# ChASE-library/ChASE

Hardware: AMD Instinct MI355X
Metric: chebyshev_filter_hemm_gflops (higher is better)
Workload: dtype complex f64

## Files before the change

chase_amd/capi.py:

```python
import ctypes as C
import os
import numpy as np

_HERE = os.path.dirname(os.path.abspath(__file__))
LIB_PATH = os.environ.get("CHASE_HIP_LIB") or os.path.join(_HERE, "lib", "libchase_hip.so")


class ChaseHipError(RuntimeError):
    def __init__(self, code, where, text=""):
        super().__init__(f"{where} failed with status {code}: {text}")
        self.code = code


def _load():
    if not os.path.exists(LIB_PATH):
        raise ImportError(
            f"{LIB_PATH} not found: build it with `make` (or `python -c 'import __graft_entry__ as g; g.build()'`). "
            "chase_amd has no CPU fallback.")
    try:
        import torch
    except Exception:
        pass
    return C.CDLL(LIB_PATH, mode=C.RTLD_GLOBAL)

# ... 141 lines not shown

    def timer_start(self):
        check(lib.chase_hip_timer_start(self.h), "timer_start")

    def timer_stop(self):
        ms = C.c_float()
        check(lib.chase_hip_timer_stop(self.h, C.byref(ms)), "timer_stop")
        return ms.value

    def gemm(self, opA, m, n, k, alpha, A, lda, B, ldb, beta, Cm, ldc, cplx):
        op = opA.encode()[0:1]
        if cplx:
            check(lib.chase_hip_gemm_z(self.h, op, m, n, k, _z2(alpha), A, lda, B, ldb, _z2(beta), Cm, ldc), "gemm_z")
        else:
            check(lib.chase_hip_gemm_d(self.h, op, m, n, k, float(alpha), A, lda, B, ldb, float(beta), Cm, ldc),
                  "gemm_d")

    def hash64(self, ptr, m, n, ld, cplx):
        h = C.c_ulonglong()
        check(lib.chase_hip_hash64(self.h, int(cplx), m, n, ptr, ld, C.byref(h)), "hash64")
        return h.value

    def gen_clement(self, N, cplx, scale=1.0, perturb=0.0, seed=42):
        dH = self.empty((N, N), np.complex128 if cplx else np.float64)
        check(lib.chase_hip_gen_clement(self.h, int(cplx), dH.ptr, N, N, N, N, N, 1, 0, 0, N, 1, 0, 0, float(scale),
                                        float(perturb), seed), "gen_clement")
        return dH

    def load_matrix(self, path, N, cplx):
        dH = self.empty((N, N), np.complex128 if cplx else np.float64)
        check(lib.chase_hip_load_matrix_shard(self.h, str(path).encode(), int(cplx), N, N, N, N, 1, 0, N, 1, 0, dH.ptr, N),
              "load_matrix_shard")
        return dH

    def save_matrix(self, path, dA):
        cplx = dA.dtype == np.complex128
        check(lib.chase_hip_save_matrix(self.h, str(path).encode(), int(cplx), dA.shape[0],
                                        dA.shape[1] if len(dA.shape) > 1 else 1, dA.ptr, dA.shape[0]), "save_matrix")

    def gen_bse(self, N, cplx=True, dmin=1.0, dmax=11.0, offdiag=1e-3, seed=7):
        dH = self.empty((N, N), np.complex128 if cplx else np.float64)
        check(lib.chase_hip_gen_bse(self.h, int(cplx), dH.ptr, N, N, N, N, N, 1, 0, N, 1, 0, float(dmin), float(dmax),
                                    float(offdiag), seed), "gen_bse")
        return dH

    def mfma_f64_peak(self):
        t = c_double()
        check(lib.chase_hip_mfma_f64_peak(self.h, C.byref(t)), "mfma_f64_peak")
        return t.value

    def hbm_copy_peak(self, nbytes=1 << 30):
        g = c_double()
        check(lib.chase_hip_hbm_copy_peak(self.h, nbytes, C.byref(g)), "hbm_copy_peak")
        return g.value


_sig("chase_hip_set_lapack_lib", c_int, C.c_char_p)
_sig("chase_hip_lapack_provider", C.c_char_p)
_sig("chase_hip_set_host_threads", c_int, c_int)
_sig("chase_hip_ctx_set_phase", c_int, c_void_p, c_int)
_sig("chase_hip_ctx_set_gemm_min_rounds", c_int, c_void_p, c_int)
_sig("chase_hip_fill_normal", c_int, c_void_p, c_int, c_int, c_int, c_void_p, c_long, c_long, c_long, c_long,
     C.c_ulonglong)
_sig("chase_hip_gen_clement", c_int, c_void_p, c_int, c_void_p, c_long, c_int, c_int, c_long, c_int, c_int, c_int,
     c_long, c_int, c_int, c_int, c_long, c_double, c_double, C.c_ulonglong)
_sig("chase_hip_gen_bse", c_int, c_void_p, c_int, c_void_p, c_long, c_int, c_int, c_long, c_int, c_int, c_int, c_int, c_int,
     c_int, c_double, c_double, c_double, C.c_ulonglong)
_sig("chase_hip_load_matrix_shard", c_int, c_void_p, C.c_char_p, c_int, c_long, c_int, c_int, c_int, c_int, c_int, c_int,
     c_int, c_int, c_void_p, c_long)
_sig("chase_hip_save_matrix", c_int, c_void_p, C.c_char_p, c_int, c_int, c_int, c_void_p, c_long)
_sig("chase_hip_shift_diag", c_int, c_void_p, c_int, c_int, c_void_p, c_long, c_double)
_sig("chase_hip_shift_list", c_int, c_void_p, c_int, c_void_p, c_long, c_void_p, c_void_p, c_int, c_double)
_sig("chase_hip_lacpy", c_int, c_void_p, c_int, c_int, c_int, c_void_p, c_long, c_void_p, c_long)
_sig("chase_hip_swap_cols", c_int, c_void_p, c_int, c_int, c_void_p, c_long, c_long, c_long)
_sig("chase_hip_permute_cols", c_int, c_void_p, c_int, c_int, c_void_p, c_long, c_void_p, c_long, P(c_int), P(c_int),
     c_int)
_sig("chase_hip_upload_matrix", c_int, c_void_p, c_int, c_int, c_int, c_void_p, c_long, c_void_p, c_long)
_sig("chase_hip_download_matrix", c_int, c_void_p, c_int, c_int, c_int, c_void_p, c_long, c_void_p, c_long)
_sig("chase_hip_scale_rows", c_int, c_void_p, c_int, c_int, c_int, c_void_p, c_long, c_int, c_double)
_sig("chase_hip_scale_rows_bc", c_int, c_void_p, c_int, c_int, c_int, c_void_p, c_long, c_long, c_long, c_int, c_int,
     c_double)
_sig("chase_hip_conj", c_int, c_void_p, c_int, c_int, c_void_p, c_long)
_sig("chase_hip_resid_norms", c_int, c_void_p, c_int, c_int, c_int, c_void_p, c_long, c_void_p, c_long, c_void_p,
     c_void_p, c_int)
_sig("chase_hip_gemm_workspace_bytes", c_size_t, c_int, C.c_char, c_int, c_int, c_int, c_int, c_int)
_sig("chase_hip_herk", c_int, c_void_p, c_int, c_int, c_int, c_void_p, c_long, c_void_p, c_long)
_sig("chase_hip_herkx", c_int, c_void_p, c_int, c_int, c_int, c_void_p, c_long, c_void_p, c_long, c_void_p, c_long, c_int)
_sig("chase_hip_abs_trace", c_int, c_void_p, c_int, c_int, c_void_p, c_long, P(c_double))
_sig("chase_hip_potrf_upper", c_int, c_void_p, c_int, c_int, c_void_p, c_long)
_sig("chase_hip_trsm_right_upper", c_int, c_void_p, c_int, c_int, c_int, c_void_p, c_long, c_void_p, c_long)
_sig("chase_hip_cholqr", c_int, c_void_p, c_int, c_int, c_int, c_void_p, c_long, c_void_p, c_long, c_int, c_long)
_sig("chase_hip_houseqr", c_int, c_void_p, c_int, c_int, c_int, c_void_p, c_long)
_sig("chase_hip_heevd", c_int, c_void_p, c_int, c_int, c_void_p, c_long, c_void_p)
_sig("chase_hip_heevd_gpu", c_int, c_void_p, c_int, c_int, c_void_p, c_long, c_void_p)
_sig("chase_hip_heevd_host", c_int, c_int, c_int, c_void_p, c_long, c_void_p)
_sig("chase_hip_stedc", c_int, c_void_p, c_int, c_void_p, c_void_p, c_void_p, c_void_p, c_long)
_sig("chase_hip_stemr_host", c_int, c_int, c_void_p, c_void_p, c_void_p, c_void_p, c_int)
_sig("chase_hip_col_dot", c_int, c_void_p, c_int, c_int, c_int, c_void_p, c_long, c_void_p, c_long, c_void_p)
_sig("chase_hip_col_nrm2", c_int, c_void_p, c_int, c_int, c_int, c_void_p, c_long, c_void_p)
_sig("chase_hip_col_axpy", c_int, c_void_p, c_int, c_int, c_int, c_void_p, c_int, c_int, c_double, c_void_p, c_long,
     c_void_p, c_long)
_sig("chase_hip_col_scal", c_int, c_void_p, c_int, c_int, c_int, c_void_p, c_int, c_void_p, c_long)
_sig("chase_hip_pack_upper", c_int, c_void_p, c_int, c_int, c_void_p, c_long, c_void_p)
_sig("chase_hip_unpack_upper", c_int, c_void_p, c_int, c_int, c_void_p, c_void_p, c_long, c_int)


class Stats(C.Structure):
    _fields_ = [("iterations", c_size_t), ("filtered_vecs", c_size_t), ("lanczos_vecs", c_size_t),
                ("locked", c_size_t), ("t_all", c_double), ("t_init", c_double), ("t_lanczos", c_double),
                ("t_filter", c_double), ("t_qr", c_double), ("t_rr", c_double), ("t_resid", c_double),
                ("filter_ms_device", c_double), ("lowerb", c_double), ("upperb", c_double), ("lambda_", c_double)]

    def as_dict(self):
        return {k: getattr(self, k) for k, _ in self._fields_}


_sig("chase_hip_solver_create", c_int, P(c_void_p), c_void_p, c_int, c_size_t, c_size_t, c_size_t, c_void_p, c_size_t,
     c_void_p, c_size_t, c_void_p, c_int)
_sig("chase_hip_solver_destroy", c_int, c_void_p)
_sig("chase_hip_solver_set", c_int, c_void_p, C.c_char_p, c_double)
_sig("chase_hip_solver_get", c_int, c_void_p, C.c_char_p, P(c_double))
_sig("chase_hip_solver_solve", c_int, c_void_p, c_int)
ITER_FN = C.CFUNCTYPE(c_int, c_void_p, c_size_t, c_size_t, c_size_t, c_size_t)
_sig("chase_hip_solver_set_iteration_hook", c_int, c_void_p, ITER_FN, c_void_p)
_sig("chase_hip_set_gemm3m", c_int, c_int)
_sig("chase_hip_ctx_gemm_counters", c_int, c_void_p, c_int, P(c_double), P(c_double), P(C.c_ulonglong), c_int)
_sig("chase_hip_solver_stats", c_int, c_void_p, P(Stats))
_sig("chase_hip_solver_resid", P(c_double), c_void_p)
_sig("chase_hip_solver_trace", C.c_char_p, c_void_p)
_sig("chase_hip_solver_recompute_residuals", c_int, c_void_p, c_size_t, c_void_p, c_void_p)
_sig("chase_hip_solver_tape_mode", c_int, c_void_p, c_int)
_sig("chase_hip_solver_tape_data", c_int, c_void_p, P(P(c_double)), P(c_size_t))
_sig("chase_hip_solver_tape_load", c_int, c_void_p, c_void_p, c_size_t)
_sig("chase_hip_resid_norms_dev", c_int, c_void_p, c_int, c_int, c_int, c_void_p, c_long, c_void_p, c_long, c_void_p,
     c_void_p, c_int)
_sig("chase_hip_solver_peek_v", c_int, c_void_p, c_void_p, c_void_p, c_size_t)
_sig("chase_hip_solver_hash_v", c_int, c_void_p, c_void_p, c_size_t, P(C.c_ulonglong))
_sig("chase_hip_op_start", c_int, c_void_p)
_sig("chase_hip_op_end", c_int, c_void_p)
_sig("chase_hip_op_initvecs", c_int, c_void_p, c_int)
_sig("chase_hip_op_reinit_columns", c_int, c_void_p, c_size_t, P(c_size_t), c_size_t)
_sig("chase_hip_op_shift", c_int, c_void_p, c_double, c_int)
_sig("chase_hip_op_hemm", c_int, c_void_p, c_size_t, P(c_double), P(c_double), c_size_t, c_size_t)
_sig("chase_hip_op_qr", c_int, c_void_p, c_size_t, c_double)
_sig("chase_hip_op_rr", c_int, c_void_p, c_void_p, c_size_t)
_sig("chase_hip_op_resd", c_int, c_void_p, c_void_p, c_void_p, c_size_t)
_sig("chase_hip_op_swap", c_int, c_void_p, c_size_t, c_size_t)
_sig("chase_hip_op_lock", c_int, c_void_p, c_size_t)
_sig("chase_hip_op_lanczos", c_int, c_void_p, c_size_t, c_size_t, P(c_double), c_void_p, c_void_p, c_void_p)
_sig("chase_hip_op_lanczos_dos", c_int, c_void_p, c_size_t, c_size_t, c_void_p)
_sig("chase_hip_op_check_symmetry", c_int, c_void_p, P(c_int))
_sig("chase_hip_op_sym_or_herm", c_int, c_void_p, c_char)
_sig("chase_hip_complete_hermitian", c_int, c_void_p, c_int, c_char, c_int, c_void_p, c_long)
_sig("chase_hip_hash64", c_int, c_void_p, c_int, c_int, c_int, c_void_p, c_long, P(C.c_ulonglong))
_sig("chase_hip_cols_indexed", c_int, c_void_p, c_int, c_int, c_void_p, c_long, c_void_p, c_long, c_void_p, c_int)
_sig("chase_hip_tri_mask_bc", c_int, c_void_p, c_int, c_char, c_int, c_int, c_void_p, c_long, c_long, c_int, c_int, c_long, c_int,
     c_int)
_sig("chase_hip_conj_transpose_add", c_int, c_void_p, c_int, c_int, c_int, c_void_p, c_long, c_void_p, c_void_p, c_void_p, c_long)


def set_iteration_hook(solver, fn):
    if fn is None:
        solver._iter_cb = ITER_FN()
    else:
        def _cb(user, it, filtered, locked, unconverged):
            try:
                return 1 if fn(int(it), int(filtered), int(locked), int(unconverged)) else 0
            except Exception as e:
                print("iteration hook failed:", repr(e), flush=True)
                return 1
        solver._iter_cb = ITER_FN(_cb)
    check(lib.chase_hip_solver_set_iteration_hook(solver.h, solver._iter_cb, None), "set_iteration_hook")


def recompute_residuals(solver, ncols, lam=None):
    lam = np.ascontiguousarray(solver.ritzv[:ncols] if lam is None else lam, dtype=np.float64)
    out = np.zeros(ncols)
    check(lib.chase_hip_solver_recompute_residuals(solver.h, ncols, lam.ctypes.data, out.ctypes.data), "recompute_residuals")
    return out


TAPE_OFF, TAPE_RECORD, TAPE_REPLAY = 0, 1, 2


def tape_mode(solver, mode):
    check(lib.chase_hip_solver_tape_mode(solver.h, int(mode)), "tape_mode")


def tape_get(solver):
    p, n = P(c_double)(), c_size_t()
    check(lib.chase_hip_solver_tape_data(solver.h, C.byref(p), C.byref(n)), "tape_data")
    return np.ctypeslib.as_array(p, shape=(n.value,)).copy() if n.value else np.zeros(0)


def tape_load(solver, tape):
    t = np.ascontiguousarray(tape, dtype=np.float64)
    check(lib.chase_hip_solver_tape_load(solver.h, t.ctypes.data, t.size), "tape_load")


def gemm_counters(ctx, phase, reset=False):
    a, b, n = c_double(), c_double(), C.c_ulonglong()
    check(lib.chase_hip_ctx_gemm_counters(ctx.h, phase, C.byref(a), C.byref(b), C.byref(n), int(reset)), "gemm_counters")
    return a.value, b.value, n.value


class GemmLaunch(C.Structure):
    _fields_ = [(f, c_int) for f in ("row0", "col0", "k0", "m", "n", "k", "beta_one", "bn_cols", "narrow", "m3", "ragged",
                                     "glds_ok", "gm", "gn")] + \
               [("full_tiles", c_long), ("tail_tiles", c_long)] + \
               [(f, c_int) for f in ("tail_sk", "tail_kchunk", "group_rows", "forced_split")] + \
               [("slab_bytes", c_size_t), ("plane_bytes", c_size_t)]

    def as_dict(self):
        return {k: getattr(self, k) for k, _ in self._fields_}


_sig("chase_hip_gemm_plan", c_int, c_int, c_char, c_int, c_int, c_int, c_long, c_long, c_int, c_int, c_int, c_int,
     P(GemmLaunch), c_int)


def gemm_plan(cplx, op, m, n, k, lda=None, ldb=None, aligned=True, phase=0, num_cu=256, min_rounds=0):
    lda = (m if op == "N" else k) if lda is None else lda
    ldb = k if ldb is None else ldb
    args = (int(cplx), op.encode(), m, n, k, max(lda, 1), max(ldb, 1), int(aligned), phase, num_cu, min_rounds)
    cnt = lib.chase_hip_gemm_plan(*args, None, 0)
    if cnt < 0:
        check(cnt, "gemm_plan")
    out = (GemmLaunch * max(cnt, 1))()
    assert lib.chase_hip_gemm_plan(*args, out, cnt) == cnt
    return [out[i].as_dict() for i in range(cnt)]


class Solver:

    def __init__(self, ctx, H, nev, nex, V=None, h_on_device_ptr=None, N=None, cplx=None):
        self.ctx = ctx
        if h_on_device_ptr is None:
            assert H.flags.f_contiguous and H.ndim == 2 and H.shape[0] == H.shape[1]
            self.cplx = bool(np.iscomplexobj(H))
            self.N = H.shape[0]
            self.H = H
            hptr, on_dev = H.ctypes.data, 0
        else:
            self.cplx, self.N, self.H = bool(cplx), int(N), None
            hptr, on_dev = h_on_device_ptr, 1
        self.nev, self.nex = nev, nex
        dt = np.complex128 if self.cplx else np.float64
        self.V = np.zeros((self.N, nev + nex), dtype=dt, order="F") if V is None else V
        assert self.V.flags.f_contiguous and self.V.dtype == dt
        self.ritzv = np.zeros(nev + nex, dtype=np.float64)
        h = c_void_p()
        check(lib.chase_hip_solver_create(C.byref(h), ctx.h, int(self.cplx), self.N, nev, nex, hptr, self.N,
                                          self.V.ctypes.data, self.N, self.ritzv.ctypes.data, on_dev),
              "solver_create")
        self.h = h

    def close(self):
        if self.h:
            lib.chase_hip_solver_destroy(self.h)
            self.h = None

    def set(self, **kw):
        for k, v in kw.items():
            check(lib.chase_hip_solver_set(self.h, k.encode(), float(v)), f"solver_set({k})")

    def get(self, key):
        v = c_double()
        check(lib.chase_hip_solver_get(self.h, key.encode(), C.byref(v)), f"solver_get({key})")
        return v.value

    def solve(self, trace=False):
        check(lib.chase_hip_solver_solve(self.h, int(trace)), "solver_solve")
        return self.stats()

    def set_iteration_hook(self, fn):
        set_iteration_hook(self, fn)

    def stats(self):
        s = Stats()
        check(lib.chase_hip_solver_stats(self.h, C.byref(s)), "solver_stats")
        return s.as_dict()

    def resid(self):
        p = lib.chase_hip_solver_resid(self.h)
        return np.ctypeslib.as_array(p, shape=(self.nev + self.nex,)).copy()

    def trace(self):
        return lib.chase_hip_solver_trace(self.h).decode().splitlines()

    def recompute_residuals(self, ncols, lam=None):
        return recompute_residuals(self, ncols, lam)

    def peek_v(self):
        out = np.empty_like(self.V, order="F")
        check(lib.chase_hip_solver_peek_v(self.h, self.ctx.h, out.ctypes.data, self.N), "peek_v")
        return out

    def Start(self): check(lib.chase_hip_op_start(self.h), "Start")
    def End(self): check(lib.chase_hip_op_end(self.h), "End")
    def initVecs(self, random): check(lib.chase_hip_op_initvecs(self.h, int(random)), "initVecs")

    def ReinitColumns(self, fixednev, cols):
        a = (c_size_t * len(cols))(*cols)
        check(lib.chase_hip_op_reinit_columns(self.h, fixednev, a, len(cols)), "ReinitColumns")
    def Shift(self, c, isunshift=False): check(lib.chase_hip_op_shift(self.h, float(c), int(isunshift)), "Shift")

    def HEMM(self, block, alpha, beta, offset_left, offset_right=0):
        check(lib.chase_hip_op_hemm(self.h, block, _z2(alpha), _z2(beta), offset_left, offset_right), "HEMM")

    def QR(self, fixednev, cond): check(lib.chase_hip_op_qr(self.h, fixednev, float(cond)), "QR")

    def RR(self, block, offset):
        check(lib.chase_hip_op_rr(self.h, self.ritzv.ctypes.data + 8 * offset, block), "RR")

    def Resd(self, offset):
        n = self.nev + self.nex - offset
        out = np.zeros(n)
        check(lib.chase_hip_op_resd(self.h, self.ritzv.ctypes.data + 8 * offset, out.ctypes.data, offset), "Resd")
        return out

    def Swap(self, i, j): check(lib.chase_hip_op_swap(self.h, i, j), "Swap")
    def Lock(self, n): check(lib.chase_hip_op_lock(self.h, n), "Lock")

    def Lanczos(self, M, numvec):
        ub = c_double()
        if numvec == 0:
            check(lib.chase_hip_op_lanczos(self.h, M, 0, C.byref(ub), None, None, None), "Lanczos")
            return ub.value
        theta, tau, ritzV = np.zeros(M * numvec), np.zeros(M * numvec), np.zeros(M * M)
        check(lib.chase_hip_op_lanczos(self.h, M, numvec, C.byref(ub), theta.ctypes.data, tau.ctypes.data,
                                       ritzV.ctypes.data), "Lanczos")
        return ub.value, theta, tau, ritzV.reshape(M, M, order="F")

    def checkSymmetryEasy(self):
        f = c_int()
        check(lib.chase_hip_op_check_symmetry(self.h, C.byref(f)), "checkSymmetryEasy")
        return bool(f.value)

    def symOrHermMatrix(self, uplo):
        check(lib.chase_hip_op_sym_or_herm(self.h, uplo.encode()[0:1]), "symOrHermMatrix")


_sig("chase_hip_solver_create_pseudo", c_int, P(c_void_p), c_void_p, c_int, c_size_t, c_size_t, c_size_t, c_void_p,
     c_size_t, c_void_p, c_size_t, c_void_p, c_int)
_sig("chase_hip_op_hemm_h2", c_int, c_void_p, c_size_t, P(c_double), P(c_double), P(c_double), c_size_t, c_size_t)
_sig("chase_hip_op_kconj", c_int, c_void_p, c_size_t)
_sig("chase_hip_pseudo_rr_small", c_int, c_void_p, c_int, c_int, c_void_p, c_void_p, c_void_p)
_sig("chase_hip_set_identity", c_int, c_void_p, c_int, c_int, c_void_p, c_long)


_sig("chase_hip_solver_lanczos_for_h2", c_int, c_void_p, c_int, c_int, P(c_double), P(c_size_t))


class PseudoSolver(Solver):

    def __init__(self, ctx, H, nev, nex):
        assert H.flags.f_contiguous and H.shape[0] == H.shape[1]
        self.ctx, self.H = ctx, H
        self.cplx = bool(np.iscomplexobj(H))
        self.N, self.nev, self.nex = H.shape[0], nev, nex
        dt = np.complex128 if self.cplx else np.float64
        self.ncol = 2 * (nev + nex)
        self.V = np.zeros((self.N, self.ncol), dtype=dt, order="F")
        self.ritzv = np.zeros(self.ncol)
# ... 31 lines not shown
```

chase_amd/csrc/capi_blas.hip:

```cpp
#include <hip/hip_runtime.h>
#include <cmath>
#include <cstdio>
#include <cstdlib>
#include <cstring>
#include <limits>
#include <vector>
#include "../../include/chase_hip.h"
#include "ctx.h"
#include "kernels.h"
#include "host_lapack.h"

using namespace chase_hip;

#define HIPCHK(x)                                                                                                      \
    do {                                                                                                               \
        hipError_t e_ = (x);                                                                                           \
        if (e_ != hipSuccess) return hip_fail(e_, #x);                                                                 \
    } while (0)
#define KCHK(x, what)                                                                                                  \
    do {                                                                                                               \
        int e_ = (x);                                                                                                  \
        if (e_) return hip_fail((hipError_t)e_, what);                                                                 \
    } while (0)
#define RCCHK(x)                                                                                                       \
    do {                                                                                                               \
        int r_ = (x);                                                                                                  \
        if (r_) return r_;                                                                                             \
    } while (0)

namespace {
constexpr int NB = 64;

inline int ept_of(int cplx) { return cplx ? 2 : 1; }

int gemm(chase_hip_ctx* c, int cplx, char op, int m, int n, int k, double ar, double ai, const double* A, long lda,
         const double* B, long ldb, double br, double bi, double* C, long ldc)
{
    if (m <= 0 || n <= 0) return 0;
    const double alpha[2] = {ar, ai}, beta[2] = {br, bi};
    return c->gemm(cplx != 0, op, m, n, k, alpha, A, lda, B, ldb, beta, C, ldc);
}
}

extern "C" {

int chase_hip_set_lapack_lib(const char* path) { return lapack_bind(path); }
const char* chase_hip_lapack_provider(void)
{
    lapack_bind(nullptr);
    return lapack_provider();
}
int chase_hip_host_lapack_warmup(void)
{
    int rc = lapack_bind(nullptr);
    if (rc) return rc;
    static bool done = false;
    if (done) return 0;
    const int n = 8;
    double d[n], e[n], w[n], Z[n * n];
    for (int i = 0; i < n; ++i) { d[i] = i; e[i] = 0.5; }
    rc = host_stedc(n, d, e, w, Z, n);
    if (rc) return rc;
    for (int i = 0; i < n; ++i) { d[i] = i; e[i] = 0.5; }
    rc = host_stemr(n, d, e, w, Z, n);
    if (rc) return rc;
    double A[2 * n * n];
    for (int i = 0; i < 2 * n * n; ++i) A[i] = 0.0;
    for (int i = 0; i < n; ++i) A[2 * (i + i * n)] = 1.0 + i;
    rc = host_heevd(true, n, A, n, w);
    if (rc) return rc;
    done = true;
    return 0;
}

int chase_hip_set_host_threads(int n)
{
    lapack_bind(nullptr);
    lapack_set_threads(n);
    return 0;
}

int chase_hip_ctx_set_phase(chase_hip_ctx* c, int phase)
{
    if (!c) return set_error(CHASE_HIP_EINVAL, "set_phase: NULL ctx");
    (void)hipSetDevice(c->device);
    c->phase = phase;
    return 0;
}

int chase_hip_ctx_set_gemm_min_rounds(chase_hip_ctx* c, int rounds)
{
    if (!c) return set_error(CHASE_HIP_EINVAL, "ctx_set_gemm_min_rounds: NULL context");
    c->gemm_min_rounds = rounds < 0 ? 0 : (rounds > 16 ? 16 : rounds);
    return 0;
}

int chase_hip_fill_normal(chase_hip_ctx* c, int cplx, int m, int n, void* X, long ldx, long grow0, long gcol0, long gld,
                          unsigned long long seed)
{
    if (!c || !X) return set_error(CHASE_HIP_EINVAL, "fill_normal: NULL argument");
    (void)hipSetDevice(c->device);
    if (c->oplog_on) c->oplog_add("fill_normal", m, n, 0, 0);
    if (m < 0 || n < 0 || ldx < m) return set_error(CHASE_HIP_EINVAL, "fill_normal: bad shape");
    KCHK(fill_normal(c->stream, cplx != 0, (double*)X, ldx, m, n, grow0, gcol0, gld, seed), "fill_normal");
    return 0;
}

int chase_hip_fill_normal_bc(chase_hip_ctx* c, int cplx, int m, int n, void* X, long ldx, long gld, int mb, int pr,
                             int pi, unsigned long long seed)
{
    if (!c || !X) return set_error(CHASE_HIP_EINVAL, "fill_normal_bc: NULL argument");
    (void)hipSetDevice(c->device);
    if (c->oplog_on) c->oplog_add("fill_normal_bc", m, n, 0, 0);
    if (m < 0 || n < 0 || ldx < m || mb <= 0 || pr <= 0) return set_error(CHASE_HIP_EINVAL, "fill_normal_bc: bad shape");
    KCHK(fill_normal(c->stream, cplx != 0, (double*)X, ldx, m, n, 0, 0, gld, seed, mb, pr, pi), "fill_normal_bc");
    return 0;
}

int chase_hip_rows_indexed(chase_hip_ctx* c, int cplx, const void* in, long ld_in, void* out, long ld_out,
                           const int* idx_dev, int np, int ncols, int scatter)
{
    if (!c) return set_error(CHASE_HIP_EINVAL, "rows_indexed: NULL ctx");
    (void)hipSetDevice(c->device);
    if (c->oplog_on) c->oplog_add("rows_indexed", np, ncols, scatter, 0);
    KCHK(rows_indexed(c->stream, cplx != 0, (const double*)in, ld_in, (double*)out, ld_out, idx_dev, np, ncols, scatter),
         "rows_indexed");
    return 0;
}

int chase_hip_hash64(chase_hip_ctx* c, int cplx, int m, int n, const void* A, long lda, unsigned long long* out_host)
{
    if (!c || !out_host) return set_error(CHASE_HIP_EINVAL, "hash64: NULL argument");
    (void)hipSetDevice(c->device);
    if (m < 0 || n < 0 || lda < m) return set_error(CHASE_HIP_EINVAL, "hash64: bad shape");
    *out_host = 0;
    if (m == 0 || n == 0) return 0;
    if (!A) return set_error(CHASE_HIP_EINVAL, "hash64: NULL matrix");
    const int e = ept_of(cplx);
    RCCHK(c->ensure_buf(chase_hip_ctx::BUF_SCAL, 4096));
    unsigned long long* d = (unsigned long long*)c->bufs[chase_hip_ctx::BUF_SCAL];
    HIPCHK(hipMemsetAsync(d, 0, sizeof(unsigned long long), c->stream));
    KCHK(hash64(c->stream, (const double*)A, lda * e, (long)m * e, n, d), "hash64");
    HIPCHK(hipMemcpyAsync(out_host, d, sizeof(unsigned long long), hipMemcpyDeviceToHost, c->stream));
    HIPCHK(hipStreamSynchronize(c->stream));
    return 0;
}

int chase_hip_cols_indexed(chase_hip_ctx* c, int cplx, int m, const void* in, long ld_in, void* out, long ld_out,
                           const int* idx_dev, int ncols)
{
    if (!c) return set_error(CHASE_HIP_EINVAL, "cols_indexed: NULL ctx");
    (void)hipSetDevice(c->device);
    if (c->oplog_on) c->oplog_add("cols_indexed", m, ncols, 0, 0);
    if (m < 0 || ncols < 0 || ld_in < m || ld_out < m) return set_error(CHASE_HIP_EINVAL, "cols_indexed: bad shape");
    if (m == 0 || ncols == 0) return 0;
    if (!in || !out || !idx_dev) return set_error(CHASE_HIP_EINVAL, "cols_indexed: NULL argument");
    const int e = ept_of(cplx);
    KCHK(copy_cols_indexed_range(c->stream, (const double*)in, ld_in * e, (double*)out, ld_out * e, (long)m * e, idx_dev, 0, ncols),
         "cols_indexed");
    return 0;
}

int chase_hip_complete_hermitian(chase_hip_ctx* c, int cplx, char uplo, int n, void* A, long lda)
{
    if (!c) return set_error(CHASE_HIP_EINVAL, "complete_hermitian: NULL ctx");
    (void)hipSetDevice(c->device);
    if (c->oplog_on) c->oplog_add("complete_hermitian", n, uplo, 0, 0);
    if (uplo != 'U' && uplo != 'L' && uplo != 'u' && uplo != 'l') return set_error(CHASE_HIP_EINVAL, "complete_hermitian: uplo must be 'U' or 'L'");
    if (n < 0 || lda < n) return set_error(CHASE_HIP_EINVAL, "complete_hermitian: bad shape");
    if (n == 0) return 0;
    if (!A) return set_error(CHASE_HIP_EINVAL, "complete_hermitian: NULL matrix");
    if (uplo == 'U' || uplo == 'u') KCHK(mirror_upper(c->stream, (double*)A, lda, n, ept_of(cplx)), "mirror_upper");
    else KCHK(mirror_lower(c->stream, (double*)A, lda, n, ept_of(cplx), 0), "mirror_lower");
    return 0;
}

int chase_hip_tri_mask_bc(chase_hip_ctx* c, int cplx, char uplo, int mloc, int nloc, void* H, long ldh, long mb, int pr, int pi,
                          long nb, int pc, int pj)
{
    if (!c) return set_error(CHASE_HIP_EINVAL, "tri_mask_bc: NULL ctx");
    (void)hipSetDevice(c->device);
    if (c->oplog_on) c->oplog_add("tri_mask_bc", mloc, nloc, uplo, 0);
    if (uplo != 'U' && uplo != 'L' && uplo != 'u' && uplo != 'l') return set_error(CHASE_HIP_EINVAL, "tri_mask_bc: uplo must be 'U' or 'L'");
    if (mloc < 0 || nloc < 0 || ldh < mloc || mb <= 0 || nb <= 0 || pr <= 0 || pc <= 0 || pi < 0 || pi >= pr || pj < 0 || pj >= pc)
        return set_error(CHASE_HIP_EINVAL, "tri_mask_bc: bad shape / layout");
    if (mloc == 0 || nloc == 0) return 0;
    if (!H) return set_error(CHASE_HIP_EINVAL, "tri_mask_bc: NULL matrix");
    KCHK(tri_mask_bc(c->stream, cplx != 0, (double*)H, ldh, mloc, nloc, mb, pr, pi, nb, pc, pj, (uplo == 'U' || uplo == 'u') ? 1 : 0),
         "tri_mask_bc");
    return 0;
}

int chase_hip_conj_transpose_add(chase_hip_ctx* c, int cplx, int nr, int nc, const void* P, long ldp, const int* rowmap_dev,
                                 const int* colmap_dev, void* H, long ldh)
{
    if (!c) return set_error(CHASE_HIP_EINVAL, "conj_transpose_add: NULL ctx");
    (void)hipSetDevice(c->device);
    if (c->oplog_on) c->oplog_add("conj_transpose_add", nr, nc, 0, 0);
    if (nr < 0 || nc < 0 || ldp < nr) return set_error(CHASE_HIP_EINVAL, "conj_transpose_add: bad shape");
    if (nr == 0 || nc == 0) return 0;
    if (!P || !H || !rowmap_dev || !colmap_dev) return set_error(CHASE_HIP_EINVAL, "conj_transpose_add: NULL argument");
    KCHK(conj_transpose_add(c->stream, cplx != 0, (const double*)P, ldp, nr, nc, rowmap_dev, colmap_dev, (double*)H, ldh),
         "conj_transpose_add");
    return 0;
}

int chase_hip_gen_clement(chase_hip_ctx* c, int cplx, void* H, long ldh, int mloc, int nloc, long N, int mb, int pr,
                          int pi, long roff, int nb, int pc, int pj, long coff, double scale, double perturb,
                          unsigned long long seed)
{
    if (!c || !H) return set_error(CHASE_HIP_EINVAL, "gen_clement: NULL argument");
    (void)hipSetDevice(c->device);
    if (mloc < 0 || nloc < 0 || ldh < mloc || mb <= 0 || nb <= 0 || pr <= 0 || pc <= 0)
        return set_error(CHASE_HIP_EINVAL, "gen_clement: bad shape");
    KCHK(gen_clement(c->stream, cplx != 0, (double*)H, ldh, mloc, nloc, N, mb, pr, pi, roff, nb, pc, pj, coff, scale,
                     perturb, seed),
         "gen_clement");
    return 0;
}

int chase_hip_gen_bse(chase_hip_ctx* c, int cplx, void* H, long ldh, int mloc, int nloc, long N, int mb, int pr, int pi,
                      int nb, int pc, int pj, double dmin, double dmax, double offdiag, unsigned long long seed)
{
    if (!c || !H) return set_error(CHASE_HIP_EINVAL, "gen_bse: NULL argument");
    (void)hipSetDevice(c->device);
    if (mloc < 0 || nloc < 0 || ldh < mloc || mb <= 0 || nb <= 0 || pr <= 0 || pc <= 0 || N <= 0 || N % 2)
        return set_error(CHASE_HIP_EINVAL, "gen_bse: bad shape (N must be even)");
    KCHK(gen_bse(c->stream, cplx != 0, (double*)H, ldh, mloc, nloc, N, mb, pr, pi, nb, pc, pj, dmin, dmax, offdiag, seed),
         "gen_bse");
    return 0;
}

int chase_hip_shift_diag(chase_hip_ctx* c, int cplx, int n, void* H, long ldh, double shift)
{
    if (!c || (!H && n > 0)) return set_error(CHASE_HIP_EINVAL, "shift_diag: NULL argument");
    (void)hipSetDevice(c->device);
    if (c->oplog_on) c->oplog_add("shift_diag", n, 0, 0, 0);
    if (n < 0 || ldh < n) return set_error(CHASE_HIP_EINVAL, "shift_diag: bad shape");
    KCHK(shift_diag(c->stream, (double*)H, ldh, n, ept_of(cplx), shift), "shift_diag");
    return 0;
}

int chase_hip_shift_list(chase_hip_ctx* c, int cplx, void* H, long ldh, const int* rows_dev, const int* cols_dev, int cnt,
                         double shift)
{
    if (!c) return set_error(CHASE_HIP_EINVAL, "shift_list: NULL ctx");
    (void)hipSetDevice(c->device);
    if (c->oplog_on) c->oplog_add("shift_list", cnt, 0, 0, 0);
    if (cnt < 0) return set_error(CHASE_HIP_EINVAL, "shift_list: negative count");
    KCHK(shift_list(c->stream, (double*)H, ldh, rows_dev, cols_dev, cnt, ept_of(cplx), shift), "shift_list");
    return 0;
}

int chase_hip_lacpy(chase_hip_ctx* c, int cplx, int m, int n, const void* A, long lda, void* B, long ldb)
{
    if (!c) return set_error(CHASE_HIP_EINVAL, "lacpy: NULL ctx");
    (void)hipSetDevice(c->device);
    if (c->oplog_on) c->oplog_add("lacpy", m, n, 0, 0);
    if (m < 0 || n < 0 || lda < m || ldb < m) return set_error(CHASE_HIP_EINVAL, "lacpy: bad shape");
    if (m == 0 || n == 0) return 0;
    const int e = ept_of(cplx);
    KCHK(copy2d(c->stream, (const double*)A, lda * e, (double*)B, ldb * e, (long)m * e, n), "lacpy");
    return 0;
}

int chase_hip_swap_cols(chase_hip_ctx* c, int cplx, int m, void* V, long ldv, long i, long j)
{
    if (!c || !V) return set_error(CHASE_HIP_EINVAL, "swap_cols: NULL argument");
    (void)hipSetDevice(c->device);
    if (c->oplog_on) c->oplog_add("swap_cols", m, 0, 0, 0);
    if (i == j) return 0;
    const int e = ept_of(cplx);
    double* v = (double*)V;
    KCHK(swap_cols(c->stream, v + i * ldv * e, v + j * ldv * e, (long)m * e), "swap_cols");
    return 0;
}

int chase_hip_permute_cols(chase_hip_ctx* c, int cplx, int m, void* V, long ldv, void* scratch, long lds_,
                           const int* src_host, const int* dst_host, int cnt)
{
    if (!c || !V || !scratch) return set_error(CHASE_HIP_EINVAL, "permute_cols: NULL argument");
    (void)hipSetDevice(c->device);
    if (c->oplog_on) c->oplog_add("permute_cols", m, cnt, 0, 0);
    if (cnt <= 0) return 0;
    const int e = ept_of(cplx);
    RCCHK(c->ensure_buf(chase_hip_ctx::BUF_LAMBDA, (size_t)2 * cnt * sizeof(int) + 64));
    int* ds = (int*)c->bufs[chase_hip_ctx::BUF_LAMBDA];
    int* dd = ds + cnt;
    HIPCHK(hipMemcpyAsync(ds, src_host, (size_t)cnt * sizeof(int), hipMemcpyHostToDevice, c->stream));
    HIPCHK(hipMemcpyAsync(dd, dst_host, (size_t)cnt * sizeof(int), hipMemcpyHostToDevice, c->stream));
    HIPCHK(hipStreamSynchronize(c->stream));
    KCHK(copy_cols_indexed(c->stream, (const double*)V, ldv * e, (double*)scratch, lds_ * e, (long)m * e, ds, dd, cnt),
         "permute gather");
    KCHK(copy_cols_indexed(c->stream, (const double*)scratch, lds_ * e, (double*)V, ldv * e, (long)m * e, dd, dd, cnt),
         "permute scatter");
    return 0;
}

int chase_hip_upload_matrix(chase_hip_ctx* c, int cplx, int m, int n, const void* host, long ldh, void* dev, long ldd)
{
    if (!c) return set_error(CHASE_HIP_EINVAL, "upload_matrix: NULL ctx");
    (void)hipSetDevice(c->device);
    if (c->oplog_on) c->oplog_add("upload_matrix", m, n, 0, 0);
    if (m <= 0 || n <= 0) return 0;
    const size_t es = sizeof(double) * ept_of(cplx);
    HIPCHK(hipMemcpy2DAsync(dev, (size_t)ldd * es, host, (size_t)ldh * es, (size_t)m * es, n, hipMemcpyHostToDevice,
                            c->stream));
    HIPCHK(hipStreamSynchronize(c->stream));
    return 0;
}
int chase_hip_download_matrix(chase_hip_ctx* c, int cplx, int m, int n, const void* dev, long ldd, void* host, long ldh)
{
    if (!c) return set_error(CHASE_HIP_EINVAL, "download_matrix: NULL ctx");
    (void)hipSetDevice(c->device);
    if (c->oplog_on) c->oplog_add("download_matrix", m, n, 0, 0);
    if (m <= 0 || n <= 0) return 0;
    const size_t es = sizeof(double) * ept_of(cplx);
    HIPCHK(hipMemcpy2DAsync(host, (size_t)ldh * es, dev, (size_t)ldd * es, (size_t)m * es, n, hipMemcpyDeviceToHost,
                            c->stream));
    HIPCHK(hipStreamSynchronize(c->stream));
    return 0;
}

int chase_hip_scale_rows(chase_hip_ctx* c, int cplx, int m, int n, void* X, long ldx, int row0, double s)
{
    if (!c) return set_error(CHASE_HIP_EINVAL, "scale_rows: NULL ctx");
// ... 410 lines not shown
```

chase_amd/csrc/gemm_mfma_f64.hip:

```cpp

#include <hip/hip_runtime.h>
#include <stdint.h>
#include <algorithm>
#include <atomic>
#include <cstdlib>
#include <type_traits>
#include "../../include/chase_hip.h"
#include "kernels.h"

#ifndef CHASE_M3_PIPELINE
#define CHASE_M3_PIPELINE 1
#endif
#ifndef CHASE_M3_SPLANE
#define CHASE_M3_SPLANE 1
#endif
#ifndef CHASE_M3_DEPTH
#define CHASE_M3_DEPTH 2
#endif

namespace chase_hip {

typedef double d4_t __attribute__((ext_vector_type(4)));
typedef double d2_t __attribute__((ext_vector_type(2)));
typedef d2_t d2u_t __attribute__((aligned(8)));

template <bool CPLX, bool OPA_C, bool NARROW = false>
struct Cfg {
    static_assert(!(CPLX && NARROW), "the complex tile is 64 columns wide already");
    static constexpr int NTHREADS = 256;
    static constexpr int WAVES_M = 4, WAVES_N = 1;
    static constexpr int TM = 2;
    static constexpr int TN = (CPLX || NARROW) ? 4 : 8;
    static constexpr int BM = 16 * TM * WAVES_M;
    static constexpr int BN = 16 * TN * WAVES_N;
    static constexpr int BK = CPLX ? 8 : 16;
    static constexpr int KPU = CPLX ? 1 : 2;
    static constexpr int RPU = CPLX ? 1 : 2;
    static constexpr int A_UNITS = OPA_C ? BM * 8 : BK * (BM / RPU);
    static constexpr int B_UNITS = BN * 8;
    static constexpr int A_PASSES = A_UNITS / NTHREADS;
    static constexpr int B_PASSES = B_UNITS / NTHREADS;
    static constexpr int STAGE_UNITS = A_UNITS + B_UNITS;
    static constexpr int EPT = CPLX ? 2 : 1;
    static constexpr int STAGES = (CPLX || NARROW) ? 3 : 2;
    static constexpr bool PIPELINED = CPLX || NARROW;
    static constexpr int A_GLDS = A_UNITS / 64, B_GLDS = B_UNITS / 64;
    static constexpr int GLDS_PER_WAVE = (A_GLDS + B_GLDS) / 4;
};

__device__ __forceinline__ int kidx(int r, int ku) { return r * 8 + (ku ^ ((r >> 1) & 7)); }

__device__ __forceinline__ unsigned xcd_remap(unsigned b, unsigned nblk)
{
    const unsigned q = nblk >> 3, r = nblk & 7u, x = b & 7u;
    const unsigned base = (x < r) ? x * (q + 1) : r * (q + 1) + (x - r) * q;
    return base + (b >> 3);
}

__host__ __device__ __forceinline__ void tile_coords(int t, int gm, int gn, int GR, int& bm, int& bn)
{
    const int gsz = GR * gn;
    const int g = t / gsz;
    const int first = g * GR;
    const int rows = (gm - first < GR) ? gm - first : GR;
    const int r = t - g * gsz;
    bm = first + r % rows;
    bn = r / rows;
}

struct GemmArgs {
    const double* A; const double* B; double* C;
    long lda, ldb, ldc;
    int m, n, k;
    int gm, gn;
    int group_rows;
    int bn_cols;
    int full_tiles, tail_sk, tail_kchunk;
    double* slabs;
    int glds_ok;
    const double* S; int s_nkt;
    double alpha_re, alpha_im, beta_re, beta_im;
};

template <bool CPLX, bool OPA_C, int TAG, bool RAGGED, bool M3, bool NARROW = false>
__global__ __launch_bounds__(256, 2) void gemm_f64_kernel(GemmArgs p)
{
    static_assert(CPLX || !M3, "3M applies to complex products");
    using C_ = Cfg<CPLX, OPA_C, NARROW>;
    constexpr int BM = C_::BM, BN = C_::BN, BK = C_::BK, TM = C_::TM, TN = C_::TN;
    constexpr int EPT = C_::EPT, KPU = C_::KPU, RPU = C_::RPU;
    constexpr int UM = BM / RPU;

    extern __shared__ __attribute__((aligned(16))) d2_t lds[];

    const int tid = threadIdx.x;
    const int lane = tid & 63, wave = tid >> 6;
    const int wm = wave % C_::WAVES_M, wn = wave / C_::WAVES_M;
    const int c16 = lane & 15, q = lane >> 4;

    unsigned tile;
    int kbeg = 0, kend = p.k;
    bool raw = false;
    double* slab = nullptr;
    if (blockIdx.x < (unsigned)p.full_tiles) {
        tile = xcd_remap(blockIdx.x, (unsigned)p.full_tiles);
    } else {
        const unsigned P = xcd_remap(blockIdx.x - (unsigned)p.full_tiles, gridDim.x - (unsigned)p.full_tiles);
        tile = (unsigned)p.full_tiles + P / (unsigned)p.tail_sk;
        const int bz = (int)(P % (unsigned)p.tail_sk);
        kbeg = bz * p.tail_kchunk;
        kend = min(p.k, kbeg + p.tail_kchunk);
        raw = true;
        slab = p.slabs + (size_t)P * (BM * BN * EPT);
    }
    int bm, bn;
    tile_coords((int)tile, p.gm, p.gn, p.group_rows, bm, bn);
    const int row0 = bm * BM, col0 = bn * p.bn_cols;
    const int nkt = (kend > kbeg) ? (kend - kbeg + BK - 1) / BK : 0;

    const bool interior = (row0 + BM <= p.m) && (col0 + BN <= p.n);

    d2_t ra[C_::A_PASSES], rb[C_::B_PASSES];

    auto load_tile = [&](int k0) {
        const bool kfull = (k0 + BK <= kend);
        if (interior && kfull) {
            #pragma unroll
            for (int ps = 0; ps < C_::A_PASSES; ++ps) {
                const int idx = ps * 256 + tid;
                if constexpr (!OPA_C) {
                    const int kk = idx / UM, u = idx % UM;
                    const double* g = p.A + ((long)(k0 + kk) * p.lda + row0 + u * RPU) * EPT;
                    ra[ps] = *(const d2u_t*)g;
                } else {
                    const int r = idx >> 3, ku = idx & 7;
                    const double* g = p.A + ((long)(row0 + r) * p.lda + k0 + ku * KPU) * EPT;
                    ra[ps] = *(const d2u_t*)g;
                }
            }
            #pragma unroll
            for (int ps = 0; ps < C_::B_PASSES; ++ps) {
                const int idx = ps * 256 + tid;
                const int r = idx >> 3, ku = idx & 7;
                const double* g = p.B + ((long)(col0 + r) * p.ldb + k0 + ku * KPU) * EPT;
                rb[ps] = *(const d2u_t*)g;
            }
        } else {
            #pragma unroll
            for (int ps = 0; ps < C_::A_PASSES; ++ps) {
                const int idx = ps * 256 + tid;
                d2_t v = {0.0, 0.0};
                if constexpr (!OPA_C) {
                    const int kk = idx / UM, u = idx % UM;
                    const int gi = row0 + u * RPU, gk = k0 + kk;
                    if (gk < kend) {
                        const double* g = p.A + ((long)gk * p.lda + gi) * EPT;
                        if constexpr (CPLX) { if (gi < p.m) v = *(const d2u_t*)g; }
                        else { if (gi < p.m) v.x = g[0]; if (gi + 1 < p.m) v.y = g[1]; }
                    }
                } else {
                    const int r = idx >> 3, ku = idx & 7;
                    const int gi = row0 + r, gk = k0 + ku * KPU;
                    if (gi < p.m) {
                        const double* g = p.A + ((long)gi * p.lda + gk) * EPT;
                        if constexpr (CPLX) { if (gk < kend) v = *(const d2u_t*)g; }
                        else { if (gk < kend) v.x = g[0]; if (gk + 1 < kend) v.y = g[1]; }
                    }
                }
                ra[ps] = v;
            }
            #pragma unroll
            for (int ps = 0; ps < C_::B_PASSES; ++ps) {
                const int idx = ps * 256 + tid;
                const int r = idx >> 3, ku = idx & 7;
                const int gj = col0 + r, gk = k0 + ku * KPU;
                d2_t v = {0.0, 0.0};
                if (gj < p.n) {
                    const double* g = p.B + ((long)gj * p.ldb + gk) * EPT;
                    if constexpr (CPLX) { if (gk < kend) v = *(const d2u_t*)g; }
                    else { if (gk < kend) v.x = g[0]; if (gk + 1 < kend) v.y = g[1]; }
                }
                rb[ps] = v;
            }
        }
    };

    auto store_tile = [&](int stage) {
        d2_t* sA = lds + stage * C_::STAGE_UNITS;
        d2_t* sB = sA + C_::A_UNITS;
        #pragma unroll
        for (int ps = 0; ps < C_::A_PASSES; ++ps) {
            const int idx = ps * 256 + tid;
            if constexpr (!OPA_C) {
                sA[idx] = ra[ps];
            } else {
                const int r = idx >> 3, ku = idx & 7;
                sA[kidx(r, ku)] = ra[ps];
            }
        }
        #pragma unroll
        for (int ps = 0; ps < C_::B_PASSES; ++ps) {
            const int idx = ps * 256 + tid;
            const int r = idx >> 3, ku = idx & 7;
            sB[kidx(r, ku)] = rb[ps];
        }
    };

    constexpr int NACC = CPLX ? (M3 ? 3 : 2) : 1;
    d4_t acc[NACC][TN][TM];
    #pragma unroll
    for (int z = 0; z < NACC; ++z)
        #pragma unroll
        for (int j = 0; j < TN; ++j)
            #pragma unroll
            for (int i = 0; i < TM; ++i) acc[z][j][i] = d4_t{0.0, 0.0, 0.0, 0.0};

    const int wrow = wm * (16 * TM);
    const int wcol = wn * (16 * TN);
    const int jv = RAGGED ? __builtin_amdgcn_readfirstlane(min(p.bn_cols >> 4, max(0, (p.n - col0 - wcol + 15) >> 4))) : TN;

    struct Frag { d2_t b[TN]; double a[TM][2]; };

    auto read_chunk = [&](int stage, int ch, Frag& f) __attribute__((always_inline)) {
        const d2_t* sA = lds + stage * C_::STAGE_UNITS;
        const d2_t* sB = sA + C_::A_UNITS;
        const int ku = 4 * ch + q;
        if constexpr (CPLX || OPA_C) {
            #pragma unroll
            for (int i = 0; i < TM; ++i) {
                const int r = wrow + 16 * i + c16;
                d2_t v;
                if constexpr (OPA_C) v = sA[kidx(r, ku)];
                else                 v = sA[ku * UM + r];
                f.a[i][0] = v.x; f.a[i][1] = v.y;
            }
            #pragma unroll
            for (int j = 0; j < TN; ++j) f.b[j] = sB[kidx(wcol + 16 * j + c16, ku)];
        } else {
            #pragma unroll
            for (int j = 0; j < TN; ++j) f.b[j] = sB[kidx(wcol + 16 * j + c16, ku)];
            #pragma unroll
            for (int pr = 0; pr < TM / 2; ++pr)
                #pragma unroll
                for (int s = 0; s < 2; ++s) {
                    const int kk = 8 * ch + 2 * q + s;
                    const d2_t v = sA[kk * UM + (wrow / 2) + 16 * pr + c16];
                    f.a[2 * pr][s] = v.x;
                    f.a[2 * pr + 1][s] = v.y;
                }
        }
    };

    auto no_hook = [](int) __attribute__((always_inline)) {};
    auto mfma_chunk = [&](const Frag& f, auto&& hook) __attribute__((always_inline)) {
        constexpr bool FULL = !RAGGED;
        if constexpr (CPLX && M3) {
            double sa[TM], sb[TN];
            #pragma unroll
            for (int i = 0; i < TM; ++i) sa[i] = OPA_C ? f.a[i][0] - f.a[i][1] : f.a[i][0] + f.a[i][1];
            #pragma unroll
            for (int j = 0; j < TN; ++j) sb[j] = f.b[j].x + f.b[j].y;
            #pragma unroll
            for (int j = 0; j < TN; ++j) {
                #pragma unroll
                for (int i = 0; i < TM; ++i) {
                    if (FULL || j < jv) {
                        acc[0][j][i] = __builtin_amdgcn_mfma_f64_16x16x4f64(f.b[j].x, f.a[i][0], acc[0][j][i], 0, 0, 0);
                        acc[1][j][i] = __builtin_amdgcn_mfma_f64_16x16x4f64(f.b[j].y, f.a[i][1], acc[1][j][i], 0, 0, 0);
                        acc[2][j][i] = __builtin_amdgcn_mfma_f64_16x16x4f64(sb[j], sa[i], acc[2][j][i], 0, 0, 0);
                    }
                    hook(TM * j + i);
                }
            }
        } else if constexpr (CPLX) {
            double nb[TN];
            #pragma unroll
            for (int j = 0; j < TN; ++j) nb[j] = OPA_C ? -f.b[j].x : -f.b[j].y;
            #pragma unroll
            for (int j = 0; j < TN; ++j) {
                if (FULL || j < jv)
                #pragma unroll
                for (int i = 0; i < TM; ++i) {
                    acc[0][j][i] = __builtin_amdgcn_mfma_f64_16x16x4f64(f.b[j].x, f.a[i][0], acc[0][j][i], 0, 0, 0);
                    acc[1][j][i] = __builtin_amdgcn_mfma_f64_16x16x4f64(f.b[j].y, f.a[i][0], acc[1][j][i], 0, 0, 0);
                }
                hook(j);
            }
            #pragma unroll
            for (int j = 0; j < TN; ++j) {
                if (FULL || j < jv)
                #pragma unroll
                for (int i = 0; i < TM; ++i) {
                    acc[0][j][i] = __builtin_amdgcn_mfma_f64_16x16x4f64(OPA_C ? f.b[j].y : nb[j], f.a[i][1], acc[0][j][i], 0, 0, 0);
                    acc[1][j][i] = __builtin_amdgcn_mfma_f64_16x16x4f64(OPA_C ? nb[j] : f.b[j].x, f.a[i][1], acc[1][j][i], 0, 0, 0);
                }
                hook(TN + j);
            }
        } else {
            #pragma unroll
            for (int s = 0; s < 2; ++s)
                #pragma unroll
                for (int j = 0; j < TN; ++j) {
                    if (FULL || j < jv)
                    #pragma unroll
                    for (int i = 0; i < TM; ++i)
                        acc[0][j][i] = __builtin_amdgcn_mfma_f64_16x16x4f64(
                            s == 0 ? f.b[j].x : f.b[j].y, f.a[i][s], acc[0][j][i], 0, 0, 0);
                    hook(s * TN + j);
                }
        }
    };

    auto compute = [&](int stage, auto&& hook) __attribute__((always_inline)) {
        if constexpr (C_::PIPELINED && !M3) {
            Frag f0, f1;
            read_chunk(stage, 0, f0);
            read_chunk(stage, 1, f1);
            __builtin_amdgcn_sched_barrier(0);
            mfma_chunk(f0, hook);
            mfma_chunk(f1, no_hook);
        } else {
            {
                Frag f;
                read_chunk(stage, 0, f);
                mfma_chunk(f, hook);
            }
            {
                Frag f;
                read_chunk(stage, 1, f);
                mfma_chunk(f, no_hook);
            }
        }
    };

    bool done = false;
    {
        const int nfull = (kend - kbeg) / BK;
        if ((row0 + BM <= p.m) && nfull >= 1 && p.glds_ok) {
            const int wv = __builtin_amdgcn_readfirstlane(wave);
            constexpr int NA = C_::A_GLDS / 4, NB = C_::B_GLDS / 4;
            const char* sa[NA];
            unsigned va[NA];
#ifdef CHASE_DIAG_SAME_A
            const int row0_src = 0;
#else
            const int row0_src = row0;
#endif
#ifdef CHASE_DIAG_SAME_B
            const int col0_src = 0;
#else
            const int col0_src = col0;
#endif
            const char* sb = (const char*)(p.B + ((long)col0_src * p.ldb + kbeg) * EPT);
            unsigned vb[NB];
            #pragma unroll
            for (int u = 0; u < NA; ++u) {
                const int t = wv * NA + u;
                if constexpr (!OPA_C) {
                    const int kk = CPLX ? (t >> 1) : t, half = CPLX ? (t & 1) : 0;
                    sa[u] = (const char*)(p.A + ((long)(kbeg + kk) * p.lda + row0_src) * EPT + (long)half * 128);
                    va[u] = (unsigned)lane * 16u;
                } else {
                    const int rl = lane >> 3, ku = (lane & 7) ^ ((4 * t + (lane >> 4)) & 7);
                    sa[u] = (const char*)(p.A + ((long)(row0_src + 8 * t) * p.lda + kbeg) * EPT);
                    va[u] = (unsigned)(((long)rl * p.lda + ku * KPU) * EPT * 8);
                }
            }
            #pragma unroll
            for (int u = 0; u < NB; ++u) {
                const int t = wv * NB + u;
                const int r = 8 * t + (lane >> 3), ku = (lane & 7) ^ ((r >> 1) & 7);
                const int rc = min(r, p.n - 1 - col0);
                vb[u] = (unsigned)(((long)rc * p.ldb + ku * KPU) * EPT * 8);
            }
            const long stepA = (OPA_C ? (long)BK * EPT : (long)BK * p.lda * EPT) * 8;
            constexpr long stepB = (long)BK * EPT * 8;
            int st_issue = 0;
            auto issue_one = [&](int u, int stage) __attribute__((always_inline)) {
                constexpr bool SPLIT = CPLX && M3 && CHASE_M3_SPLANE;
                d2_t* sA = SPLIT ? lds + stage * C_::A_UNITS : lds + stage * C_::STAGE_UNITS;
                d2_t* sB = SPLIT ? lds + C_::STAGES * C_::A_UNITS + stage * C_::B_UNITS : sA + C_::A_UNITS;
                if (u < NA) {
                    const unsigned dst = (unsigned)(size_t)(__attribute__((address_space(3))) void*)(sA + (wv * NA + u) * 64);
                    asm volatile("s_mov_b32 m0, %2\n\ts_nop 0\n\tglobal_load_lds_dwordx4 %0, %1"
                                 :: "v"(va[u]), "s"(sa[u]), "s"(dst) : "memory");
                    sa[u] += stepA;
                } else {
                    const int ub = u - NA;
                    const unsigned dst = (unsigned)(size_t)(__attribute__((address_space(3))) void*)(sB + (wv * NB + ub) * 64);
                    asm volatile("s_mov_b32 m0, %2\n\ts_nop 0\n\tglobal_load_lds_dwordx4 %0, %1"
                                 :: "v"(vb[ub]), "s"(sb), "s"(dst) : "memory");
                }
                if (u == NA + NB - 1) sb += stepB;
            };
            auto issue = [&]() __attribute__((always_inline)) {
                #pragma unroll
                for (int u = 0; u < NA + NB; ++u) issue_one(u, st_issue);
                st_issue = (st_issue + 1 == C_::STAGES) ? 0 : st_issue + 1;
            };
            if constexpr (C_::PIPELINED && !M3) {
                constexpr int G = C_::GLDS_PER_WAVE;
                const int npre = min(nfull, C_::STAGES);
                for (int t = 0; t < npre; ++t) issue();
                if (npre == 3)      asm volatile("s_waitcnt vmcnt(%0)" ::"n"(2 * G) : "memory");
                else if (npre == 2) asm volatile("s_waitcnt vmcnt(%0)" ::"n"(G) : "memory");
                else                asm volatile("s_waitcnt vmcnt(0)" ::: "memory");
                __builtin_amdgcn_s_barrier();
                asm volatile("" ::: "memory");
                Frag fA, fB;
                read_chunk(0, 0, fA);
                constexpr std::true_type yes{};
                constexpr std::false_type no{};
                auto kstep = [&](int kt, int st, auto fill_c) __attribute__((always_inline)) {
                    const int stn = (st + 1 == C_::STAGES) ? 0 : st + 1;
                    read_chunk(st, 1, fB);
                    __builtin_amdgcn_sched_barrier(0);
                    mfma_chunk(fA, no_hook);
                    __builtin_amdgcn_sched_barrier(0);
                    if (C_::STAGES > 2 && (decltype(fill_c)::value || kt + 2 < nfull))
                        asm volatile("s_waitcnt vmcnt(%0) lgkmcnt(0)" ::"n"(G) : "memory");
                    else
                        asm volatile("s_waitcnt vmcnt(0) lgkmcnt(0)" ::: "memory");
                    __builtin_amdgcn_s_barrier();
                    asm volatile("" ::: "memory");
                    read_chunk(stn, 0, fA);
                    __builtin_amdgcn_sched_barrier(0);
                    mfma_chunk(fB, [&](int slot) __attribute__((always_inline)) {
                        if (decltype(fill_c)::value && slot < NA + NB) {
                            __builtin_amdgcn_sched_barrier(0);
                            issue_one(slot, st);
                            __builtin_amdgcn_sched_barrier(0);
                        }
                    });
                    __builtin_amdgcn_sched_barrier(0);
                };
                static_assert(2 * TN >= NA + NB, "one copy per MFMA group of the cluster");
                int st = 0, kt = 0;
                for (; kt + C_::STAGES < nfull; ++kt) { kstep(kt, st, yes); st = (st + 1 == C_::STAGES) ? 0 : st + 1; }
                for (; kt + 1 < nfull; ++kt)          { kstep(kt, st, no);  st = (st + 1 == C_::STAGES) ? 0 : st + 1; }
                read_chunk(st, 1, fB);
                __builtin_amdgcn_sched_barrier(0);
                mfma_chunk(fA, no_hook);
                __builtin_amdgcn_sched_barrier(0);
                mfma_chunk(fB, no_hook);
            } else if constexpr (CPLX && M3 && CHASE_M3_SPLANE) {
                constexpr int G = C_::GLDS_PER_WAVE;
                constexpr int S_UNITS = 256;
                d2_t* const sring = lds + C_::STAGES * C_::STAGE_UNITS;
                const char* ssrc = (const char*)(p.S + ((size_t)bn * (size_t)p.s_nkt + (size_t)(kbeg / BK)) * 512) + wv * 1024;
                const unsigned vs = (unsigned)lane * 16u;
                int s_issue = 0;
                auto issue_s = [&]() __attribute__((always_inline)) {
                    const unsigned dst = (unsigned)(size_t)(__attribute__((address_space(3))) void*)(sring + s_issue * S_UNITS + wv * 64);
                    asm volatile("s_mov_b32 m0, %2\n\ts_nop 0\n\tglobal_load_lds_dwordx4 %0, %1"
                                 :: "v"(vs), "s"(ssrc), "s"(dst) : "memory");
                    ssrc += 4096;
                    s_issue ^= 1;
                };
                constexpr bool DEPTH1 = (CHASE_M3_DEPTH == 1);
                const int npre = min(nfull, DEPTH1 ? 2 : C_::STAGES);
                issue_s(); issue();
                if (npre > 1) { issue_s(); issue(); }
                if (npre > 2) issue();
                if (npre == 3)      asm volatile("s_waitcnt vmcnt(%0)" ::"n"(2 * G + 1) : "memory");
                else if (npre == 2) asm volatile("s_waitcnt vmcnt(%0)" ::"n"(G + 1) : "memory");
                else                asm volatile("s_waitcnt vmcnt(0)" ::: "memory");
                __builtin_amdgcn_s_barrier();
                asm volatile("" ::: "memory");
                auto ld_a = [&](int stage, int ch, int i) __attribute__((always_inline)) -> d2_t {
                    const d2_t* sA = lds + stage * C_::A_UNITS;
                    const int ku = 4 * ch + q, r = wrow + 16 * i + c16;
                    if constexpr (OPA_C) return sA[kidx(r, ku)];
                    else                 return sA[ku * UM + r];
                };
                auto ld_b = [&](int stage, int ch, int j) __attribute__((always_inline)) -> d2_t {
                    const d2_t* sB = lds + C_::STAGES * C_::A_UNITS + stage * C_::B_UNITS;
                    return sB[kidx(wcol + 16 * j + c16, 4 * ch + q)];
                };
                static_assert(((C_::STAGES * C_::STAGE_UNITS * 16) & 4096) == 0, "ring base must have bit 12 clear");
                unsigned soff = (unsigned)(C_::STAGES * C_::STAGE_UNITS * 16) + (unsigned)((q >> 1) * 1024 + c16 * 16 + (q & 1) * 8);
                auto ld_s = [&](int ch, int j) __attribute__((always_inline)) -> double {
                    return *(const double*)((const char*)lds + soff + ch * 2048 + j * 256);
                };
                d2_t aC[TM], bF[TN];
                double sS[TN];
                #pragma unroll
                for (int i = 0; i < TM; ++i) aC[i] = ld_a(0, 0, i);
                #pragma unroll
                for (int j = 0; j < TN; ++j) { bF[j] = ld_b(0, 0, j); sS[j] = ld_s(0, j); }
                auto cluster = [&](int nstage, int nch, auto more_c, auto fill_t_c, auto fill_s_c, int fstage = 0) __attribute__((always_inline)) {
                    constexpr bool more = decltype(more_c)::value;
                    constexpr bool fill_t = decltype(fill_t_c)::value;
                    constexpr bool fill_s = decltype(fill_s_c)::value;
                    #pragma unroll
                    for (int i = 0; i < TM; ++i) {
#ifdef CHASE_DIAG_NO_SA
                        const double sa = aC[i].x;
#else
                        const double sa = OPA_C ? aC[i].x - aC[i].y : aC[i].x + aC[i].y;
#endif
                        #pragma unroll
                        for (int j = 0; j < TN; ++j) {
                            if (!RAGGED || j < jv) {
                                acc[0][j][i] = __builtin_amdgcn_mfma_f64_16x16x4f64(bF[j].x, aC[i].x, acc[0][j][i], 0, 0, 0);
                                acc[1][j][i] = __builtin_amdgcn_mfma_f64_16x16x4f64(bF[j].y, aC[i].y, acc[1][j][i], 0, 0, 0);
                                acc[2][j][i] = __builtin_amdgcn_mfma_f64_16x16x4f64(sS[j], sa, acc[2][j][i], 0, 0, 0);
                            }
                            const int slot = TN * i + j;
                            if (fill_s && slot == 0) {
                                __builtin_amdgcn_sched_barrier(0);
                                issue_s();
                                __builtin_amdgcn_sched_barrier(0);
                            }
                            if (fill_t && slot >= 1 && slot - 1 < NA + NB) {
                                __builtin_amdgcn_sched_barrier(0);
                                issue_one(slot - 1, fstage);
                                __builtin_amdgcn_sched_barrier(0);
                            }
                            __builtin_amdgcn_sched_barrier(0);
                            if (more && i == TM - 1) { bF[j] = ld_b(nstage, nch, j); sS[j] = ld_s(nch, j); }
                            __builtin_amdgcn_sched_barrier(0);
                        }
                        if (more) aC[i] = ld_a(nstage, nch, i);
                        __builtin_amdgcn_sched_barrier(0);
                    }
                };
                static_assert(TM * TN >= NA + NB + 1, "one copy per (i, j) slot of the cluster");
                constexpr std::true_type yes{};
                constexpr std::false_type no{};
                auto kstep = [&](int kt, int st, auto fill_t_c, auto fill_s_c) __attribute__((always_inline)) {
                    const int stn = (st + 1 == C_::STAGES) ? 0 : st + 1;
                    cluster(st, 1, yes, no, no);
                    if (!DEPTH1 && (decltype(fill_t_c)::value || kt + 2 < nfull))
                        asm volatile("s_waitcnt vmcnt(%0) lgkmcnt(0)" ::"n"(G) : "memory");
                    else
                        asm volatile("s_waitcnt vmcnt(0) lgkmcnt(0)" ::: "memory");
                    __builtin_amdgcn_s_barrier();
                    asm volatile("" ::: "memory");
                    soff ^= 4096u;
                    __builtin_amdgcn_sched_barrier(0);
                    cluster(stn, 0, yes, fill_t_c, fill_s_c, DEPTH1 ? (st == 0 ? C_::STAGES - 1 : st - 1) : st);
                };
                int kt = 0;
                constexpr int AHEAD = DEPTH1 ? 2 : C_::STAGES;
                if constexpr (C_::STAGES == 3) {
                    for (; kt + 2 + AHEAD < nfull; kt += 3) {
                        kstep(kt, 0, yes, yes);
                        kstep(kt + 1, 1, yes, yes);
                        kstep(kt + 2, 2, yes, yes);
                    }
                }
                int st = 0;
                for (; kt + AHEAD < nfull; ++kt) { kstep(kt, st, yes, yes); st = (st + 1 == C_::STAGES) ? 0 : st + 1; }
                if (!DEPTH1 && kt + 2 < nfull)        { kstep(kt, st, no, yes);  st = (st + 1 == C_::STAGES) ? 0 : st + 1; ++kt; }
                for (; kt + 1 < nfull; ++kt)          { kstep(kt, st, no, no);   st = (st + 1 == C_::STAGES) ? 0 : st + 1; }
                cluster(st, 1, yes, no, no);
                __builtin_amdgcn_sched_barrier(0);
                cluster(st, 1, no, no, no);
            } else if constexpr (CPLX && M3 && CHASE_M3_PIPELINE) {
                constexpr int G = C_::GLDS_PER_WAVE;
                const int npre = min(nfull, C_::STAGES);
                for (int t = 0; t < npre; ++t) issue();
                if (npre == 3)      asm volatile("s_waitcnt vmcnt(%0)" ::"n"(2 * G) : "memory");
                else if (npre == 2) asm volatile("s_waitcnt vmcnt(%0)" ::"n"(G) : "memory");
                else                asm volatile("s_waitcnt vmcnt(0)" ::: "memory");
                __builtin_amdgcn_s_barrier();
                asm volatile("" ::: "memory");
                auto ld_a = [&](int stage, int ch, d2_t (&a)[TM]) __attribute__((always_inline)) {
                    const d2_t* sA = lds + stage * C_::STAGE_UNITS;
                    const int ku = 4 * ch + q;
                    #pragma unroll
                    for (int i = 0; i < TM; ++i) {
                        const int r = wrow + 16 * i + c16;
                        if constexpr (OPA_C) a[i] = sA[kidx(r, ku)];
                        else                 a[i] = sA[ku * UM + r];
                    }
                };
                auto ld_b = [&](int stage, int ch, int j) __attribute__((always_inline)) -> d2_t {
                    const d2_t* sB = lds + stage * C_::STAGE_UNITS + C_::A_UNITS;
                    return sB[kidx(wcol + 16 * j + c16, 4 * ch + q)];
                };
                d2_t aC[TM], aN[TM], bF[TN];
                ld_a(0, 0, aC);
                #pragma unroll
                for (int j = 0; j < TN; ++j) bF[j] = ld_b(0, 0, j);
                auto cluster = [&](int nstage, int nch, auto more_c, auto fill_c, int fstage = 0) __attribute__((always_inline)) {
                    constexpr bool more = decltype(more_c)::value;
                    constexpr bool fill = decltype(fill_c)::value;
                    double sa[TM];
                    #pragma unroll
                    for (int i = 0; i < TM; ++i) sa[i] = OPA_C ? aC[i].x - aC[i].y : aC[i].x + aC[i].y;
                    if (more) ld_a(nstage, nch, aN);
                    #pragma unroll
                    for (int j = 0; j < TN; ++j) {
                        const double sb = bF[j].x + bF[j].y;
                        #pragma unroll
                        for (int i = 0; i < TM; ++i) {
                            if (!RAGGED || j < jv) {
                                acc[0][j][i] = __builtin_amdgcn_mfma_f64_16x16x4f64(bF[j].x, aC[i].x, acc[0][j][i], 0, 0, 0);
                                acc[1][j][i] = __builtin_amdgcn_mfma_f64_16x16x4f64(bF[j].y, aC[i].y, acc[1][j][i], 0, 0, 0);
                                acc[2][j][i] = __builtin_amdgcn_mfma_f64_16x16x4f64(sb, sa[i], acc[2][j][i], 0, 0, 0);
                            }
                            if (fill && (TM * j + i) < NA + NB) {
                                __builtin_amdgcn_sched_barrier(0);
                                issue_one(TM * j + i, fstage);
                                __builtin_amdgcn_sched_barrier(0);
                            }
                        }
                        if (more) bF[j] = ld_b(nstage, nch, j);
                        __builtin_amdgcn_sched_barrier(0);
                    }
                    #pragma unroll
                    for (int i = 0; i < TM; ++i) aC[i] = aN[i];
                };
                static_assert(TM * TN >= NA + NB, "one copy per (j, i) slot of the cluster");
                constexpr std::true_type yes{};
                constexpr std::false_type no{};
                auto kstep = [&](int kt, int st, auto fill_c) __attribute__((always_inline)) {
                    const int stn = (st + 1 == C_::STAGES) ? 0 : st + 1;
                    cluster(st, 1, yes, no);
                    if (C_::STAGES > 2 && (decltype(fill_c)::value || kt + 2 < nfull))
                        asm volatile("s_waitcnt vmcnt(%0) lgkmcnt(0)" ::"n"(G) : "memory");
                    else
                        asm volatile("s_waitcnt vmcnt(0) lgkmcnt(0)" ::: "memory");
                    __builtin_amdgcn_s_barrier();
                    asm volatile("" ::: "memory");
                    __builtin_amdgcn_sched_barrier(0);
                    cluster(stn, 0, yes, fill_c, st);
                };
                int kt = 0;
#ifdef CHASE_NO_RAGGED_C_UNROLL
                constexpr bool unroll3 = (C_::STAGES == 3) && !(RAGGED && OPA_C);
#else
                constexpr bool unroll3 = (C_::STAGES == 3);
#endif
                if constexpr (unroll3) {
                    for (; kt + 2 + C_::STAGES < nfull; kt += 3) {
                        kstep(kt, 0, yes);
                        kstep(kt + 1, 1, yes);
                        kstep(kt + 2, 2, yes);
                    }
                }
                int st = 0;
                for (; kt + C_::STAGES < nfull; ++kt) { kstep(kt, st, yes); st = (st + 1 == C_::STAGES) ? 0 : st + 1; }
                for (; kt + 1 < nfull; ++kt)          { kstep(kt, st, no);  st = (st + 1 == C_::STAGES) ? 0 : st + 1; }
                cluster(st, 1, yes, no);
                __builtin_amdgcn_sched_barrier(0);
                cluster(st, 1, no, no);
            } else {
                constexpr int DEPTH = C_::STAGES - 1;
                issue();
                if (DEPTH > 1 && nfull > 1) issue();
                int st_comp = 0;
                auto kstep = [&](int kt, auto fill_c) __attribute__((always_inline)) {
                    if (DEPTH > 1 && kt + 1 < nfull) asm volatile("s_waitcnt vmcnt(%0)" ::"n"(C_::GLDS_PER_WAVE) : "memory");
                    else                             asm volatile("s_waitcnt vmcnt(0)" ::: "memory");
                    __builtin_amdgcn_s_barrier();
                    asm volatile("" ::: "memory");
                    const int st_fill = (st_comp + DEPTH) % C_::STAGES;
                    compute(st_comp, [&](int slot) __attribute__((always_inline)) {
                        if (decltype(fill_c)::value && slot < NA + NB) {
                            __builtin_amdgcn_sched_barrier(0);
                            issue_one(slot, st_fill);
                            __builtin_amdgcn_sched_barrier(0);
                        }
                    });
                    st_comp = (st_comp + 1 == C_::STAGES) ? 0 : st_comp + 1;
                };
                static_assert(2 * TN >= NA + NB, "one copy per MFMA group of the cluster");
                int kt = 0;
                for (; kt + DEPTH < nfull; ++kt) kstep(kt, std::true_type());
                for (; kt < nfull; ++kt)         kstep(kt, std::false_type());
            }
            if constexpr (!M3) {
            if (nfull * BK < kend - kbeg) {
                const int st = nfull % C_::STAGES;
                __syncthreads();
                load_tile(kbeg + nfull * BK);
                store_tile(st);
                __syncthreads();
                compute(st, no_hook);
            }
            }
            done = true;
        }
    }
    if constexpr (!M3) {
    if (!done && nkt > 0) {
        load_tile(kbeg);
        store_tile(0);
        __syncthreads();
        for (int kt = 0; kt < nkt; ++kt) {
            const int cur = kt & 1;
            if (kt + 1 < nkt) load_tile(kbeg + (kt + 1) * BK);
            compute(cur, no_hook);
            if (kt + 1 < nkt) store_tile(cur ^ 1);
            __syncthreads();
        }
    }

    }
    double* Cb = raw ? slab : p.C;
    const long ldc_e = raw ? BM : p.ldc;
    const int srow0 = raw ? 0 : row0, scol0 = raw ? 0 : col0;
    const int m_e = raw ? BM : p.m, n_e = raw ? BN : p.n;
    const double are = p.alpha_re, aim = p.alpha_im, bre = p.beta_re, bim = p.beta_im;
    const bool has_beta = (bre != 0.0) || (bim != 0.0);

    #pragma unroll
    for (int j = 0; j < TN; ++j) {
        if (j >= jv) continue;
        #pragma unroll
        for (int g = 0; g < 4; ++g) {
            __builtin_amdgcn_sched_barrier(0);
            const int gj = scol0 + wcol + 16 * j + q + 4 * g;
            if (gj >= n_e) continue;
            if constexpr (CPLX) {
                #pragma unroll
                for (int i = 0; i < TM; ++i) {
                    const int gi = srow0 + wrow + 16 * i + c16;
                    if (gi >= m_e) continue;
                    double* c = Cb + ((long)gj * ldc_e + gi) * 2;
                    double xr, xi;
                    if constexpr (M3) {
                        const double p1 = acc[0][j][i][g], p2 = acc[1][j][i][g], p3 = acc[NACC - 1][j][i][g];
                        xr = OPA_C ? p1 + p2 : p1 - p2;
                        xi = OPA_C ? (p3 - p1) + p2 : (p3 - p1) - p2;
                    } else { xr = acc[0][j][i][g]; xi = acc[1][j][i][g]; }
                    d2_t out;
                    if (raw) { out = d2_t{xr, xi}; }
                    else {
                        out = d2_t{are * xr - aim * xi, are * xi + aim * xr};
                        if (has_beta) {
                            const d2_t old = *(const d2u_t*)c;
                            out.x += bre * old.x - bim * old.y;
                            out.y += bre * old.y + bim * old.x;
                        }
                    }
                    *(d2u_t*)c = out;
                }
            } else if constexpr (!OPA_C) {
                #pragma unroll
                for (int pr = 0; pr < TM / 2; ++pr) {
                    const int gi = srow0 + wrow + 32 * pr + 2 * c16;
                    if (gi >= m_e) continue;
                    double* c = Cb + (long)gj * ldc_e + gi;
                    double x0 = acc[0][j][2 * pr][g], x1 = acc[0][j][2 * pr + 1][g];
                    if (!raw) {
                        x0 *= are; x1 *= are;
                        if (has_beta) { x0 += bre * c[0]; if (gi + 1 < m_e) x1 += bre * c[1]; }
                    }
                    if (gi + 1 < m_e) *(d2u_t*)c = d2_t{x0, x1};
                    else c[0] = x0;
                }
            } else {
                #pragma unroll
                for (int i = 0; i < TM; ++i) {
                    const int gi = srow0 + wrow + 16 * i + c16;
                    if (gi >= m_e) continue;
                    double* c = Cb + (long)gj * ldc_e + gi;
                    double x0 = acc[0][j][i][g];
                    if (!raw) { x0 *= are; if (has_beta) x0 += bre * c[0]; }
                    c[0] = x0;
                }
            }
        }
    }
}

constexpr int TAIL_PARTS = 4;
template <bool CPLX, int BM, int BN>
__global__ __launch_bounds__(256) void tail_reduce_kernel(const double* __restrict__ slabs, int first_tile, int sk,
                                                          int gn, int m, int n, double* __restrict__ C, long ldc,
                                                          double are, double aim, double bre, double bim, int group_rows,
                                                          int bn_cols)
{
    constexpr int EPT = CPLX ? 2 : 1;
    const int tt = blockIdx.x / TAIL_PARTS, part = blockIdx.x % TAIL_PARTS;
    const int tile = first_tile + tt;
    int bm, bn;
    tile_coords(tile, (m + BM - 1) / BM, gn, group_rows, bm, bn);
    const int row0 = bm * BM, col0 = bn * bn_cols;
    const double* base = slabs + (size_t)tt * sk * (BM * BN * EPT);
    const bool has_beta = (bre != 0.0) || (bim != 0.0);
    constexpr int SHARE = BM * BN / TAIL_PARTS;
    for (int e = part * SHARE + threadIdx.x; e < (part + 1) * SHARE; e += 256) {
        const int li = e % BM, lj = e / BM;
        const int gi = row0 + li, gj = col0 + lj;
        if (gi >= m || gj >= n || lj >= bn_cols) continue;
        if constexpr (CPLX) {
            double sr = 0.0, si = 0.0;
            for (int z = 0; z < sk; ++z) {
                const d2_t v = *(const d2_t*)(base + ((size_t)z * BM * BN + e) * 2);
                sr += v.x; si += v.y;
            }
            double* c = C + ((long)gj * ldc + gi) * 2;
            double orr = are * sr - aim * si, oi = are * si + aim * sr;
            if (has_beta) { const double cr = c[0], ci = c[1]; orr += bre * cr - bim * ci; oi += bre * ci + bim * cr; }
            c[0] = orr; c[1] = oi;
        } else {
            double sum = 0.0;
            for (int z = 0; z < sk; ++z) sum += base[(size_t)z * BM * BN + e];
            double* c = C + (long)gj * ldc + gi;
            double o = are * sum;
            if (has_beta) o += bre * c[0];
            c[0] = o;
        }
    }
}

__global__ __launch_bounds__(256) void splane_kernel(const double* __restrict__ B, long ldb, int n, int k, int bn_cols, int nkt,
                                                     double* __restrict__ S)
{
    __shared__ double sm[64][65];
    const int bn = blockIdx.y, k0 = blockIdx.x * 64, col0 = bn * bn_cols, t = threadIdx.x;
    #pragma unroll 4
    for (int it = 0; it < 16; ++it) {
        const int c = 4 * it + (t >> 6), kl = t & 63;
        const int col = min(col0 + c, n - 1);
        double v = 0.0;
        if (k0 + kl < k) { const d2_t b = *(const d2u_t*)(B + ((long)col * ldb + k0 + kl) * 2); v = b.x + b.y; }
        sm[kl][c] = v;
    }
    __syncthreads();
    #pragma unroll 4
    for (int it = 0; it < 8; ++it) {
        const int kp = 4 * it + (t >> 6), c = t & 63, kk = k0 + 2 * kp;
        if (kk < k) *(d2_t*)(S + ((size_t)bn * nkt + (kk >> 3)) * 512 + ((kk & 7) >> 1) * 128 + c * 2) = d2_t{sm[2 * kp][c], sm[2 * kp + 1][c]};
    }
}
static size_t splane_bytes(int n, int k, int bn_cols)
{
    if (bn_cols <= 0 || bn_cols > 64) bn_cols = 64;
    return (size_t)((n + bn_cols - 1) / bn_cols) * (size_t)((k + 7) / 8) * 4096;
}

static std::atomic<int> g_gemm3m{-1};
int gemm3m_enabled()
{
    int v = g_gemm3m.load(std::memory_order_relaxed);
    if (v < 0) {
        const char* e = getenv("CHASE_HIP_GEMM3M");
        v = (e ? atoi(e) != 0 : true) ? 1 : 0;
        g_gemm3m.store(v, std::memory_order_relaxed);
    }
    return v;
}
void gemm3m_set(int on) { g_gemm3m.store(on ? 1 : 0, std::memory_order_relaxed); }

static int choose_tail_sk(long tail, long slots, int nkt, size_t slab_bytes, size_t ws_bytes)
{
    if (tail <= 0 || nkt < 16) return 1;
    const int sk_max = (int)std::min<long>(std::min<long>(64, nkt / 8), (long)(ws_bytes / (slab_bytes * (size_t)tail)));
    int sk = 1;
    double best = 1e30;
    for (int c = 1; c <= sk_max; ++c) {
        const double rounds = (double)((tail * c + slots - 1) / slots) / c + 0.004 * c;
        if (rounds < best - 1e-12) { best = rounds; sk = c; }
    }
    return sk;
}

struct LaunchInfo { int device; double* exec_flops; int min_rounds; };

static int forced_split(long tiles, long slots, int nkt, size_t slab_bytes, int min_rounds)
{
    if (min_rounds <= 0 || tiles <= 0 || tiles >= (long)min_rounds * slots) return 1;
    long sk = ((long)min_rounds * slots + tiles - 1) / tiles;
    sk = std::min<long>(sk, 8);
    sk = std::min<long>(sk, nkt / 64);
    sk = std::min<long>(sk, (long)(GEMM_WS_CAP / (slab_bytes * (size_t)tiles)));
    return sk < 2 ? 1 : (int)sk;
}
constexpr int MAX_DEVICES = 64;

struct PartPlan { long full, tail; int sk; size_t ws_bytes; bool forced = false; };
template <bool CPLX, bool OPA_C, bool NARROW = false>
static PartPlan plan_part(int m, int n, int k, int bn_cols, int num_cu, int min_rounds)
{
    using C_ = Cfg<CPLX, OPA_C, NARROW>;
    if (bn_cols <= 0 || bn_cols > C_::BN) bn_cols = C_::BN;
    const long tiles = (long)((m + C_::BM - 1) / C_::BM) * ((n + bn_cols - 1) / bn_cols);
    const long slots = 2L * num_cu;
    const int nkt = (k + C_::BK - 1) / C_::BK;
    const size_t slab_bytes = (size_t)C_::BM * C_::BN * sizeof(double) * C_::EPT;
    PartPlan p{tiles, 0, 1, 0};
    if (m <= 0 || n <= 0 || k <= 0) return p;
    const int fs = forced_split(tiles, slots, nkt, slab_bytes, min_rounds);
    if (fs > 1) { p.full = 0; p.tail = tiles; p.sk = fs; p.forced = true; }
    else {
        const long tail = tiles % slots;
        const int sk = tail > 0 ? choose_tail_sk(tail, slots, nkt, slab_bytes, GEMM_WS_CAP) : 1;
        if (sk > 1) { p.full = tiles - tail; p.tail = tail; p.sk = sk; }
    }
    p.ws_bytes = p.tail > 0 ? slab_bytes * (size_t)p.tail * p.sk : 0;
    return p;
}

struct ColPiece { int c0, n, bn_cols; bool narrow; };
struct ColsPlan { int npieces; ColPiece piece[2]; };
template <bool CPLX, bool OPA_C> static int uniform_tile_cols(int m, int n, int k);
static int real_narrow_mode()
{
    static const int mode = [] { const char* e = getenv("CHASE_HIP_REAL_NARROW"); return e ? atoi(e) : 1; }();
    return mode;
}
template <bool CPLX, bool OPA_C>
static ColsPlan plan_cols(int m, int n, int k, bool have_ws)
{
    using C_ = Cfg<CPLX, OPA_C>;
    const ColsPlan single{1, {{0, n, 0, false}, {0, 0, 0, false}}};
    const int rem = n % C_::BN;
    if constexpr (!CPLX) {
        const int mode = real_narrow_mode();
        auto narrow_stride = [](int r) { const int ng = (r + 15) / 16, nt = (ng + 3) / 4; return 16 * ((ng + nt - 1) / nt); };
        if (mode != 0 && n <= 64) return ColsPlan{1, {{0, n, narrow_stride(n), true}, {0, 0, 0, false}}};
        if (!have_ws || n <= C_::BN || rem == 0) return single;
        if (rem > C_::BN - 16) return single;
        if (mode != 0 && rem <= 64) {
            const double t_group = 2.0 * m * (double)k * 16.0 / 75.0e12;
            const double t_pass = (double)m * k * 8.0 / 5.5e12;
            const int g = (rem + 15) / 16;
            if (mode == 2 || 0.75 * t_pass + 0.68 * g * t_group + 10e-6 < C_::TN * t_group)
                return ColsPlan{2, {{0, n - rem, 0, false}, {n - rem, rem, 16 * g, true}}};
            return single;
        }
        return ColsPlan{2, {{0, n - rem, 0, false}, {n - rem, rem, 0, false}}};
    } else {
        const bool balanced = (C_::WAVES_N == 1);
        if (!(have_ws && balanced && n > C_::BN && rem != 0 && rem <= C_::BN - 16)) return single;
        const int bnu = uniform_tile_cols<CPLX, OPA_C>(m, n, k);
        if (bnu > 0) return ColsPlan{1, {{0, n, bnu, false}, {0, 0, 0, false}}};
        return ColsPlan{2, {{0, n - rem, 0, false}, {n - rem, rem, 0, false}}};
    }
}

struct PartDecision {
    int gm, gn, bn_cols, group_rows;
    PartPlan pl;
    int kchunk;
    bool glds_ok, ragged, m3;
    size_t plane_bytes;
};
template <bool CPLX, bool OPA_C, bool NARROW>
static PartDecision decide_part(int m, int n, int k, long lda, long ldb, bool aligned16, bool have_ws, int num_cu,
                                bool allow3m, int min_rounds, int bn_cols)
{
    using C_ = Cfg<CPLX, OPA_C, NARROW>;
    PartDecision d;
    if (bn_cols <= 0 || bn_cols > C_::BN) bn_cols = C_::BN;
    d.bn_cols = bn_cols;
    d.gm = (m + C_::BM - 1) / C_::BM; d.gn = (n + bn_cols - 1) / bn_cols;
    static const int group_env = [] { const char* e = getenv("CHASE_HIP_TILE_GROUP"); const int v = e ? atoi(e) : 0; return v < 0 ? 0 : v; }();
    d.group_rows = group_env > 0 ? group_env : ((d.gn >= 16 && (long)d.gm * d.gn >= 16L * 2 * num_cu) ? 4 : 2);
    const int nkt = (k + C_::BK - 1) / C_::BK;
    d.pl = plan_part<CPLX, OPA_C, NARROW>(m, n, k, bn_cols, num_cu, min_rounds);
    if (!have_ws) d.pl = PartPlan{(long)d.gm * d.gn, 0, 1, 0};
    d.kchunk = ((nkt + d.pl.sk - 1) / d.pl.sk) * C_::BK;
    d.glds_ok = aligned16 && (CPLX || ((lda % 2 == 0) && (ldb % 2 == 0))) &&
                (double)std::max(lda, ldb) * C_::BM * C_::EPT * 8 < 4.0e9;
    d.ragged = (bn_cols < C_::BN) || (d.gn * C_::BN - n) >= 16;
    d.m3 = CPLX && allow3m && gemm3m_enabled() != 0 && d.glds_ok && k > 0 && (m % C_::BM == 0) && (k % C_::BK == 0) &&
           (d.kchunk % C_::BK == 0) && (!CHASE_M3_SPLANE || have_ws);
    d.plane_bytes = (d.m3 && CHASE_M3_SPLANE) ? splane_bytes(n, k, bn_cols) : 0;
    return d;
}

template <bool CPLX, bool OPA_C, int TAG, bool NARROW = false>
static int launch_gemm_part(hipStream_t st, int m, int n, int k, const double* alpha, const double* A, long lda,
                            const double* B, long ldb, const double* beta, double* C, long ldc,
                            double* ws, size_t ws_bytes, int num_cu, bool allow3m, const LaunchInfo& li,
                            int bn_cols = 0)
{
    using C_ = Cfg<CPLX, OPA_C, NARROW>;
    if (m <= 0 || n <= 0) return 0;
    const PartDecision d = decide_part<CPLX, OPA_C, NARROW>(m, n, k, lda, ldb, (((uintptr_t)A | (uintptr_t)B) % 16 == 0),
                                                            ws != nullptr, num_cu, allow3m, li.min_rounds, bn_cols);
    if (d.pl.ws_bytes > ws_bytes) return GEMM_F64_EWORKSPACE;
    GemmArgs a;
    a.A = A; a.B = B; a.C = C; a.lda = lda; a.ldb = ldb; a.ldc = ldc; a.m = m; a.n = n; a.k = k;
    a.gm = d.gm; a.gn = d.gn; a.bn_cols = d.bn_cols; a.group_rows = d.group_rows;
    a.alpha_re = alpha[0]; a.alpha_im = CPLX ? alpha[1] : 0.0;
    a.beta_re = beta[0];   a.beta_im = CPLX ? beta[1] : 0.0;
    const long full = d.pl.full, tail = d.pl.tail;
    const int sk = d.pl.sk;
    a.full_tiles = (int)full; a.tail_sk = sk; a.tail_kchunk = d.kchunk; a.slabs = ws;
    a.glds_ok = d.glds_ok;
    const unsigned grid = (unsigned)(full + tail * sk);
    const size_t lds_bytes = (size_t)C_::STAGES * C_::STAGE_UNITS * sizeof(d2_t);
    const size_t lds_bytes3 = lds_bytes + (CHASE_M3_SPLANE ? 2 * 4096 : 0);
    const bool ragged = d.ragged;
    const int dev = (li.device >= 0 && li.device < MAX_DEVICES) ? li.device : 0;
    static std::atomic<bool> attr_set[MAX_DEVICES];
    if (!attr_set[dev].load(std::memory_order_relaxed)) {
        (void)hipFuncSetAttribute((const void*)gemm_f64_kernel<CPLX, OPA_C, TAG, false, false, NARROW>, hipFuncAttributeMaxDynamicSharedMemorySize, (int)lds_bytes);
        (void)hipFuncSetAttribute((const void*)gemm_f64_kernel<CPLX, OPA_C, TAG, true, false, NARROW>, hipFuncAttributeMaxDynamicSharedMemorySize, (int)lds_bytes);
        attr_set[dev].store(true, std::memory_order_relaxed);
    }
    constexpr bool CAN3M = CPLX;
    const bool ok3m = d.m3;
    a.S = nullptr; a.s_nkt = 0;
    if constexpr (CAN3M) {
        static std::atomic<bool> attr3[MAX_DEVICES];
        if (!attr3[dev].load(std::memory_order_relaxed)) {
            (void)hipFuncSetAttribute((const void*)gemm_f64_kernel<CPLX, OPA_C, TAG, false, CAN3M>, hipFuncAttributeMaxDynamicSharedMemorySize, (int)lds_bytes3);
            (void)hipFuncSetAttribute((const void*)gemm_f64_kernel<CPLX, OPA_C, TAG, true, CAN3M>, hipFuncAttributeMaxDynamicSharedMemorySize, (int)lds_bytes3);
            attr3[dev].store(true, std::memory_order_relaxed);
        }
        if (ok3m && CHASE_M3_SPLANE) {
            const size_t off = (d.pl.ws_bytes + 255) & ~(size_t)255;
            if (off + d.plane_bytes > ws_bytes) return GEMM_F64_EWORKSPACE;
            double* S = (double*)((char*)ws + off);
            hipLaunchKernelGGL(splane_kernel, dim3((unsigned)((k + 63) / 64), (unsigned)a.gn), dim3(256), 0, st, B, ldb, n, k,
                               d.bn_cols, k / C_::BK, S);
            a.S = S; a.s_nkt = k / C_::BK;
        }
        if (ok3m) {
            if (ragged) hipLaunchKernelGGL((gemm_f64_kernel<CPLX, OPA_C, TAG, true, CAN3M>), dim3(grid), dim3(256), lds_bytes3, st, a);
            else        hipLaunchKernelGGL((gemm_f64_kernel<CPLX, OPA_C, TAG, false, CAN3M>), dim3(grid), dim3(256), lds_bytes3, st, a);
        }
    }
    if (!(CAN3M && ok3m)) {
        if (ragged) hipLaunchKernelGGL((gemm_f64_kernel<CPLX, OPA_C, TAG, true, false, NARROW>), dim3(grid), dim3(256), lds_bytes, st, a);
        else        hipLaunchKernelGGL((gemm_f64_kernel<CPLX, OPA_C, TAG, false, false, NARROW>), dim3(grid), dim3(256), lds_bytes, st, a);
    }
    if (tail > 0) {
        hipLaunchKernelGGL((tail_reduce_kernel<CPLX, C_::BM, C_::BN>), dim3((unsigned)tail * TAIL_PARTS), dim3(256), 0, st, ws,
                           (int)full, sk, a.gn, m, n, C, ldc, a.alpha_re, a.alpha_im, a.beta_re, a.beta_im, a.group_rows, a.bn_cols);
    }
    if (li.exec_flops) *li.exec_flops += 2.0 * (CPLX ? 4.0 : 1.0) * m * (double)n * k * ((CAN3M && ok3m) ? 0.75 : 1.0);
    return (int)hipGetLastError();
}

template <bool CPLX, bool OPA_C>
static int uniform_tile_cols(int m, int n, int k)
{
    using C_ = Cfg<CPLX, OPA_C>;
    static const int mode = [] { const char* e = getenv("CHASE_HIP_UNIFORM_TILES"); return e ? atoi(e) : 1; }();
    if (mode == 0 || (!CPLX && mode != 2)) return 0;
    const int ng = (n + 15) / 16, ntiles = (ng + C_::TN - 1) / C_::TN, g = (ng + ntiles - 1) / ntiles;
    if (g >= C_::TN) return 0;
    const double t_group = 2.0 * (CPLX ? 3.0 : 1.0) * m * (double)k * 16.0 / 73.0e12;
    const double t_pass = (double)m * k * C_::EPT * 8.0 / 6.0e12;
    const int whole = n / C_::BN, rem_groups = (n % C_::BN + 15) / 16;
    const double cost_split = whole * C_::TN * t_group + std::max(rem_groups * t_group, t_pass) + 10e-6;
    const double cost_uniform = std::max((double)ntiles * g * t_group, t_pass);
    if (mode == 2 || cost_uniform < cost_split) return 16 * g;
    return 0;
}

template <bool CPLX, bool OPA_C>
static bool split3m_applies(int m, int n, int k, bool allow3m)
{
    using C_ = Cfg<CPLX, OPA_C>;
    if (!CPLX || !allow3m || gemm3m_enabled() == 0) return false;
    if (m % C_::BM == 0 && k % C_::BK == 0) return false;
    return m >= 8 * C_::BM && k >= 64 * C_::BK && n >= 16;
}

struct Piece { int r0, c0, k0, m, n, k, bn_cols; bool narrow, beta_one, allow3m; };

template <bool CPLX, bool OPA_C, class F>
static int for_each_piece(int m, int n, int k, bool have_ws, bool allow3m, F&& f)
{
    auto cols = [&](int r0, int k0, int mm, int kk, bool beta_one, bool a3) {
        const ColsPlan cp = plan_cols<CPLX, OPA_C>(mm, n, kk, have_ws);
        for (int i = 0; i < cp.npieces; ++i) {
            const ColPiece& pc = cp.piece[i];
            if (const int rc = f(Piece{r0, pc.c0, k0, mm, pc.n, kk, pc.bn_cols, pc.narrow, beta_one, a3})) return rc;
        }
        return 0;
    };
    if (!split3m_applies<CPLX, OPA_C>(m, n, k, allow3m)) return cols(0, 0, m, k, false, allow3m);
    using C_ = Cfg<CPLX, OPA_C>;
    const int m1 = m - m % C_::BM, k1 = k - k % C_::BK;
    int rc = cols(0, 0, m1, k1, false, true);
    if (rc == 0 && k1 < k) rc = cols(0, k1, m1, k - k1, true, false);
    if (rc == 0 && m1 < m) rc = cols(m1, 0, m - m1, k, false, false);
    return rc;
}

template <bool CPLX, bool OPA_C, int TAG>
static int launch_gemm(hipStream_t st, int m, int n, int k, const double* alpha, const double* A, long lda,
                       const double* B, long ldb, const double* beta, double* C, long ldc,
                       double* ws, size_t ws_bytes, int num_cu, bool allow3m, const LaunchInfo& li)
{
    constexpr int EPT = CPLX ? 2 : 1;
    const double one[2] = {1.0, 0.0};
    return for_each_piece<CPLX, OPA_C>(m, n, k, ws != nullptr, allow3m, [&](const Piece& pc) {
        const double* Ap = A + (OPA_C ? ((long)pc.r0 * lda + pc.k0) : ((long)pc.k0 * lda + pc.r0)) * EPT;
        const double* Bp = B + ((long)pc.c0 * ldb + pc.k0) * EPT;
        double* Cp = C + ((long)pc.c0 * ldc + pc.r0) * EPT;
        const double* bp = pc.beta_one ? one : beta;
        if constexpr (!CPLX) {
            if (pc.narrow)
                return launch_gemm_part<CPLX, OPA_C, TAG, true>(st, pc.m, pc.n, pc.k, alpha, Ap, lda, Bp, ldb, bp, Cp, ldc, ws, ws_bytes, num_cu, pc.allow3m, li, pc.bn_cols);
        }
        return launch_gemm_part<CPLX, OPA_C, TAG, false>(st, pc.m, pc.n, pc.k, alpha, Ap, lda, Bp, ldb, bp, Cp, ldc, ws, ws_bytes, num_cu, pc.allow3m, li, pc.bn_cols);
    });
}

template <bool CPLX, bool OPA_C>
static size_t ws_need(int m, int n, int k, int num_cu, int min_rounds)
{
    if (m <= 0 || n <= 0 || k <= 0) return 0;
    const ColsPlan cp = plan_cols<CPLX, OPA_C>(m, n, k, true);
    size_t need = 0;
    for (int i = 0; i < cp.npieces; ++i) {
        const ColPiece& pc = cp.piece[i];
        size_t b;
        if constexpr (!CPLX) {
            b = pc.narrow ? plan_part<CPLX, OPA_C, true>(m, pc.n, k, pc.bn_cols, num_cu, min_rounds).ws_bytes
                          : plan_part<CPLX, OPA_C, false>(m, pc.n, k, pc.bn_cols, num_cu, min_rounds).ws_bytes;
        } else {
            b = plan_part<CPLX, OPA_C, false>(m, pc.n, k, pc.bn_cols, num_cu, min_rounds).ws_bytes;
            if (CHASE_M3_SPLANE && gemm3m_enabled() != 0) b = ((b + 255) & ~(size_t)255) + splane_bytes(pc.n, k, pc.bn_cols);
        }
        need = std::max(need, b);
    }
    return need;
}

size_t gemm_f64_ws_need(bool cplx, char opA, int m, int n, int k, int num_cu, int min_rounds)
{
    const bool opc = (opA == 'C' || opA == 'c' || opA == 'T' || opA == 't');
    if (!cplx) return opc ? ws_need<false, true>(m, n, k, num_cu, min_rounds) : ws_need<false, false>(m, n, k, num_cu, min_rounds);
    auto need = [&](int mm, int kk) {
        return opc ? ws_need<true, true>(mm, n, kk, num_cu, min_rounds) : ws_need<true, false>(mm, n, kk, num_cu, min_rounds);
    };
    size_t r = need(m, k);
    const bool split = opc ? split3m_applies<true, true>(m, n, k, true) : split3m_applies<true, false>(m, n, k, true);
    if (split) {
        const int m1 = m - m % 128, k1 = k - k % 8;
        r = std::max(r, need(m1, k1));
        if (k1 < k) r = std::max(r, need(m1, k - k1));
        if (m1 < m) r = std::max(r, need(m - m1, k));
    }
    return r;
}

static bool tag_allows3m(int tag)
{
    static const bool rr3m = [] { const char* e = getenv("CHASE_HIP_GEMM3M_RR"); return e ? atoi(e) != 0 : true; }();
    return tag == 1 || (tag == 2 && rr3m);
}

int gemm_f64(hipStream_t st, bool cplx, char opA, int m, int n, int k, const double* alpha, const double* A, long lda,
             const double* B, long ldb, const double* beta, double* C, long ldc, double* ws, size_t ws_bytes, int num_cu,
             int tag, int device, double* exec_flops, int min_rounds)
{
    const bool opc = (opA == 'C' || opA == 'c' || opA == 'T' || opA == 't');
    const LaunchInfo li{device, exec_flops, min_rounds};
    const bool allow3m = tag_allows3m(tag);
#define CHASE_GEMM_DISPATCH(CP, OC)                                                                                    \
    (tag == 1 ? launch_gemm<CP, OC, 1>(st, m, n, k, alpha, A, lda, B, ldb, beta, C, ldc, ws, ws_bytes, num_cu, allow3m, li) \
              : launch_gemm<CP, OC, 0>(st, m, n, k, alpha, A, lda, B, ldb, beta, C, ldc, ws, ws_bytes, num_cu, allow3m, li))
    if (!cplx) return opc ? CHASE_GEMM_DISPATCH(false, true) : CHASE_GEMM_DISPATCH(false, false);
    return opc ? CHASE_GEMM_DISPATCH(true, true) : CHASE_GEMM_DISPATCH(true, false);
#undef CHASE_GEMM_DISPATCH
}

template <bool CPLX, bool OPA_C>
static int plan_query(int m, int n, int k, long lda, long ldb, bool aligned16, bool allow3m, int num_cu, int min_rounds,
                      chase_hip_gemm_launch* out, int max_out)
{
    constexpr int EPT = CPLX ? 2 : 1;
    int cnt = 0;
    for_each_piece<CPLX, OPA_C>(m, n, k, true, allow3m, [&](const Piece& pc) {
        if (pc.m <= 0 || pc.n <= 0) return 0;
        const long aoff = OPA_C ? (long)pc.r0 * lda + pc.k0 : (long)pc.k0 * lda + pc.r0, boff = (long)pc.c0 * ldb + pc.k0;
        const bool al = aligned16 && (((aoff | boff) * EPT * 8) % 16 == 0);
        PartDecision d;
        if (!CPLX && pc.narrow) d = decide_part<CPLX, OPA_C, !CPLX>(pc.m, pc.n, pc.k, lda, ldb, al, true, num_cu, pc.allow3m, min_rounds, pc.bn_cols);
        else                    d = decide_part<CPLX, OPA_C, false>(pc.m, pc.n, pc.k, lda, ldb, al, true, num_cu, pc.allow3m, min_rounds, pc.bn_cols);
        if (out && cnt < max_out) {
            chase_hip_gemm_launch& r = out[cnt];
            r.row0 = pc.r0; r.col0 = pc.c0; r.k0 = pc.k0; r.m = pc.m; r.n = pc.n; r.k = pc.k;
            r.beta_one = pc.beta_one; r.bn_cols = d.bn_cols; r.narrow = pc.narrow; r.m3 = d.m3; r.ragged = d.ragged;
            r.glds_ok = d.glds_ok; r.gm = d.gm; r.gn = d.gn; r.full_tiles = d.pl.full; r.tail_tiles = d.pl.tail;
            r.tail_sk = d.pl.sk; r.tail_kchunk = d.kchunk; r.group_rows = d.group_rows; r.forced_split = d.pl.forced;
            r.slab_bytes = d.pl.ws_bytes; r.plane_bytes = d.plane_bytes;
        }
        ++cnt;
        return 0;
    });
    return cnt;
}

int gemm_f64_plan(bool cplx, char opA, int m, int n, int k, long lda, long ldb, bool aligned16, int tag, int num_cu, int min_rounds,
                  chase_hip_gemm_launch* out, int max_out)
{
    const bool opc = (opA == 'C' || opA == 'c' || opA == 'T' || opA == 't');
    if (m <= 0 || n <= 0) return 0;
    const bool a3 = tag_allows3m(tag);
    if (!cplx) return opc ? plan_query<false, true>(m, n, k, lda, ldb, aligned16, a3, num_cu, min_rounds, out, max_out)
                          : plan_query<false, false>(m, n, k, lda, ldb, aligned16, a3, num_cu, min_rounds, out, max_out);
    return opc ? plan_query<true, true>(m, n, k, lda, ldb, aligned16, a3, num_cu, min_rounds, out, max_out)
               : plan_query<true, false>(m, n, k, lda, ldb, aligned16, a3, num_cu, min_rounds, out, max_out);
}

__global__ __launch_bounds__(256, 2) void mfma_f64_peak_kernel(double* out, int iters)
{
    d4_t acc[16];
    #pragma unroll
    for (int i = 0; i < 16; ++i) acc[i] = d4_t{0.0, 0.0, 0.0, 0.0};
    double a = 1.0 + threadIdx.x * 1e-3, b = 1.0 - threadIdx.x * 1e-3;
    for (int it = 0; it < iters; ++it) {
        #pragma unroll
        for (int i = 0; i < 16; ++i) acc[i] = __builtin_amdgcn_mfma_f64_16x16x4f64(a, b, acc[i], 0, 0, 0);
    }
    double s = 0.0;
    #pragma unroll
    for (int i = 0; i < 16; ++i) s += acc[i][0] + acc[i][1] + acc[i][2] + acc[i][3];
    out[(size_t)blockIdx.x * blockDim.x + threadIdx.x] = s;
}

int mfma_f64_peak(hipStream_t st, double* out, int blocks, int iters)
{
    hipLaunchKernelGGL(mfma_f64_peak_kernel, dim3(blocks), dim3(256), 0, st, out, iters);
    return (int)hipGetLastError();
}

}
```

chase_amd/csrc/kernels.h:

```cpp
#pragma once
#include <hip/hip_runtime.h>
#include <stddef.h>

struct chase_hip_gemm_launch;

namespace chase_hip {

int gemm_f64(hipStream_t st, bool cplx, char opA, int m, int n, int k, const double* alpha, const double* A, long lda,
             const double* B, long ldb, const double* beta, double* C, long ldc, double* ws, size_t ws_bytes,
             int num_cu, int tag = 0, int device = 0, double* exec_flops = nullptr, int min_rounds = 0);
constexpr size_t GEMM_WS_CAP = (size_t)640 << 20;
size_t gemm_f64_ws_need(bool cplx, char opA, int m, int n, int k, int num_cu, int min_rounds = 0);
constexpr int GEMM_F64_EWORKSPACE = -77001;
int gemm3m_enabled();
void gemm3m_set(int on);
int gemm_f64_plan(bool cplx, char opA, int m, int n, int k, long lda, long ldb, bool aligned16, int tag, int num_cu, int min_rounds,
                  chase_hip_gemm_launch* out, int max_out);

int mfma_f64_peak(hipStream_t st, double* out, int blocks, int iters);
int stream_copy(hipStream_t st, void* dst, const void* src, size_t bytes);

int shift_diag(hipStream_t st, double* H, long ld, int n, int ept, double shift);
int shift_list(hipStream_t st, double* H, long ld, const int* rows, const int* cols, int cnt, int ept, double shift);
int shift_diag_dev(hipStream_t st, double* A, long ld, int n, int ept, const double* nrmf_dev, double factor);
int abs_trace(hipStream_t st, const double* A, long ld, int n, int ept, double* out_dev);
int copy2d(hipStream_t st, const double* src, long ld_src_d, double* dst, long ld_dst_d, long md, int ncols);
int swap_cols(hipStream_t st, double* a, double* b, long md);
int rows_indexed(hipStream_t st, bool cplx, const double* in, long ld_in, double* out, long ld_out, const int* idx_dev,
                 int np, int ncols, int scatter);
int hash64(hipStream_t st, const double* x, long ld_d, long md, int ncols, unsigned long long* out_dev);
int tri_mask_bc(hipStream_t st, bool cplx, double* H, long ldh, int mloc, int nloc, long mb, int pr, int pi, long nb, int pc,
                int pj, int keep_upper);
int conj_transpose_add(hipStream_t st, bool cplx, const double* P, long ldp, int nr, int nc, const int* rowmap_dev,
                       const int* colmap_dev, double* H, long ldh);
int copy_cols_indexed(hipStream_t st, const double* src, long ld_src_d, double* dst, long ld_dst_d, long md,
                      const int* src_idx_dev, const int* dst_idx_dev, int cnt);
int copy_cols_indexed_range(hipStream_t st, const double* src, long ld_src_d, double* dst, long ld_dst_d, long md,
                            const int* src_idx_dev, int dst0, int cnt);
int resid_norms(hipStream_t st, const double* W, long ldw_d, const double* V, long ldv_d, const double* lambda_dev,
                long md, int ncols, double* out_dev, int do_sqrt);
int sqrt_inplace(hipStream_t st, double* x, int n);
int col_dot(hipStream_t st, bool cplx, const double* X, long ldx_d, const double* Y, long ldy_d, int m, int ncols,
            double* out_dev);
int col_axpy(hipStream_t st, bool cplx, const double* a_dev, int a_is_real, int a_stride, double sgn, const double* X,
             long ldx_d, double* Y, long ldy_d, int m, int ncols);
int col_scal(hipStream_t st, const double* a_dev, int inv, double* X, long ldx_d, long md, int ncols);
int scale_rows(hipStream_t st, double* X, long ldx_d, long row0_d, long md, int ncols, double s);
int scale_rows_bc(hipStream_t st, double* X, long ldx_d, long m, int ncols, int ept, long g0, long nb, int p, int q, double s);
int conj_inplace(hipStream_t st, double* X, long ldx_d, int m, int ncols);
int pack_upper(hipStream_t st, const double* A, long lda, int n, int ept, double* P);
int unpack_upper(hipStream_t st, double* P, int n, int ept, double* A, long lda);
int mirror_upper(hipStream_t st, double* A, long lda, int n, int ept);
int mirror_lower(hipStream_t st, double* A, long lda, int n, int ept, int zero_diag_imag = 1);

int fill_normal(hipStream_t st, bool cplx, double* X, long ldx, int m, int n, long grow0, long gcol0, long gld,
                unsigned long long seed, int mb = 0, int pr = 1, int pi = 0);
int gen_clement(hipStream_t st, bool cplx, double* H, long ldh, int mloc, int nloc, long N, int mb, int pr, int pi,
                long roff, int nb, int pc, int pj, long coff, double scale, double perturb, unsigned long long seed);
int gen_bse(hipStream_t st, bool cplx, double* H, long ldh, int mloc, int nloc, long N, int mb, int pr, int pi, int nb,
            int pc, int pj, double dmin, double dmax, double offdiag, unsigned long long seed);

}
struct chase_hip_ctx;
namespace chase_hip {
int stedc_gpu(chase_hip_ctx* c, int n, const double* d, const double* e, double* w_host, double* Z_dev, long ldz);

int potf2_trtri(hipStream_t st, bool cplx, double* A, long lda, int nb, int joff, double* Tinv, int* info_dev);
int trtri_diag(hipStream_t st, bool cplx, const double* R, long ldr, int n, double* Tinv);

}
```

chase_amd/csrc/vec_kernels.hip:

```cpp
#include <hip/hip_runtime.h>
#include <algorithm>
#include <cstdio>
#include "kernels.h"
#include "ctx.h"
#include "../../include/chase_hip.h"

int chase_hip_ctx::gemm(bool cplx, char opA, int m, int n, int k, const double* alpha, const double* A, long lda,
                        const double* B, long ldb, const double* beta, double* C, long ldc)
{
    if (m <= 0 || n <= 0) return 0;
    if (oplog_on) oplog_add(cplx ? (opA == 'N' ? "gemm_zN" : "gemm_zC") : (opA == 'N' ? "gemm_dN" : "gemm_dC"), m, n, k,
                            phase * 100 + gemm_min_rounds);
    const size_t need = std::max(chase_hip::gemm_f64_ws_need(cplx, opA, m, n, k, num_cu, gemm_min_rounds), (size_t)8 << 20);
    int rc = ensure_ws((need + ((size_t)32 << 20) - 1) & ~(((size_t)32 << 20) - 1));
    if (rc) return rc;
    const int ph = (phase >= 0 && phase <= 3) ? phase : 0;
    int e = chase_hip::gemm_f64(stream, cplx, opA, m, n, k, alpha, A, lda, B, ldb, beta, C, ldc, (double*)ws, ws_bytes,
                                num_cu, phase, device, &flops_exec[ph], gemm_min_rounds);
    if (e == chase_hip::GEMM_F64_EWORKSPACE)
        return chase_hip::set_error(CHASE_HIP_EINVAL, "gemm: split-K workspace smaller than gemm_f64_ws_need for this shape");
    if (e) return chase_hip::hip_fail((hipError_t)e, "gemm launch");
    flops_model[ph] += 2.0 * (cplx ? 4.0 : 1.0) * m * (double)n * k;
    ++gemm_calls[ph];
    return 0;
// ... 206 lines not shown
            const double2* x = (const double2*)(X + (long)j * ldx);
            double2* y = (double2*)(Y + (long)j * ldy);
            for (int i = blockIdx.x * 256 + threadIdx.x; i < m; i += gridDim.x * 256) {
                const double2 xv = x[i]; double2 yv = y[i];
                yv.x += ar * xv.x - ai * xv.y;
                yv.y += ar * xv.y + ai * xv.x;
                y[i] = yv;
            }
        } else {
            const double av = sgn * a[(long)j * a_stride];
            const double* x = X + (long)j * ldx;
            double* y = Y + (long)j * ldy;
            for (int i = blockIdx.x * 256 + threadIdx.x; i < m; i += gridDim.x * 256) y[i] += av * x[i];
        }
    }
}

__global__ __launch_bounds__(256) void col_scal_kernel(const double* __restrict__ a, int inv, double* __restrict__ X,
                                                       long ldx, long md, int ncols)
{
    for (int j = blockIdx.y; j < ncols; j += gridDim.y) {
        const double s = inv ? 1.0 / a[j] : a[j];
        double* x = X + (long)j * ldx;
        for (long i = (long)blockIdx.x * 256 + threadIdx.x; i < md; i += (long)gridDim.x * 256) x[i] *= s;
    }
}

__global__ __launch_bounds__(256) void scale_rows_kernel(double* __restrict__ X, long ldx, long row0_d, long md,
                                                         int ncols, double s)
{
    for (int j = blockIdx.y; j < ncols; j += gridDim.y) {
        double* x = X + (long)j * ldx;
        for (long i = row0_d + (long)blockIdx.x * 256 + threadIdx.x; i < md; i += (long)gridDim.x * 256) x[i] *= s;
    }
}

__global__ __launch_bounds__(256) void scale_rows_bc_kernel(double* __restrict__ X, long ldx_d, long m, int ncols, int ept,
                                                            long g0, long nb, int p, int q, double s)
{
    for (int j = blockIdx.y; j < ncols; j += gridDim.y) {
        double* x = X + (long)j * ldx_d;
        for (long i = (long)blockIdx.x * 256 + threadIdx.x; i < m * ept; i += (long)gridDim.x * 256) {
            const long l = i / ept;
            const long g = ((l / nb) * p + q) * nb + l % nb;
            if (g >= g0) x[i] *= s;
        }
    }
}

__global__ __launch_bounds__(256) void conj_kernel(double* __restrict__ X, long ldx_d, int m, int ncols)
{
    for (int j = blockIdx.y; j < ncols; j += gridDim.y) {
        double* x = X + (long)j * ldx_d;
        for (int i = blockIdx.x * 256 + threadIdx.x; i < m; i += gridDim.x * 256) x[2 * i + 1] = -x[2 * i + 1];
    }
}

__global__ void pack_upper_kernel(const double* __restrict__ A, long lda, int n, int ept, double* __restrict__ P, int unpack,
                                  double* __restrict__ Aout)
{
    const int j = blockIdx.x;
    const long base = (long)j * (j + 1) / 2;
    for (int i = threadIdx.x; i <= j; i += blockDim.x) {
        for (int e = 0; e < ept; ++e) {
            if (!unpack) P[(base + i) * ept + e] = A[((long)j * lda + i) * ept + e];
            else Aout[((long)j * lda + i) * ept + e] = P[(base + i) * ept + e];
        }
    }
}

__global__ void mirror_upper_kernel(double* __restrict__ A, long lda, int n, int ept)
{
    const int j = blockIdx.x;
    for (int i = j + 1 + threadIdx.x; i < n; i += blockDim.x) {
        const double* s = A + ((long)i * lda + j) * ept;
        double* d = A + ((long)j * lda + i) * ept;
        d[0] = s[0];
        if (ept == 2) d[1] = -s[1];
    }
}

__global__ __launch_bounds__(256) void copy_cols_indexed_kernel(const double* __restrict__ src, long lds_, double* __restrict__ dst,
                                                                long ldd, long md, const int* __restrict__ src_idx,
                                                                const int* __restrict__ dst_idx, int cnt)
{
    for (int c = blockIdx.y; c < cnt; c += gridDim.y) {
        const double* s = src + (long)src_idx[c] * lds_;
        double* d = dst + (long)(dst_idx ? dst_idx[c] : c) * ldd;
        for (long i = (long)blockIdx.x * 256 + threadIdx.x; i < md; i += (long)gridDim.x * 256) d[i] = s[i];
    }
}

template <int EPT>
__global__ __launch_bounds__(256) void rows_indexed_kernel(const double* __restrict__ in, long ld_in,
                                                           double* __restrict__ out, long ld_out,
                                                           const int* __restrict__ idx, int np, int ncols, int scatter)
{
    for (int c = blockIdx.y; c < ncols; c += gridDim.y) {
        for (int p = blockIdx.x * 256 + threadIdx.x; p < np; p += gridDim.x * 256) {
            const long r = idx[p];
            const double* s = in + ((long)c * ld_in + (scatter ? p : r)) * EPT;
            double* d = out + ((long)c * ld_out + (scatter ? r : p)) * EPT;
            d[0] = s[0];
            if (EPT == 2) d[1] = s[1];
        }
    }
}

template <int EPT>
__global__ __launch_bounds__(256) void tri_mask_bc_kernel(double* __restrict__ H, long ldh, int mloc, int nloc, long mb, int pr,
                                                          int pi, long nb, int pc, int pj, int keep_upper)
{
    for (int jl = blockIdx.y; jl < nloc; jl += gridDim.y) {
        const long gj = ((long)(jl / nb) * pc + pj) * nb + jl % nb;
        for (int il = blockIdx.x * 256 + threadIdx.x; il < mloc; il += gridDim.x * 256) {
            const long gi = ((long)(il / mb) * pr + pi) * mb + il % mb;
            double* h = H + ((long)jl * ldh + il) * EPT;
            if (gi == gj) { h[0] *= 0.5; if (EPT == 2) h[1] *= 0.5; }
            else if (keep_upper ? (gi > gj) : (gi < gj)) { h[0] = 0.0; if (EPT == 2) h[1] = 0.0; }
        }
    }
}

template <int EPT>
__global__ __launch_bounds__(256) void conj_transpose_add_kernel(const double* __restrict__ P, long ldp, int nr, int nc,
                                                                 const int* __restrict__ rowmap, const int* __restrict__ colmap,
                                                                 double* __restrict__ H, long ldh)
{
    for (int b = blockIdx.y; b < nc; b += gridDim.y) {
        const long hr = colmap[b];
        for (int a = blockIdx.x * 256 + threadIdx.x; a < nr; a += gridDim.x * 256) {
            const double* p = P + ((long)b * ldp + a) * EPT;
            double* h = H + ((long)rowmap[a] * ldh + hr) * EPT;
            h[0] += p[0];
            if (EPT == 2) h[1] -= p[1];
        }
    }
}

__global__ __launch_bounds__(256) void hash64_kernel(const unsigned long long* __restrict__ x, long ld_w, long m_w, int ncols,
                                                     unsigned long long* __restrict__ out)
{
    unsigned long long acc = 0;
    for (int c = blockIdx.y; c < ncols; c += gridDim.y)
        for (long i = (long)blockIdx.x * 256 + threadIdx.x; i < m_w; i += (long)gridDim.x * 256) {
            unsigned long long v = x[(long)c * ld_w + i] ^ (0x9E3779B97F4A7C15ull * (unsigned long long)((long)c * m_w + i + 1));
            v ^= v >> 33; v *= 0xff51afd7ed558ccdull; v ^= v >> 33; v *= 0xc4ceb9fe1a85ec53ull; v ^= v >> 33;
            acc += v;
        }
    for (int off = 32; off > 0; off >>= 1) acc += __shfl_down(acc, off);
    if ((threadIdx.x & 63) == 0) atomicAdd(out, acc);
}

__global__ void mirror_lower_kernel(double* __restrict__ A, long lda, int n, int ept, int zero_diag_imag)
{
    const int j = blockIdx.x;
    if (threadIdx.x == 0 && ept == 2 && zero_diag_imag) A[((long)j * lda + j) * 2 + 1] = 0.0;
    for (int i = j + 1 + threadIdx.x; i < n; i += blockDim.x) {
        const double* s = A + ((long)j * lda + i) * ept;
        double* d = A + ((long)i * lda + j) * ept;
        d[0] = s[0];
        if (ept == 2) d[1] = -s[1];
    }
}

static inline unsigned cdiv(long a, long b) { return (unsigned)((a + b - 1) / b); }
static inline dim3 grid2(long md, int ncols)
{
    unsigned gx = cdiv(md, 256 * 4); if (gx < 1) gx = 1; if (gx > 64) gx = 64;
    unsigned gy = ncols < 1 ? 1 : (ncols > 1024 ? 1024 : ncols);
    return dim3(gx, gy);
}

int shift_diag(hipStream_t st, double* H, long ld, int n, int ept, double shift)
{
    if (n <= 0) return 0;
    hipLaunchKernelGGL(shift_diag_kernel, dim3(cdiv(n, 256)), dim3(256), 0, st, H, ld, n, ept, shift);
    return (int)hipGetLastError();
}
int shift_list(hipStream_t st, double* H, long ld, const int* rows, const int* cols, int cnt, int ept, double shift)
{
    if (cnt <= 0) return 0;
    hipLaunchKernelGGL(shift_list_kernel, dim3(cdiv(cnt, 256)), dim3(256), 0, st, H, ld, rows, cols, cnt, ept, shift);
    return (int)hipGetLastError();
}
int shift_diag_dev(hipStream_t st, double* A, long ld, int n, int ept, const double* nrmf, double factor)
{
    if (n <= 0) return 0;
    hipLaunchKernelGGL(shift_diag_dev_kernel, dim3(cdiv(n, 256)), dim3(256), 0, st, A, ld, n, ept, nrmf, factor);
    return (int)hipGetLastError();
}
int abs_trace(hipStream_t st, const double* A, long ld, int n, int ept, double* out_dev)
{
    hipLaunchKernelGGL(abs_trace_kernel, dim3(1), dim3(256), 0, st, A, ld, n, ept, out_dev);
    return (int)hipGetLastError();
}
int copy2d(hipStream_t st, const double* src, long ld_src_d, double* dst, long ld_dst_d, long md, int ncols)
{
    if (md <= 0 || ncols <= 0) return 0;
    const int vec2 = ((md & 1) == 0) && ((ld_src_d & 1) == 0) && ((ld_dst_d & 1) == 0) &&
                     (((uintptr_t)src & 15) == 0) && (((uintptr_t)dst & 15) == 0);
    hipLaunchKernelGGL(copy2d_kernel, grid2(md, ncols), dim3(256), 0, st, src, ld_src_d, dst, ld_dst_d, md, ncols, vec2);
    return (int)hipGetLastError();
}
int copy_cols_indexed(hipStream_t st, const double* src, long ld_src_d, double* dst, long ld_dst_d, long md,
                      const int* src_idx_dev, const int* dst_idx_dev, int cnt)
{
    if (cnt <= 0 || md <= 0) return 0;
    hipLaunchKernelGGL(copy_cols_indexed_kernel, grid2(md, cnt), dim3(256), 0, st, src, ld_src_d, dst, ld_dst_d, md,
                       src_idx_dev, dst_idx_dev, cnt);
    return (int)hipGetLastError();
}
int copy_cols_indexed_range(hipStream_t st, const double* src, long ld_src_d, double* dst, long ld_dst_d, long md,
                            const int* src_idx_dev, int dst0, int cnt)
{
    if (cnt <= 0 || md <= 0) return 0;
    hipLaunchKernelGGL(copy_cols_indexed_kernel, grid2(md, cnt), dim3(256), 0, st, src, ld_src_d, dst + (long)dst0 * ld_dst_d,
                       ld_dst_d, md, src_idx_dev, (const int*)nullptr, cnt);
    return (int)hipGetLastError();
}
int hash64(hipStream_t st, const double* x, long ld_d, long md, int ncols, unsigned long long* out_dev)
{
    if (md <= 0 || ncols <= 0) return 0;
    hipLaunchKernelGGL(hash64_kernel, grid2(md, ncols), dim3(256), 0, st, (const unsigned long long*)x, ld_d, md, ncols, out_dev);
    return (int)hipGetLastError();
}
int tri_mask_bc(hipStream_t st, bool cplx, double* H, long ldh, int mloc, int nloc, long mb, int pr, int pi, long nb, int pc,
                int pj, int keep_upper)
{
    if (mloc <= 0 || nloc <= 0) return 0;
    const dim3 g = grid2(mloc, nloc);
    if (cplx) hipLaunchKernelGGL(tri_mask_bc_kernel<2>, g, dim3(256), 0, st, H, ldh, mloc, nloc, mb, pr, pi, nb, pc, pj, keep_upper);
    else      hipLaunchKernelGGL(tri_mask_bc_kernel<1>, g, dim3(256), 0, st, H, ldh, mloc, nloc, mb, pr, pi, nb, pc, pj, keep_upper);
    return (int)hipGetLastError();
}
int conj_transpose_add(hipStream_t st, bool cplx, const double* P, long ldp, int nr, int nc, const int* rowmap_dev,
                       const int* colmap_dev, double* H, long ldh)
{
    if (nr <= 0 || nc <= 0) return 0;
    const dim3 g = grid2(nr, nc);
    if (cplx) hipLaunchKernelGGL(conj_transpose_add_kernel<2>, g, dim3(256), 0, st, P, ldp, nr, nc, rowmap_dev, colmap_dev, H, ldh);
    else      hipLaunchKernelGGL(conj_transpose_add_kernel<1>, g, dim3(256), 0, st, P, ldp, nr, nc, rowmap_dev, colmap_dev, H, ldh);
    return (int)hipGetLastError();
}
int rows_indexed(hipStream_t st, bool cplx, const double* in, long ld_in, double* out, long ld_out, const int* idx_dev,
                 int np, int ncols, int scatter)
{
    if (np <= 0 || ncols <= 0) return 0;
    const dim3 g = grid2(np, ncols);
    if (cplx) hipLaunchKernelGGL(rows_indexed_kernel<2>, g, dim3(256), 0, st, in, ld_in, out, ld_out, idx_dev, np, ncols, scatter);
    else      hipLaunchKernelGGL(rows_indexed_kernel<1>, g, dim3(256), 0, st, in, ld_in, out, ld_out, idx_dev, np, ncols, scatter);
    return (int)hipGetLastError();
}
int swap_cols(hipStream_t st, double* a, double* b, long md)
{
    if (md <= 0 || a == b) return 0;
    unsigned g = cdiv(md, 256 * 4); if (g > 256) g = 256;
    hipLaunchKernelGGL(swap_kernel, dim3(g), dim3(256), 0, st, a, b, md);
    return (int)hipGetLastError();
}
int resid_norms(hipStream_t st, const double* W, long ldw_d, const double* V, long ldv_d, const double* lambda_dev,
                long md, int ncols, double* out_dev, int do_sqrt)
{
    if (ncols <= 0) return 0;
    hipLaunchKernelGGL(resid_norms_kernel, dim3(ncols), dim3(256), 0, st, W, ldw_d, V, ldv_d, lambda_dev, md, out_dev,
                       do_sqrt);
    return (int)hipGetLastError();
}
int sqrt_inplace(hipStream_t st, double* x, int n)
{
    if (n <= 0) return 0;
    hipLaunchKernelGGL(sqrt_inplace_kernel, dim3(cdiv(n, 256)), dim3(256), 0, st, x, n);
    return (int)hipGetLastError();
}
int col_dot(hipStream_t st, bool cplx, const double* X, long ldx_d, const double* Y, long ldy_d, int m, int ncols,
            double* out_dev)
{
    if (ncols <= 0) return 0;
    if (cplx) hipLaunchKernelGGL(col_dot_kernel<true>, dim3(ncols), dim3(256), 0, st, X, ldx_d, Y, ldy_d, m, out_dev);
    else      hipLaunchKernelGGL(col_dot_kernel<false>, dim3(ncols), dim3(256), 0, st, X, ldx_d, Y, ldy_d, m, out_dev);
    return (int)hipGetLastError();
}
int col_axpy(hipStream_t st, bool cplx, const double* a_dev, int a_is_real, int a_stride, double sgn, const double* X,
             long ldx_d, double* Y, long ldy_d, int m, int ncols)
{
    if (ncols <= 0 || m <= 0) return 0;
    const dim3 g = grid2(m, ncols);
    if (cplx) hipLaunchKernelGGL(col_axpy_kernel<true>, g, dim3(256), 0, st, a_dev, a_is_real, a_stride, sgn, X, ldx_d, Y, ldy_d, m, ncols);
    else      hipLaunchKernelGGL(col_axpy_kernel<false>, g, dim3(256), 0, st, a_dev, a_is_real, a_stride, sgn, X, ldx_d, Y, ldy_d, m, ncols);
    return (int)hipGetLastError();
}
int col_scal(hipStream_t st, const double* a_dev, int inv, double* X, long ldx_d, long md, int ncols)
{
    if (ncols <= 0 || md <= 0) return 0;
    hipLaunchKernelGGL(col_scal_kernel, grid2(md, ncols), dim3(256), 0, st, a_dev, inv, X, ldx_d, md, ncols);
    return (int)hipGetLastError();
}
int scale_rows(hipStream_t st, double* X, long ldx_d, long row0_d, long md, int ncols, double s)
{
    if (ncols <= 0 || md <= row0_d) return 0;
    hipLaunchKernelGGL(scale_rows_kernel, grid2(md - row0_d, ncols), dim3(256), 0, st, X, ldx_d, row0_d, md, ncols, s);
    return (int)hipGetLastError();
}
int scale_rows_bc(hipStream_t st, double* X, long ldx_d, long m, int ncols, int ept, long g0, long nb, int p, int q, double s)
{
    if (ncols <= 0 || m <= 0) return 0;
    hipLaunchKernelGGL(scale_rows_bc_kernel, grid2(m * ept, ncols), dim3(256), 0, st, X, ldx_d, m, ncols, ept, g0, nb, p, q, s);
    return (int)hipGetLastError();
}
int conj_inplace(hipStream_t st, double* X, long ldx_d, int m, int ncols)
{
    if (ncols <= 0 || m <= 0) return 0;
    hipLaunchKernelGGL(conj_kernel, grid2(m, ncols), dim3(256), 0, st, X, ldx_d, m, ncols);
    return (int)hipGetLastError();
}
int pack_upper(hipStream_t st, const double* A, long lda, int n, int ept, double* P)
{
    if (n <= 0) return 0;
    hipLaunchKernelGGL(pack_upper_kernel, dim3(n), dim3(128), 0, st, A, lda, n, ept, P, 0, (double*)nullptr);
    return (int)hipGetLastError();
}
int unpack_upper(hipStream_t st, double* P, int n, int ept, double* A, long lda)
{
    if (n <= 0) return 0;
    hipLaunchKernelGGL(pack_upper_kernel, dim3(n), dim3(128), 0, st, (const double*)nullptr, lda, n, ept, P, 1, A);
    return (int)hipGetLastError();
}
int mirror_lower(hipStream_t st, double* A, long lda, int n, int ept, int zero_diag_imag)
{
    if (n <= 0) return 0;
    hipLaunchKernelGGL(mirror_lower_kernel, dim3(n), dim3(128), 0, st, A, lda, n, ept, zero_diag_imag);
    return (int)hipGetLastError();
}
int mirror_upper(hipStream_t st, double* A, long lda, int n, int ept)
{
    if (n <= 1) return 0;
    hipLaunchKernelGGL(mirror_upper_kernel, dim3(n), dim3(128), 0, st, A, lda, n, ept);
    return (int)hipGetLastError();
}

}
```

chase_amd/host/chase_hip_impl.hpp:

```cpp
#pragma once
#include <cmath>
#include <complex>
#include <cstdlib>
#include <cstring>
#include <limits>
#include <random>
#include <stdexcept>
#include <string>
#include <vector>
#include "../../include/chase_hip.h"
#include "impl_extras.hpp"
#include "interface.hpp"
#include "output_override.hpp"
#include "roctx.hpp"

namespace chase_amd {

template <class T> struct is_cplx : std::false_type {};
template <class R> struct is_cplx<std::complex<R>> : std::true_type {};

struct HipStatusError : std::runtime_error {
    int code;
    HipStatusError(int c, const std::string& where)
        : std::runtime_error(where + " failed (" + std::to_string(c) + "): " + chase_hip_last_error()), code(c) {}
};
inline void hip_ok(int rc, const char* where) { if (rc < 0) throw HipStatusError(rc, where); }

template <class T, class BaseT = ChaseBase<T>, class ConfigT = ChaseConfig<T>>
class ChaseHip : public WithOutput<BaseT>, public HipImplExtras {
public:
    using R = Base<T>;
    static constexpr int CP = is_cplx<T>::value ? 1 : 0;

    ChaseHip(chase_hip_ctx* ctx, std::size_t N, std::size_t nev, std::size_t nex, T* H, std::size_t ldh, T* V1,
             std::size_t ldv, R* ritzv, bool h_on_device = false)
        : ctx_(ctx), N_(N), nev_(nev), nex_(nex), nevex_(nev + nex), H_(H), ldh_(ldh), V1_(V1), ldv_(ldv),
          ritzv_(ritzv), h_on_device_(h_on_device), config_(N, nev, nex), resid_(nev + nex, 0), perm_(nev + nex)
    {
        if (!ctx) throw std::invalid_argument("ChaseHip: null context");
        if (N == 0 || nevex_ == 0 || nevex_ > N) throw std::invalid_argument("ChaseHip: need 0 < nev+nex <= N");
        if (ldh < N || ldv < N) throw std::invalid_argument("ChaseHip: leading dimension smaller than N");
        for (std::size_t i = 0; i < nevex_; ++i) perm_[i] = (int)i;
        if (h_on_device_) { dH_ = H; ldd_h_ = ldh; }
        else { alloc((void**)&dH_, N_ * N_ * sizeof(T)); ldd_h_ = N_; own_h_ = true; }
        alloc((void**)&dV1_, N_ * nevex_ * sizeof(T));
        alloc((void**)&dV2_, N_ * nevex_ * sizeof(T));
        alloc((void**)&dA_, nevex_ * nevex_ * sizeof(T));
        alloc((void**)&dScal_, 4096);
    }
    ~ChaseHip() override
    {
        for (void* p : owned_) chase_hip_free(ctx_, p);
    }

    std::size_t GetN() const override { return N_; }
    std::size_t GetNev() override { return nev_; }
    std::size_t GetNex() override { return nex_; }
    std::size_t GetLanczosIter() override { return lanczosIter_; }
    std::size_t GetNumLanczos() override { return numLanczos_; }
    std::size_t GetRitzvBlockSize() const override { return nevex_; }
    R* GetRitzv() override { return ritzv_; }
    R* GetResid() override { return resid_.data(); }
    ConfigT& GetConfig() override { return config_; }
    int get_nprocs() override { return 1; }
    int get_rank() override { return 0; }
    bool isSym() override { return true; }
    bool isPseudoHerm() override { return false; }
    bool checkPseudoHermicityEasy() override { return false; }
    void Sort(R*, R*, R*) override {}
    void ApplyKconjugate(std::size_t) override {}
    void HEMM_H2(std::size_t, T, T, T, std::size_t, std::size_t = 0) override
    {
        throw std::logic_error("ChaseHip: HEMM_H2 belongs to the pseudo-Hermitian Impl");
    }
    void set_early_locked_residuals(std::vector<R> r) override { early_ = std::move(r); }
    const std::vector<R>& early_locked_residuals() const { return early_; }
    std::size_t locked() const override { return locked_; }
    void* device_V1() override { flush_swaps(); return dV1_; }
    std::size_t local_rows() const override { return N_; }
    T* device_V2() { return dV2_; }
    T* device_H() { return dH_; }
    double filter_ms() const override { return filter_ms_; }

    bool checkSymmetryEasy() override
    {
        CHASE_PHASE(ctx_, "checkSymmetryEasy");
        if (!h_resident_) upload_H();
        std::vector<T> v(N_);
        std::mt19937 gen(1337);
        std::normal_distribution<> d;
        for (auto& x : v) x = rnd(d, gen);
        T* u = dV2_;
        hip_ok(chase_hip_upload_matrix(ctx_, CP, (int)N_, 1, v.data(), (long)N_, u, (long)N_), "upload");
        gemm('N', N_, 1, N_, T(1), dH_, ldd_h_, u, N_, T(0), u + N_, N_);
        gemm('C', N_, 1, N_, T(1), dH_, ldd_h_, u, N_, T(0), u + 2 * N_, N_);
        std::vector<T> a(N_), b(N_);
        hip_ok(chase_hip_download_matrix(ctx_, CP, (int)N_, 1, u + N_, (long)N_, a.data(), (long)N_), "download");
        hip_ok(chase_hip_download_matrix(ctx_, CP, (int)N_, 1, u + 2 * N_, (long)N_, b.data(), (long)N_), "download");
        double diff = 0, nrm = 0;
        for (std::size_t i = 0; i < N_; ++i) { diff += std::norm(a[i] - b[i]); nrm += std::norm(a[i]); }
        return std::sqrt(diff) <= 1e-10 * std::max(1.0, std::sqrt(nrm));
    }

    void symOrHermMatrix(char uplo) override
    {
        if (h_on_device_) {
            hip_ok(chase_hip_complete_hermitian(ctx_, CP, uplo, (int)N_, dH_, (long)ldd_h_), "complete_hermitian");
            hv_valid_ = false;
            return;
        }
        const bool up = (uplo == 'U' || uplo == 'u');
        for (std::size_t j = 0; j < N_; ++j)
            for (std::size_t i = 0; i < j; ++i) {
                if (up) H_[j + i * ldh_] = conj_(H_[i + j * ldh_]);
                else    H_[i + j * ldh_] = conj_(H_[j + i * ldh_]);
            }
        h_resident_ = false;
    }

    void Start() override { locked_ = 0; }

    void initVecs(bool random) override
    {
        CHASE_PHASE(ctx_, "initVecs");
        hv_valid_ = false;
        if (random && device_rng_) {
            hip_ok(chase_hip_fill_normal(ctx_, CP, (int)N_, (int)nevex_, dV1_, (long)N_, 0, 0, (long)N_, 1337ull), "fill_normal");
        } else {
            if (random) {
                std::mt19937 gen(1337.0);
                std::normal_distribution<> d;
                for (std::size_t j = 0; j < nevex_; ++j)
                    for (std::size_t i = 0; i < N_; ++i) V1_[i + j * ldv_] = rnd(d, gen);
            }
            hip_ok(chase_hip_upload_matrix(ctx_, CP, (int)N_, (int)nevex_, V1_, (long)ldv_, dV1_, (long)N_), "upload V");
        }
        hip_ok(chase_hip_lacpy(ctx_, CP, (int)N_, (int)nevex_, dV1_, (long)N_, dV2_, (long)N_), "lacpy");
        reset_perm();
        upload_H();
    }

    void ReinitColumns(std::size_t fixednev, std::size_t const* col_indices, std::size_t n_indices) override
    {
        CHASE_PHASE(ctx_, "ReinitColumns");
        if (n_indices == 0) return;
        flush_swaps();
        hv_valid_ = false;
        std::mt19937 gen(4242);
        std::normal_distribution<> d;
        std::vector<T> h(N_);
        for (std::size_t c = 0; c < n_indices; ++c) {
            const std::size_t j = fixednev + col_indices[c];
            if (j >= nevex_) throw std::invalid_argument("ReinitColumns: column out of range");
            for (auto& x : h) x = rnd(d, gen);
            hip_ok(chase_hip_upload_matrix(ctx_, CP, (int)N_, 1, h.data(), (long)N_, dV1_ + j * N_, (long)N_), "upload column");
            hip_ok(chase_hip_lacpy(ctx_, CP, (int)N_, 1, dV1_ + j * N_, (long)N_, dV2_ + j * N_, (long)N_), "lacpy");
        }
    }

    void End() override
    {
        CHASE_PHASE(ctx_, "End");
        flush_swaps();
        hip_ok(chase_hip_download_matrix(ctx_, CP, (int)N_, (int)nevex_, dV1_, (long)N_, V1_, (long)ldv_), "download V");
    }

    void FilterPhaseStart() override
    {
        roctx_push("chase:Filter");
        flush_swaps();
        chase_hip_ctx_set_phase(ctx_, 1);
        hip_ok(chase_hip_timer_start(ctx_), "timer");
    }
    void FilterPhaseEnd() override
    {
        float ms = 0;
        hip_ok(chase_hip_timer_stop(ctx_, &ms), "timer");
        chase_hip_ctx_set_phase(ctx_, 0);
        filter_ms_ += ms;
        roctx_pop(ctx_);
    }
    void set_device_rng(bool f) override { device_rng_ = f; }
    void reset_counters() override { filter_ms_ = 0; hemm_calls_ = 0; hemm_reused_vecs_ = 0; }
    std::size_t hemm_calls() const override { return hemm_calls_; }
    std::size_t hemm_reused_vecs() const override { return hemm_reused_vecs_; }

    void Shift(T c, bool = false) override
    {
        hv_shift_ += std::real(c);
        hip_ok(chase_hip_shift_diag(ctx_, CP, (int)N_, dH_, (long)ldd_h_, std::real(c)), "shift_diag");
    }

    void HEMM(std::size_t block, T alpha, T beta, std::size_t offset_left, std::size_t offset_right = 0) override
    {
        flush_swaps();
        const std::size_t ncols = (offset_right < block) ? block - offset_right : 0;
        if (ncols != 0) {
            const std::size_t c0 = locked_ + offset_left;
            if (hv_valid_ && beta == T(0) && std::imag(alpha) == 0.0 && c0 >= hv_locked_ &&
                c0 + ncols <= hv_locked_ + hv_block_) {
                T* v1 = dV1_ + c0 * N_;
                T* v2 = dV2_ + c0 * N_;
                hip_ok(chase_hip_lacpy(ctx_, CP, (int)N_, (int)ncols, dHV_ + c0 * N_, (long)N_, v2, (long)N_), "lacpy");
                if (hv_shift_ != 0.0) {
                    const double sc[2] = {hv_shift_, 0.0};
                    hip_ok(chase_hip_memcpy_h2d(ctx_, dScal_, sc, sizeof sc), "h2d");
                    hip_ok(chase_hip_col_axpy(ctx_, CP, (int)N_, (int)ncols, (const double*)dScal_, 0, 0, 1.0, v1, (long)N_, v2,
                                              (long)N_), "axpy shift");
                }
                hip_ok(chase_hip_scale_rows(ctx_, CP, (int)N_, (int)ncols, v2, (long)N_, 0, std::real(alpha)), "scale");
                hemm_reused_vecs_ += ncols;
            } else {
                gemm('N', N_, ncols, N_, alpha, dH_, ldd_h_, dV1_ + c0 * N_, N_, beta, dV2_ + c0 * N_, N_);
                ++hemm_calls_;
            }
        }
        hv_valid_ = false;
        std::swap(dV1_, dV2_);
    }

    void QR(std::size_t, R cond) override
    {
        CHASE_PHASE(ctx_, "QR");
        flush_swaps(); hv_valid_ = false;
        hip_ok(chase_hip_lacpy(ctx_, CP, (int)N_, (int)locked_, dV1_, (long)N_, dV2_, (long)N_), "lacpy");
        int disable = config_.DoCholQR() ? 0 : 1;
        if (const char* s = std::getenv("CHASE_DISABLE_CHOLQR")) disable = std::atoi(s);
        R thld_hi = 1e8, thld_lo = 2e1;
        if (const char* s = std::getenv("CHASE_CHOLQR1_THLD")) thld_lo = std::atof(s);
        last_qr_variant_ = 0;
        if (disable == 1 && cond != (R)1.0) {
            householder();
        } else {
            const int variant = (cond > thld_hi) ? 3 : (cond < thld_lo ? 1 : 2);
            last_qr_variant_ = variant;
            const int info = chase_hip_cholqr(ctx_, CP, (int)N_, (int)nevex_, dV1_, (long)N_, dA_, (long)nevex_,
                                              variant, (long)N_);
            hip_ok(info, "cholqr");
            if (info != 0) householder();
        }
        hip_ok(chase_hip_lacpy(ctx_, CP, (int)N_, (int)locked_, dV2_, (long)N_, dV1_, (long)N_), "lacpy");
    }
    int last_qr_variant() const override { return last_qr_variant_; }

    void RR(R* ritzv, std::size_t block) override
    {
        CHASE_PHASE(ctx_, "RR");
        flush_swaps();
        T* Q = dV1_ + locked_ * N_;
        T* W = dV2_ + locked_ * N_;
        chase_hip_ctx_set_phase(ctx_, 2);
        gemm('C', N_, block, N_, T(1), dH_, ldd_h_, Q, N_, T(0), W, N_);
        chase_hip_ctx_set_phase(ctx_, 0);
        hip_ok(chase_hip_herkx(ctx_, CP, (int)block, (int)N_, W, (long)N_, Q, (long)N_, dA_, (long)block, 1), "herkx");
        hip_ok(chase_hip_heevd(ctx_, CP, (int)block, dA_, (long)block, ritzv), "heevd");
        hv_valid_ = false;
        if (resd_reuse_) {
            if (!dHV_) alloc((void**)&dHV_, N_ * nevex_ * sizeof(T));
            gemm('N', N_, block, block, T(1), W, N_, dA_, block, T(0), dHV_ + locked_ * N_, N_);
            hv_valid_ = true; hv_locked_ = locked_; hv_block_ = block; hv_shift_ = 0.0;
        }
        gemm('N', N_, block, block, T(1), Q, N_, dA_, block, T(0), W, N_);
        std::swap(dV1_, dV2_);
    }

    void Resd(R* ritzv, R* resd, std::size_t) override
    {
        CHASE_PHASE(ctx_, "Resd");
        flush_swaps();
        const std::size_t sub = nevex_ - locked_;
        T* V = dV1_ + locked_ * N_;
        T* W = dV2_ + locked_ * N_;
        const bool reused = hv_valid_ && hv_shift_ == 0.0 && hv_locked_ == locked_ && hv_block_ == sub;
        if (reused) W = dHV_ + locked_ * N_;
        else {
            chase_hip_ctx_set_phase(ctx_, 2);
            gemm('N', N_, sub, N_, T(1), dH_, ldd_h_, V, N_, T(0), W, N_);
            chase_hip_ctx_set_phase(ctx_, 0);
        }
        hip_ok(chase_hip_resid_norms(ctx_, CP, (int)N_, (int)sub, W, (long)N_, V, (long)N_, ritzv, resd, 0), "resid");
        if (reused || CP) recheck_borderline(ritzv, resd, sub, reused);
        if (resd != resid_.data() + locked_) std::memcpy(resid_.data() + locked_, resd, sub * sizeof(R));
    }

    void recheck_borderline(const R* ritzv, R* resd, std::size_t sub, bool reused)
    {
        static const bool on = [] { const char* e = std::getenv("CHASE_HIP_RESD_RECHECK"); return e ? std::atoi(e) != 0 : true; }();
        if (!on) return;
        const R tol = (R)config_.GetTol();
        const R window = std::min(std::max((R)1e-3 * tol, (R)4 * std::numeric_limits<R>::epsilon() * norm_h_), (R)0.5 * tol);
        std::vector<std::size_t> idx;
        if (forced_recheck_ >= 0) {
            for (std::size_t j = 0; j < std::min<std::size_t>((std::size_t)forced_recheck_, sub); ++j) idx.push_back(j);
        } else {
            for (std::size_t j = 0; j < sub; ++j)
                if (std::abs(resd[j] - tol) <= window) idx.push_back(j);
        }
        if (idx.empty()) return;
        const std::size_t k = idx.size();
        (void)reused;
        T* Vs = dV2_ + locked_ * N_;
        if (2 * k > sub) {
            chase_hip_ctx_set_phase(ctx_, 3);
            gemm('N', N_, sub, N_, T(1), dH_, ldd_h_, dV1_ + locked_ * N_, N_, T(0), Vs, N_);
            chase_hip_ctx_set_phase(ctx_, 0);
            hip_ok(chase_hip_resid_norms(ctx_, CP, (int)N_, (int)sub, Vs, (long)N_, dV1_ + locked_ * N_, (long)N_, ritzv, resd, 0), "resid");
            resd_rechecked_ += sub;
            return;
        }
        T* Ws = Vs + k * N_;
        std::vector<R> lam(k), out(k);
        for (std::size_t i = 0; i < k; ++i) {
            lam[i] = ritzv[idx[i]];
            hip_ok(chase_hip_lacpy(ctx_, CP, (int)N_, 1, dV1_ + (locked_ + idx[i]) * N_, (long)N_, Vs + i * N_, (long)N_), "lacpy");
        }
        chase_hip_ctx_set_phase(ctx_, 3);
        gemm('N', N_, k, N_, T(1), dH_, ldd_h_, Vs, N_, T(0), Ws, N_);
        chase_hip_ctx_set_phase(ctx_, 0);
        hip_ok(chase_hip_resid_norms(ctx_, CP, (int)N_, (int)k, Ws, (long)N_, Vs, (long)N_, lam.data(), out.data(), 0), "resid");
        for (std::size_t i = 0; i < k; ++i) resd[idx[i]] = out[i];
        resd_rechecked_ += k;
    }
    void set_forced_recheck(long k) override { forced_recheck_ = k; }
    std::size_t resd_rechecked() const override { return resd_rechecked_; }

    void recompute_residuals(std::size_t ncols, const double* lambda, double* out) override
    {
        CHASE_PHASE(ctx_, "recompute_residuals");
        if (ncols > nevex_) throw std::invalid_argument("recompute_residuals: more columns than the Impl holds");
        flush_swaps();
        hv_valid_ = false;
        chase_hip_ctx_set_phase(ctx_, 3);
        gemm('N', N_, ncols, N_, T(1), dH_, ldd_h_, dV1_, N_, T(0), dV2_, N_);
        chase_hip_ctx_set_phase(ctx_, 0);
        hip_ok(chase_hip_resid_norms(ctx_, CP, (int)N_, (int)ncols, dV2_, (long)N_, dV1_, (long)N_, lambda, out, 0), "resid");
    }

    void Swap(std::size_t i, std::size_t j) override
    {
        if (i == j) return;
        std::swap(perm_[i], perm_[j]);
        perm_dirty_ = true;
    }
    void Lock(std::size_t new_converged) override { locked_ += new_converged; }

    void Lanczos(std::size_t m, R* upperb) override
    {
        CHASE_PHASE(ctx_, "Lanczos");
        lanczosIter_ = m; numLanczos_ = 1;
        std::vector<R> theta(m);
        lanczos_core(m, 1, false, upperb, theta.data(), nullptr, nullptr);
    }
    void Lanczos(std::size_t M, std::size_t numvec, R* upperb, R* ritzv, R* Tau, R* ritzV) override
    {
        CHASE_PHASE(ctx_, "Lanczos");
        lanczosIter_ = M; numLanczos_ = numvec;
        lanczos_core(M, numvec, true, upperb, ritzv, Tau, ritzV);
    }
    void LanczosDos(std::size_t idx, std::size_t m, T* ritzVc) override
    {
        CHASE_PHASE(ctx_, "LanczosDos");
        hv_valid_ = false;
        flush_swaps();
        hip_ok(chase_hip_upload_matrix(ctx_, CP, (int)m, (int)idx, ritzVc, (long)m, dA_, (long)m), "upload ritzV");
        gemm('N', N_, idx, m, T(1), dV1_, N_, dA_, m, T(0), dV2_, N_);
        hip_ok(chase_hip_lacpy(ctx_, CP, (int)N_, (int)m, dV2_, (long)N_, dV1_, (long)N_), "lacpy");
    }

private:
    static T rnd(std::normal_distribution<>& d, std::mt19937& g)
    {
        if constexpr (is_cplx<T>::value) { const double re = d(g); const double im = d(g); return T(re, im); }
        else return T(d(g));
    }
    static T conj_(T x) { if constexpr (is_cplx<T>::value) return std::conj(x); else return x; }

    void alloc(void** p, std::size_t bytes)
    {
        int rc = chase_hip_malloc(ctx_, p, bytes);
        if (rc) throw HipStatusError(rc, "chase_hip_malloc");
        owned_.push_back(*p);
    }
    void upload_H()
    {
        if (!h_on_device_)
            hip_ok(chase_hip_upload_matrix(ctx_, CP, (int)N_, (int)N_, H_, (long)ldh_, dH_, (long)ldd_h_), "upload H");
        h_resident_ = true;
    }
    void gemm(char op, std::size_t m, std::size_t n, std::size_t k, T alpha, const T* A, std::size_t lda, const T* B,
              std::size_t ldb, T beta, T* C, std::size_t ldc)
    {
        int rc;
        if constexpr (is_cplx<T>::value) {
            const double a[2] = {alpha.real(), alpha.imag()}, b[2] = {beta.real(), beta.imag()};
            rc = chase_hip_gemm_z(ctx_, op, (int)m, (int)n, (int)k, a, A, (long)lda, B, (long)ldb, b, C, (long)ldc);
        } else {
            rc = chase_hip_gemm_d(ctx_, op, (int)m, (int)n, (int)k, alpha, A, (long)lda, B, (long)ldb, beta, C, (long)ldc);
        }
        hip_ok(rc, "gemm");
    }
    void householder()
    {
        last_qr_variant_ = 0;
        hip_ok(chase_hip_houseqr(ctx_, CP, (int)N_, (int)nevex_, dV1_, (long)N_), "houseqr");
    }
    void reset_perm()
    {
        for (std::size_t i = 0; i < nevex_; ++i) perm_[i] = (int)i;
        perm_dirty_ = false;
    }
    void flush_swaps()
    {
        if (!perm_dirty_) return;
        std::vector<int> src, dst;
        for (std::size_t j = 0; j < nevex_; ++j)
            if (perm_[j] != (int)j) { src.push_back(perm_[j]); dst.push_back((int)j); }
        if (!src.empty()) {
            hip_ok(chase_hip_permute_cols(ctx_, CP, (int)N_, dV1_, (long)N_, dV2_, (long)N_, src.data(), dst.data(),
                                          (int)src.size()), "permute_cols");
            if (hv_valid_)
                hip_ok(chase_hip_permute_cols(ctx_, CP, (int)N_, dHV_, (long)N_, dV2_, (long)N_, src.data(), dst.data(),
                                              (int)src.size()), "permute_cols");
        }
        reset_perm();
    }

    void lanczos_core(std::size_t M, std::size_t nv, bool store, R* upperb, R* theta, R* Tau, R* ritzV)
    {
        flush_swaps(); hv_valid_ = false;
        if (!h_resident_) upload_H();
        constexpr int E = CP ? 2 : 1;
        T *v0, *v1, *v2;
        double *d_alpha, *d_beta, *d_nrm0;
        void* blk = nullptr;
        const std::size_t vec_bytes = 3 * N_ * nv * sizeof(T);
        const std::size_t sc_bytes = (M * nv * E + M * nv + nv) * sizeof(double);
        int rc = chase_hip_malloc(ctx_, &blk, vec_bytes + sc_bytes);
        if (rc) throw HipStatusError(rc, "lanczos workspace");
        v0 = (T*)blk; v1 = v0 + N_ * nv; v2 = v1 + N_ * nv;
        d_alpha = (double*)(v2 + N_ * nv); d_beta = d_alpha + M * nv * E; d_nrm0 = d_beta + M * nv;
        const int n = (int)N_, nvi = (int)nv;
        try {
            hip_ok(chase_hip_memset(ctx_, blk, 0, vec_bytes + sc_bytes), "memset");
            hip_ok(chase_hip_lacpy(ctx_, CP, n, nvi, dV1_, (long)N_, v1, (long)N_), "lacpy");
            hip_ok(chase_hip_col_nrm2(ctx_, CP, n, nvi, v1, (long)N_, d_nrm0), "nrm2");
            hip_ok(chase_hip_col_scal(ctx_, CP, n, nvi, d_nrm0, 1, v1, (long)N_), "scal");
            for (std::size_t k = 0; k < M; ++k) {
                if (store)
                    hip_ok(chase_hip_lacpy(ctx_, CP, n, 1, v1 + (nv - 1) * N_, (long)N_, dV1_ + k * N_, (long)N_), "lacpy");
                gemm('C', N_, nv, N_, T(1), dH_, ldd_h_, v1, N_, T(0), v2, N_);
                double* ak = d_alpha + k * nv * E;
                hip_ok(chase_hip_col_dot(ctx_, CP, n, nvi, v1, (long)N_, v2, (long)N_, ak), "dot");
                hip_ok(chase_hip_col_axpy(ctx_, CP, n, nvi, ak, 0, 1, -1.0, v1, (long)N_, v2, (long)N_), "axpy");
                if (k > 0)
                    hip_ok(chase_hip_col_axpy(ctx_, CP, n, nvi, d_beta + (k - 1) * nv, 1, 1, -1.0, v0, (long)N_, v2,
                                              (long)N_), "axpy");
                hip_ok(chase_hip_col_nrm2(ctx_, CP, n, nvi, v2, (long)N_, d_beta + k * nv), "nrm2");
                if (k == M - 1) break;
                hip_ok(chase_hip_col_scal(ctx_, CP, n, nvi, d_beta + k * nv, 1, v2, (long)N_), "scal");
                T* t = v0; v0 = v1; v1 = v2; v2 = t;
            }
            if (store) hip_ok(chase_hip_lacpy(ctx_, CP, n, nvi, v1, (long)N_, dV1_, (long)N_), "lacpy");
            std::vector<double> h_alpha(M * nv * E), h_beta(M * nv);
            hip_ok(chase_hip_memcpy_d2h(ctx_, h_alpha.data(), d_alpha, h_alpha.size() * sizeof(double)), "d2h");
            hip_ok(chase_hip_memcpy_d2h(ctx_, h_beta.data(), d_beta, h_beta.size() * sizeof(double)), "d2h");
            chase_hip_free(ctx_, blk);
            blk = nullptr;

            std::vector<double> d(M), e(M), w(M), Z(M * M);
            R ub = 0;
            for (std::size_t i = 0; i < nv; ++i) {
                for (std::size_t k = 0; k < M; ++k) {
                    d[k] = h_alpha[(k * nv + i) * E];
                    e[k] = (k + 1 < M) ? h_beta[k * nv + i] : 0.0;
                }
                hip_ok(chase_hip_stemr_host((int)M, d.data(), e.data(), w.data(), Z.data(), (int)M), "stemr");
                for (std::size_t k = 0; k < M; ++k) {
                    theta[k + i * M] = w[k];
                    if (Tau) Tau[k + i * M] = std::abs(Z[k * M]) * std::abs(Z[k * M]);
                }
                if (ritzV) std::memcpy(ritzV, Z.data(), M * M * sizeof(double));
                const R cand = std::max(std::abs(w[0]), std::abs(w[M - 1])) + std::abs(h_beta[(M - 1) * nv + i]);
                ub = (i == 0) ? cand : std::max(ub, cand);
            }
            *upperb = ub;
            norm_h_ = std::abs(ub);
        } catch (...) {
            if (blk) chase_hip_free(ctx_, blk);
            throw;
        }
    }

    chase_hip_ctx* ctx_;
    std::size_t N_, nev_, nex_, nevex_;
    T* H_; std::size_t ldh_;
    T* V1_; std::size_t ldv_;
    R* ritzv_;
    bool h_on_device_, own_h_ = false, h_resident_ = false;
    ConfigT config_;
    std::vector<R> resid_, early_;
    std::vector<int> perm_;
    bool perm_dirty_ = false;
    std::size_t locked_ = 0, lanczosIter_ = 0, numLanczos_ = 0;
    T *dH_ = nullptr, *dV1_ = nullptr, *dV2_ = nullptr, *dA_ = nullptr, *dHV_ = nullptr;
    std::size_t ldd_h_ = 0;
    bool hv_valid_ = false, resd_reuse_ = std::getenv("CHASE_HIP_RESD_REUSE") ? std::atoi(std::getenv("CHASE_HIP_RESD_REUSE")) != 0 : true;
    std::size_t hv_locked_ = 0, hv_block_ = 0, hemm_reused_vecs_ = 0;
    double hv_shift_ = 0.0;
    void* dScal_ = nullptr;
    std::vector<void*> owned_;
    double filter_ms_ = 0;
    std::size_t hemm_calls_ = 0, resd_rechecked_ = 0;
    long forced_recheck_ = -1;
    R norm_h_ = 0;
    bool device_rng_ = false;
    int last_qr_variant_ = 0;
};

}
```

chase_amd/host/impl_extras.hpp:

```cpp
#pragma once
#include <cstddef>

namespace chase_amd {

struct HipImplExtras {
    virtual ~HipImplExtras() = default;
    virtual std::size_t locked() const = 0;
    virtual int last_qr_variant() const = 0;
    virtual double filter_ms() const = 0;
    virtual std::size_t hemm_calls() const = 0;
    virtual std::size_t hemm_reused_vecs() const { return 0; }
    virtual std::size_t resd_rechecked() const { return 0; }
    virtual void set_device_rng(bool) = 0;
    virtual void reset_counters() = 0;
    virtual void* device_V1() = 0;
    virtual std::size_t local_rows() const = 0;
    virtual void recompute_residuals(std::size_t ncols, const double* lambda, double* out) = 0;
    virtual void set_forced_recheck(long) {}
    virtual void set_forced_qr(int) {}
    virtual std::size_t forced_qr_retries() const { return 0; }
    virtual void set_replay_tolerant(bool) {}
    virtual std::size_t replay_tolerated() const { return 0; }
};

}
```

chase_amd/host/solver_capi.cpp:

```cpp
#include <cstdio>
#include <cstring>
#include <memory>
#include <string>
#include "../../include/chase_hip.h"
#include "../../include/chase_hip_solver.h"
#include "../../include/chase_hip_grid.h"
#include "algorithm.hpp"
#include "chase_hip_impl.hpp"
#include "pchase_hip_impl.hpp"
#include "chase_hip_pseudo_impl.hpp"
#include "pchase_hip_pseudo_impl.hpp"
#include "tape.hpp"

namespace chase_hip { int set_error(int code, const char* what); }
using namespace chase_amd;

using zc = std::complex<double>;
struct chase_hip_solver {
    int cplx = 0, pseudo = 0;
    std::unique_ptr<ChaseBase<double>> d;
    std::unique_ptr<ChaseBase<zc>> z;
    HipImplExtras* ex = nullptr;
    pChaseHip<double>* pd = nullptr;
    pChaseHip<zc>* pz = nullptr;
// ... 18 lines not shown
        return chase_hip::set_error(CHASE_HIP_EINVAL, (std::string(where) + ": " + e.what()).c_str());
    } catch (const std::exception& e) {
        return chase_hip::set_error(CHASE_HIP_EINVAL, (std::string(where) + ": " + e.what()).c_str());
    }
}
#define DISPATCH(s, expr)                                                                                              \
    do {                                                                                                               \
        if ((s)->cplx) { auto& k = *(s)->z; expr; } else { auto& k = *(s)->d; expr; }                                  \
    } while (0)
}

extern "C" {

int chase_hip_solver_create(chase_hip_solver** out, chase_hip_ctx* ctx, int cplx, size_t N, size_t nev, size_t nex,
                            void* H, size_t ldh, void* V, size_t ldv, double* ritzv, int h_on_device)
{
    if (!out || !ctx || !H || !V || !ritzv) return chase_hip::set_error(CHASE_HIP_EINVAL, "solver_create: NULL argument");
    auto s = std::make_unique<chase_hip_solver>();
    s->cplx = cplx ? 1 : 0;
    chase_hip_host_lapack_warmup();
    int rc = guarded("solver_create", [&] {
        if (cplx) {
            auto* p = new ChaseHip<zc>(ctx, N, nev, nex, (zc*)H, ldh, (zc*)V, ldv, ritzv, h_on_device != 0);
            s->z.reset(p); s->ex = p;
        } else {
            auto* p = new ChaseHip<double>(ctx, N, nev, nex, (double*)H, ldh, (double*)V, ldv, ritzv, h_on_device != 0);
            s->d.reset(p); s->ex = p;
        }
    });
    if (rc) return rc;
    *out = s.release();
    return 0;
}

int chase_hip_solver_create_pseudo(chase_hip_solver** out, chase_hip_ctx* ctx, int cplx, size_t N, size_t nev, size_t nex,
                                   void* H, size_t ldh, void* V, size_t ldv, double* ritzv, int h_on_device)
{
    if (!out || !ctx || !H || !V || !ritzv) return chase_hip::set_error(CHASE_HIP_EINVAL, "solver_create_pseudo: NULL argument");
    auto s = std::make_unique<chase_hip_solver>();
    s->cplx = cplx ? 1 : 0;
    s->pseudo = 1;
    chase_hip_host_lapack_warmup();
    int rc = guarded("solver_create_pseudo", [&] {
        if (cplx) {
            auto* p = new ChaseHipPseudo<zc>(ctx, N, nev, nex, (zc*)H, ldh, (zc*)V, ldv, ritzv, h_on_device != 0);
            s->z.reset(p); s->ex = p;
        } else {
            auto* p = new ChaseHipPseudo<double>(ctx, N, nev, nex, (double*)H, ldh, (double*)V, ldv, ritzv, h_on_device != 0);
            s->d.reset(p); s->ex = p;
        }
    });
    if (rc) return rc;
    *out = s.release();
    return 0;
}

int chase_hip_psolver_create(chase_hip_solver** out, chase_hip_ctx* ctx, chase_hip_grid* grid, int cplx, size_t N,
                             size_t nev, size_t nex, size_t mb, size_t nb, void* H_loc_dev, size_t ldh, double* ritzv)
{
    if (!out || !ctx || !grid || !H_loc_dev || !ritzv)
        return chase_hip::set_error(CHASE_HIP_EINVAL, "psolver_create: NULL argument");
    auto s = std::make_unique<chase_hip_solver>();
    s->cplx = cplx ? 1 : 0;
    chase_hip_host_lapack_warmup();
    int rc = guarded("psolver_create", [&] {
        if (cplx) {
            auto* p = new pChaseHip<zc>(ctx, grid, N, nev, nex, mb, nb, (zc*)H_loc_dev, ldh, ritzv);
            s->z.reset(p); s->ex = p; s->pz = p;
        } else {
            auto* p = new pChaseHip<double>(ctx, grid, N, nev, nex, mb, nb, (double*)H_loc_dev, ldh, ritzv);
            s->d.reset(p); s->ex = p; s->pd = p;
        }
    });
    if (rc) return rc;
    *out = s.release();
    return 0;
}

int chase_hip_psolver_create_pseudo(chase_hip_solver** out, chase_hip_ctx* ctx, chase_hip_grid* grid, int cplx, size_t N,
                                    size_t nev, size_t nex, size_t mb, size_t nb, void* H_loc_dev, size_t ldh,
                                    double* ritzv)
{
    if (!out || !ctx || !grid || !H_loc_dev || !ritzv)
        return chase_hip::set_error(CHASE_HIP_EINVAL, "psolver_create_pseudo: NULL argument");
    auto s = std::make_unique<chase_hip_solver>();
    s->cplx = cplx ? 1 : 0;
    s->pseudo = 1;
    chase_hip_host_lapack_warmup();
    int rc = guarded("psolver_create_pseudo", [&] {
        if (cplx) {
            auto* p = new pChaseHipPseudo<zc>(ctx, grid, N, nev, nex, mb, nb, (zc*)H_loc_dev, ldh, ritzv);
            s->z.reset(p); s->ex = p; s->pz = p;
        } else {
            auto* p = new pChaseHipPseudo<double>(ctx, grid, N, nev, nex, mb, nb, (double*)H_loc_dev, ldh, ritzv);
            s->d.reset(p); s->ex = p; s->pd = p;
        }
    });
    if (rc) return rc;
    *out = s.release();
    return 0;
}

int chase_hip_psolver_local_shape(chase_hip_solver* s, size_t* m_loc, size_t* n_loc)
{
    if (!s || (!s->pd && !s->pz)) return chase_hip::set_error(CHASE_HIP_EINVAL, "not a distributed solver");
    if (m_loc) *m_loc = s->ex->local_rows();
    if (n_loc) *n_loc = s->pz ? s->pz->local_cols_h() : s->pd->local_cols_h();
    return 0;
}
int chase_hip_psolver_upload_v(chase_hip_solver* s, const void* host, size_t ldv)
{
    if (!s || (!s->pd && !s->pz)) return chase_hip::set_error(CHASE_HIP_EINVAL, "not a distributed solver");
    return guarded("upload_v", [&] { if (s->pz) s->pz->upload_local_V((const zc*)host, ldv); else s->pd->upload_local_V((const double*)host, ldv); });
}
int chase_hip_psolver_download_v(chase_hip_solver* s, void* host, size_t ldv)
{
    if (!s || (!s->pd && !s->pz)) return chase_hip::set_error(CHASE_HIP_EINVAL, "not a distributed solver");
    return guarded("download_v", [&] { if (s->pz) s->pz->download_local_V((zc*)host, ldv); else s->pd->download_local_V((double*)host, ldv); });
}
int chase_hip_psolver_set_pipeline(chase_hip_solver* s, int on)
{
    if (!s || (!s->pd && !s->pz)) return chase_hip::set_error(CHASE_HIP_EINVAL, "not a distributed solver");
    if (s->pz) s->pz->set_pipeline(on != 0); else s->pd->set_pipeline(on != 0);
    return 0;
}

int chase_hip_solver_destroy(chase_hip_solver* s)
{
    delete s;
    return 0;
}

int chase_hip_solver_set(chase_hip_solver* s, const char* key, double v)
{
    if (!s || !key) return chase_hip::set_error(CHASE_HIP_EINVAL, "solver_set: NULL argument");
    const std::string name(key);
    int rc = 0;
    const int grc = guarded("solver_set", [&] { DISPATCH(s, {
        auto& c = k.GetConfig();
        if (name == "tol") c.SetTol(v);
        else if (name == "deg") c.SetDeg((size_t)v);
        else if (name == "maxdeg") c.SetMaxDeg((size_t)v);
        else if (name == "degextra") c.SetDegExtra((size_t)v);
        else if (name == "maxiter") c.SetMaxIter((size_t)v);
        else if (name == "lanczositer") c.SetLanczosIter((size_t)v);
        else if (name == "numlanczos") c.SetNumLanczos((size_t)v);
        else if (name == "opt") c.SetOpt(v != 0);
        else if (name == "approx") c.SetApprox(v != 0);
        else if (name == "cholqr") c.SetCholQR(v != 0);
        else if (name == "decayingrate") c.SetDecayingRate((float)v);
        else if (name == "clusteraware") c.SetClusterAwareDegrees(v != 0);
        else if (name == "upperbscale") c.SetUpperbScaleRate((float)v);
        else if (name == "device_rng") s->ex->set_device_rng(v != 0);
        else if (name == "panel_cols" && (s->pd || s->pz)) { if (s->pz) s->pz->set_panel_cols((size_t)v); else s->pd->set_panel_cols((size_t)v); }
        else if (name == "panel_rounds" && (s->pd || s->pz)) { if (s->pz) s->pz->set_panel_rounds((int)v); else s->pd->set_panel_rounds((int)v); }
        else if (name == "pipeline" && (s->pd || s->pz)) { if (s->pz) s->pz->set_pipeline(v != 0); else s->pd->set_pipeline(v != 0); }
        else if (name == "reset_counters") s->ex->reset_counters();
        else rc = chase_hip::set_error(CHASE_HIP_EINVAL, "solver_set: unknown key");
    }); });
    return grc ? grc : rc;
}

int chase_hip_solver_get(chase_hip_solver* s, const char* key, double* out)
{
    if (!s || !key || !out) return chase_hip::set_error(CHASE_HIP_EINVAL, "solver_get: NULL argument");
    const std::string name(key);
    int rc = 0;
    DISPATCH(s, {
        auto& c = k.GetConfig();
        if (name == "tol") *out = c.GetTol();
        else if (name == "deg") *out = (double)c.GetDeg();
        else if (name == "maxdeg") *out = (double)c.GetMaxDeg();
        else if (name == "degextra") *out = (double)c.GetDegExtra();
        else if (name == "maxiter") *out = (double)c.GetMaxIter();
        else if (name == "lanczositer") *out = (double)c.GetLanczosIter();
        else if (name == "numlanczos") *out = (double)c.GetNumLanczos();
        else if (name == "opt") *out = c.DoOptimization();
        else if (name == "approx") *out = c.UseApprox();
        else if (name == "cholqr") *out = c.DoCholQR();
        else if (name == "decayingrate") *out = c.GetDecayingRate();
        else if (name == "clusteraware") *out = c.UseClusterAwareDegrees();
        else if (name == "upperbscale") *out = c.GetUpperbScaleRate();
        else if (name == "locked") *out = (double)s->ex->locked();
        else if (name == "qr_ortho_check" && (s->pd || s->pz)) *out = s->pz ? s->pz->last_ortho_check() : s->pd->last_ortho_check();
        else if (name == "panel_cols" && (s->pd || s->pz)) *out = (double)(s->pz ? s->pz->panel_cols() : s->pd->panel_cols());
        else if (name == "panel_rounds" && (s->pd || s->pz)) *out = (double)(s->pz ? s->pz->panel_rounds() : s->pd->panel_rounds());
        else if (name == "pipeline" && (s->pd || s->pz)) *out = (double)(s->pz ? s->pz->pipeline() : s->pd->pipeline());
        else if (name == "rr_disagreements" && (s->pd || s->pz)) *out = (double)(s->pz ? s->pz->rr_disagreements() : s->pd->rr_disagreements());
        else if (name == "qr_variant") *out = (double)s->ex->last_qr_variant();
        else if (name == "filter_ms") *out = s->ex->filter_ms();
        else if (name == "hemm_calls") *out = (double)s->ex->hemm_calls();
        else if (name == "hemm_reused_vecs") *out = (double)s->ex->hemm_reused_vecs();
        else if (name == "resd_rechecked") *out = (double)s->ex->resd_rechecked();
        else if (name == "tape_qr_mismatches") *out = (double)s->tape.qr_variant_mismatches;
        else if (name == "tape_qr_retries") *out = (double)s->ex->forced_qr_retries();
        else if (name == "tape_tolerated") *out = (double)s->ex->replay_tolerated();
        else if (name == "tape_position") *out = (double)s->tape.pos;
        else if (name == "tape_size") *out = (double)s->tape.data.size();
        else if (name == "iterations") *out = (double)s->stats.iterations;
        else if (name == "filtered_vecs") *out = (double)s->stats.filtered_vecs;
        else rc = chase_hip::set_error(CHASE_HIP_EINVAL, "solver_get: unknown key");
    });
    return rc;
}

int chase_hip_solver_set_iteration_hook(chase_hip_solver* s, chase_hip_iteration_fn fn, void* user)
{
    if (!s) return chase_hip::set_error(CHASE_HIP_EINVAL, "set_iteration_hook: NULL solver");
    s->trace.iter_hook = fn;
    s->trace.iter_user = user;
    return 0;
}

int chase_hip_solver_solve(chase_hip_solver* s, int record_trace)
{
    if (!s) return chase_hip::set_error(CHASE_HIP_EINVAL, "solver_solve: NULL solver");
    s->stats = SolveStats();
    s->trace.lines.clear();
    s->trace.enabled = record_trace != 0;
    return guarded("solve", [&] {
        if (s->pseudo && s->tape_mode) {
            if (s->cplx) {
                TapeKernel<zc> tk(s->z.get(), s->ex, &s->tape, (TapeKernel<zc>::Mode)s->tape_mode);
                Algorithm<zc, ChaseBase<zc>>::solve_pseudo(&tk, &s->stats, &s->trace);
            } else {
                TapeKernel<double> tk(s->d.get(), s->ex, &s->tape, (TapeKernel<double>::Mode)s->tape_mode);
                Algorithm<double, ChaseBase<double>>::solve_pseudo(&tk, &s->stats, &s->trace);
            }
        } else if (s->pseudo) {
            if (s->cplx) Algorithm<zc, ChaseBase<zc>>::solve_pseudo(s->z.get(), &s->stats, &s->trace);
            else Algorithm<double, ChaseBase<double>>::solve_pseudo(s->d.get(), &s->stats, &s->trace);
        } else if (s->tape_mode) {
            if (s->cplx) {
                TapeKernel<zc> tk(s->z.get(), s->ex, &s->tape, (TapeKernel<zc>::Mode)s->tape_mode);
                Algorithm<zc, ChaseBase<zc>>::solve(&tk, &s->stats, &s->trace);
            } else {
                TapeKernel<double> tk(s->d.get(), s->ex, &s->tape, (TapeKernel<double>::Mode)s->tape_mode);
                Algorithm<double, ChaseBase<double>>::solve(&tk, &s->stats, &s->trace);
            }
        } else {
            if (s->cplx) Algorithm<zc, ChaseBase<zc>>::solve(s->z.get(), &s->stats, &s->trace);
            else Algorithm<double, ChaseBase<double>>::solve(s->d.get(), &s->stats, &s->trace);
        }
    });
}

int chase_hip_solver_tape_mode(chase_hip_solver* s, int mode)
{
    if (!s || mode < 0 || mode > 2) return chase_hip::set_error(CHASE_HIP_EINVAL, "tape_mode: 0, 1 or 2");
    s->tape_mode = mode;
    return 0;
}
int chase_hip_solver_tape_data(chase_hip_solver* s, const double** data, size_t* count)
{
    if (!s || !data || !count) return chase_hip::set_error(CHASE_HIP_EINVAL, "tape_data: NULL argument");
    *data = s->tape.data.data();
    *count = s->tape.data.size();
    return 0;
}
int chase_hip_solver_tape_load(chase_hip_solver* s, const double* data, size_t count)
{
    if (!s || (!data && count)) return chase_hip::set_error(CHASE_HIP_EINVAL, "tape_load: NULL argument");
    s->tape.data.assign(data, data + count);
    s->tape.rewind();
    return 0;
}

int chase_hip_solver_lanczos_for_h2(chase_hip_solver* s, int numvec, int m, double* upperb, size_t* idx)
{
    if (!s || !upperb || !idx) return chase_hip::set_error(CHASE_HIP_EINVAL, "lanczos_for_h2: NULL argument");
    if (!s->pseudo) return chase_hip::set_error(CHASE_HIP_EINVAL, "lanczos_for_h2: not a pseudo-Hermitian solver");
    return guarded("lanczos_for_H2", [&] {
        if (s->cplx) {
            auto* k = s->z.get();
            *idx = Algorithm<zc, ChaseBase<zc>>::lanczos_for_H2(k, (int)k->GetN(), numvec, m, (int)(k->GetNev() + k->GetNex()),
                                                                 upperb, k->GetRitzv());
        } else {
            auto* k = s->d.get();
            *idx = Algorithm<double, ChaseBase<double>>::lanczos_for_H2(k, (int)k->GetN(), numvec, m,
                                                                        (int)(k->GetNev() + k->GetNex()), upperb, k->GetRitzv());
        }
    });
}

int chase_hip_solver_stats(chase_hip_solver* s, chase_hip_stats* o)
{
    if (!s || !o) return chase_hip::set_error(CHASE_HIP_EINVAL, "solver_stats: NULL argument");
    const SolveStats& t = s->stats;
    o->iterations = t.iterations; o->filtered_vecs = t.filtered_vecs; o->lanczos_vecs = t.lanczos_vecs;
    o->locked = t.locked;
    o->t_all = t.t_all; o->t_init = t.t_init; o->t_lanczos = t.t_lanczos; o->t_filter = t.t_filter; o->t_qr = t.t_qr;
    o->t_rr = t.t_rr; o->t_resid = t.t_resid;
    o->lowerb = t.lowerb; o->upperb = t.upperb; o->lambda = t.lambda;
    double fm = 0;
    chase_hip_solver_get(s, "filter_ms", &fm);
    o->filter_ms_device = fm;
    return 0;
}

const double* chase_hip_solver_resid(chase_hip_solver* s)
{
    if (!s) return nullptr;
    const double* r = nullptr;
    DISPATCH(s, r = k.GetResid());
    return r;
}

const char* chase_hip_solver_trace(chase_hip_solver* s)
{
    if (!s) return "";
    s->trace_text.clear();
    for (const auto& l : s->trace.lines) { s->trace_text += l; s->trace_text += '\n'; }
    return s->trace_text.c_str();
}

int chase_hip_op_start(chase_hip_solver* s) { return guarded("Start", [&] { DISPATCH(s, k.Start()); }); }
int chase_hip_op_end(chase_hip_solver* s) { return guarded("End", [&] { DISPATCH(s, k.End()); }); }
int chase_hip_op_reinit_columns(chase_hip_solver* s, size_t fixednev, const size_t* col_indices, size_t n_indices)
{
    if (!s || (!col_indices && n_indices)) return chase_hip::set_error(CHASE_HIP_EINVAL, "ReinitColumns: NULL argument");
    return guarded("ReinitColumns", [&] { DISPATCH(s, k.ReinitColumns(fixednev, col_indices, n_indices)); });
}
int chase_hip_op_initvecs(chase_hip_solver* s, int random)
{
    return guarded("initVecs", [&] { DISPATCH(s, k.initVecs(random != 0)); });
}
int chase_hip_op_shift(chase_hip_solver* s, double c, int isunshift)
{
    return guarded("Shift", [&] {
        if (s->cplx) s->z->Shift(std::complex<double>(c, 0), isunshift != 0);
        else s->d->Shift(c, isunshift != 0);
    });
}
int chase_hip_op_hemm(chase_hip_solver* s, size_t block, const double* alpha, const double* beta, size_t offset_left,
                      size_t offset_right)
{
    return guarded("HEMM", [&] {
        if (s->cplx)
            s->z->HEMM(block, std::complex<double>(alpha[0], alpha[1]), std::complex<double>(beta[0], beta[1]),
                       offset_left, offset_right);
        else s->d->HEMM(block, alpha[0], beta[0], offset_left, offset_right);
    });
}
int chase_hip_op_hemm_h2(chase_hip_solver* s, size_t block, const double* alpha, const double* beta, const double* gamma,
                         size_t offset_left, size_t offset_right)
{
// ... 75 lines not shown
```

include/chase_hip.h:

```cpp
#ifndef CHASE_HIP_H
#define CHASE_HIP_H

#include <stddef.h>

#ifdef __cplusplus
extern "C" {
#endif

#define CHASE_HIP_OK 0
#define CHASE_HIP_EINVAL (-1001)
#define CHASE_HIP_ENODEV (-1002)
#define CHASE_HIP_ENOMEM (-1003)
#define CHASE_HIP_ENOTCONV (-1004)
#define CHASE_HIP_ECOMM (-1005)
#define CHASE_HIP_ELAPACK (-1006)
#define CHASE_HIP_EIO (-1007)

typedef struct chase_hip_ctx chase_hip_ctx;

int chase_hip_ctx_create(chase_hip_ctx** out, int device, void* stream);
int chase_hip_ctx_destroy(chase_hip_ctx* ctx);
int chase_hip_ctx_sync(chase_hip_ctx* ctx);
void* chase_hip_ctx_stream(chase_hip_ctx* ctx);
int chase_hip_ctx_oplog(chase_hip_ctx* ctx, int on);
int chase_hip_ctx_oplog_mute(chase_hip_ctx* ctx, int delta);
const char* chase_hip_ctx_oplog_text(chase_hip_ctx* ctx);
const char* chase_hip_last_error(void);
int chase_hip_device_info(chase_hip_ctx* ctx, int* num_cu, int* clock_khz, size_t* hbm_bytes, char* name,
                          int name_len);
int chase_hip_device_bus_id(chase_hip_ctx* ctx, char* out, int len);
const char* chase_hip_version(void);
int chase_hip_device_count(void);

int chase_hip_malloc(chase_hip_ctx* ctx, void** dev, size_t bytes);
int chase_hip_free(chase_hip_ctx* ctx, void* dev);
int chase_hip_memcpy_h2d(chase_hip_ctx* ctx, void* dev, const void* host, size_t bytes);
int chase_hip_memcpy_d2h(chase_hip_ctx* ctx, void* host, const void* dev, size_t bytes);
int chase_hip_memcpy_d2d(chase_hip_ctx* ctx, void* dst, const void* src, size_t bytes);
int chase_hip_memset(chase_hip_ctx* ctx, void* dev, int value, size_t bytes);
int chase_hip_timer_start(chase_hip_ctx* ctx);
int chase_hip_timer_stop(chase_hip_ctx* ctx, float* ms);

int chase_hip_gemm_d(chase_hip_ctx* ctx, char opA, int m, int n, int k, double alpha, const double* A, long lda,
                     const double* B, long ldb, double beta, double* C, long ldc);
int chase_hip_gemm_z(chase_hip_ctx* ctx, char opA, int m, int n, int k, const double alpha[2], const void* A,
                     long lda, const void* B, long ldb, const double beta[2], void* C, long ldc);

size_t chase_hip_gemm_workspace_bytes(int cplx, char opA, int m, int n, int k, int num_cu, int min_rounds);
typedef struct chase_hip_gemm_launch {
    int row0, col0, k0;
    int m, n, k;
    int beta_one;
    int bn_cols;
    int narrow;
    int m3;
    int ragged;
    int glds_ok;
    int gm, gn;
    long full_tiles;
    long tail_tiles;
    int tail_sk, tail_kchunk;
    int group_rows;
    int forced_split;
    size_t slab_bytes;
    size_t plane_bytes;
} chase_hip_gemm_launch;
int chase_hip_gemm_plan(int cplx, char opA, int m, int n, int k, long lda, long ldb, int aligned16, int phase, int num_cu,
                        int min_rounds, chase_hip_gemm_launch* out, int max_out);
int chase_hip_gemm3m_enabled(void);
int chase_hip_set_gemm3m(int on);
int chase_hip_ctx_gemm_counters(chase_hip_ctx* ctx, int phase, double* flops_model, double* flops_executed,
                                unsigned long long* calls, int reset);
int chase_hip_mfma_f64_peak(chase_hip_ctx* ctx, double* tflops);
int chase_hip_hbm_copy_peak(chase_hip_ctx* ctx, size_t bytes, double* gbps);

int chase_hip_ctx_set_phase(chase_hip_ctx* ctx, int phase);
int chase_hip_ctx_set_gemm_min_rounds(chase_hip_ctx* ctx, int rounds);

int chase_hip_fill_normal(chase_hip_ctx* ctx, int cplx, int m, int n, void* X, long ldx, long grow0, long gcol0,
                          long gld, unsigned long long seed);
int chase_hip_fill_normal_bc(chase_hip_ctx* ctx, int cplx, int m, int n, void* X, long ldx, long gld, int mb, int pr,
                             int pi, unsigned long long seed);
int chase_hip_rows_indexed(chase_hip_ctx* ctx, int cplx, const void* in, long ld_in, void* out, long ld_out,
                           const int* idx_dev, int np, int ncols, int scatter);
int chase_hip_hash64(chase_hip_ctx* ctx, int cplx, int m, int n, const void* A, long lda, unsigned long long* out_host);
int chase_hip_cols_indexed(chase_hip_ctx* ctx, int cplx, int m, const void* in, long ld_in, void* out, long ld_out,
                           const int* idx_dev, int ncols);
int chase_hip_complete_hermitian(chase_hip_ctx* ctx, int cplx, char uplo, int n, void* A, long lda);
int chase_hip_tri_mask_bc(chase_hip_ctx* ctx, int cplx, char uplo, int mloc, int nloc, void* H, long ldh, long mb, int pr, int pi,
                          long nb, int pc, int pj);
int chase_hip_conj_transpose_add(chase_hip_ctx* ctx, int cplx, int nr, int nc, const void* P, long ldp, const int* rowmap_dev,
                                 const int* colmap_dev, void* H, long ldh);
int chase_hip_gen_clement(chase_hip_ctx* ctx, int cplx, void* H, long ldh, int mloc, int nloc, long N, int mb, int pr,
                          int pi, long roff, int nb, int pc, int pj, long coff, double scale, double perturb,
                          unsigned long long seed);
int chase_hip_gen_bse(chase_hip_ctx* ctx, int cplx, void* H, long ldh, int mloc, int nloc, long N, int mb, int pr, int pi,
                      int nb, int pc, int pj, double dmin, double dmax, double offdiag, unsigned long long seed);
int chase_hip_load_matrix_shard(chase_hip_ctx* ctx, const char* path, int cplx, long N, int mloc, int nloc, int mb,
                                int pr, int pi, int nb, int pc, int pj, void* dev, long ldd);
int chase_hip_save_matrix(chase_hip_ctx* ctx, const char* path, int cplx, int m, int n, const void* dev, long ldd);
int chase_hip_save_matrix_shard(chase_hip_ctx* ctx, const char* path, int cplx, long N, int mloc, int nloc, int mb,
                                int pr, int pi, int nb, int pc, int pj, const void* dev, long ldd);

int chase_hip_set_lapack_lib(const char* path);
const char* chase_hip_lapack_provider(void);
int chase_hip_set_host_threads(int n);
int chase_hip_host_lapack_warmup(void);

int chase_hip_shift_diag(chase_hip_ctx* ctx, int cplx, int n, void* H, long ldh, double shift);
int chase_hip_shift_list(chase_hip_ctx* ctx, int cplx, void* H, long ldh, const int* rows_dev, const int* cols_dev,
                         int cnt, double shift);
int chase_hip_lacpy(chase_hip_ctx* ctx, int cplx, int m, int n, const void* A, long lda, void* B, long ldb);
int chase_hip_swap_cols(chase_hip_ctx* ctx, int cplx, int m, void* V, long ldv, long i, long j);
int chase_hip_permute_cols(chase_hip_ctx* ctx, int cplx, int m, void* V, long ldv, void* scratch, long lds,
                           const int* src_host, const int* dst_host, int cnt);
int chase_hip_upload_matrix(chase_hip_ctx* ctx, int cplx, int m, int n, const void* host, long ldh, void* dev, long ldd);
int chase_hip_download_matrix(chase_hip_ctx* ctx, int cplx, int m, int n, const void* dev, long ldd, void* host,
                              long ldh);
int chase_hip_scale_rows(chase_hip_ctx* ctx, int cplx, int m, int n, void* X, long ldx, int row0, double s);
int chase_hip_scale_rows_bc(chase_hip_ctx* ctx, int cplx, int m, int n, void* X, long ldx, long g0, long nb, int p, int q,
                            double s);
int chase_hip_conj(chase_hip_ctx* ctx, int m, int n, void* X, long ldx);
int chase_hip_resid_norms(chase_hip_ctx* ctx, int cplx, int m, int n, const void* W, long ldw, const void* V, long ldv,
                          const double* lambda_host, double* resid_host, int squared);

int chase_hip_resid_norms_dev(chase_hip_ctx* ctx, int cplx, int m, int n, const void* W, long ldw, const void* V, long ldv,
                              const double* lambda_host, double* out_dev, int squared);

int chase_hip_herk(chase_hip_ctx* ctx, int cplx, int n, int k, const void* V, long ldv, void* A, long lda);
int chase_hip_herkx(chase_hip_ctx* ctx, int cplx, int n, int k, const void* A, long lda, const void* B, long ldb, void* C,
                    long ldc, int mirror);
int chase_hip_abs_trace(chase_hip_ctx* ctx, int cplx, int n, const void* A, long lda, double* out_host);
int chase_hip_potrf_upper(chase_hip_ctx* ctx, int cplx, int n, void* A, long lda);
int chase_hip_trsm_right_upper(chase_hip_ctx* ctx, int cplx, int m, int n, const void* R, long ldr, void* V, long ldv);
int chase_hip_cholqr(chase_hip_ctx* ctx, int cplx, int m, int n, void* V, long ldv, void* A, long lda, int variant,
                     long m_global);
int chase_hip_houseqr(chase_hip_ctx* ctx, int cplx, int m, int n, void* V, long ldv);

int chase_hip_heevd(chase_hip_ctx* ctx, int cplx, int n, void* A, long lda, double* w_host);
int chase_hip_heevd_gpu(chase_hip_ctx* ctx, int cplx, int n, void* A, long lda, double* w_host);
int chase_hip_pseudo_rr_small(chase_hip_ctx* ctx, int cplx, int n, void* A_dev, void* M_dev, double* ritzv_host);
int chase_hip_set_identity(chase_hip_ctx* ctx, int cplx, int n, void* A, long lda);
int chase_hip_heevd_host(int cplx, int n, void* A_host, long lda, double* w_host);
int chase_hip_stemr_host(int n, double* d, double* e, double* w, double* Z, int ldz);
int chase_hip_stedc(chase_hip_ctx* ctx, int n, const double* d_host, const double* e_host, double* w_host, double* Z_dev,
                    long ldz);

int chase_hip_col_dot(chase_hip_ctx* ctx, int cplx, int m, int n, const void* X, long ldx, const void* Y, long ldy,
                      double* out_dev);
int chase_hip_col_nrm2(chase_hip_ctx* ctx, int cplx, int m, int n, const void* X, long ldx, double* out_dev);
int chase_hip_col_sumsq(chase_hip_ctx* ctx, int cplx, int m, int n, const void* X, long ldx, double* out_dev);
int chase_hip_sqrt_inplace(chase_hip_ctx* ctx, double* x_dev, int n);
int chase_hip_col_axpy(chase_hip_ctx* ctx, int cplx, int m, int n, const double* a_dev, int a_is_real, int a_stride,
                       double sgn, const void* X, long ldx, void* Y, long ldy);
int chase_hip_col_scal(chase_hip_ctx* ctx, int cplx, int m, int n, const double* a_dev, int inverse, void* X, long ldx);

int chase_hip_pack_upper(chase_hip_ctx* ctx, int cplx, int n, const void* A, long lda, void* P);
int chase_hip_unpack_upper(chase_hip_ctx* ctx, int cplx, int n, const void* P, void* A, long lda, int mirror);

#ifdef __cplusplus
}
#endif
#endif
```

Before: 100,400.

## Reorder split-K tail pieces, use op N for Hermitian RR, drop dead M3 paths

Adds a piece_order mode for the split-K tail in the MFMA f64 GEMM. When every tile is a forced-split tail tile, consecutive blocks now cover 64 different tiles at the same k-chunk instead of all k-chunks of one tile, and the slab indexing is updated to match. Separately, the Rayleigh-Ritz H*Q product uses op 'N' instead of 'C' once a new device kernel confirms H is exactly Hermitian, avoiding the conjugate-transpose access pattern; that check costs one extra kernel plus a host sync per H. It also removes the unused M3 pipeline and diagnostic compile paths.

```diff
diff --git a/chase_amd/capi.py b/chase_amd/capi.py
--- a/chase_amd/capi.py
+++ b/chase_amd/capi.py
@@ -317,6 +317,7 @@
 _sig("chase_hip_op_check_symmetry", c_int, c_void_p, P(c_int))
 _sig("chase_hip_op_sym_or_herm", c_int, c_void_p, c_char)
 _sig("chase_hip_complete_hermitian", c_int, c_void_p, c_int, c_char, c_int, c_void_p, c_long)
+_sig("chase_hip_is_hermitian", c_int, c_void_p, c_int, c_int, c_void_p, c_long, P(c_int))
 _sig("chase_hip_hash64", c_int, c_void_p, c_int, c_int, c_int, c_void_p, c_long, P(C.c_ulonglong))
 _sig("chase_hip_cols_indexed", c_int, c_void_p, c_int, c_int, c_void_p, c_long, c_void_p, c_long, c_void_p, c_int)
 _sig("chase_hip_tri_mask_bc", c_int, c_void_p, c_int, c_char, c_int, c_int, c_void_p, c_long, c_long, c_int, c_int, c_long, c_int,
@@ -374,7 +375,7 @@
                                      "glds_ok", "gm", "gn")] + \
                [("full_tiles", c_long), ("tail_tiles", c_long)] + \
                [(f, c_int) for f in ("tail_sk", "tail_kchunk", "group_rows", "forced_split")] + \
-               [("slab_bytes", c_size_t), ("plane_bytes", c_size_t)]
+               [("slab_bytes", c_size_t), ("plane_bytes", c_size_t), ("piece_order", c_int)]
 
     def as_dict(self):
         return {k: getattr(self, k) for k, _ in self._fields_}
diff --git a/chase_amd/csrc/capi_blas.hip b/chase_amd/csrc/capi_blas.hip
--- a/chase_amd/csrc/capi_blas.hip
+++ b/chase_amd/csrc/capi_blas.hip
@@ -172,6 +172,25 @@
     if (!A) return set_error(CHASE_HIP_EINVAL, "complete_hermitian: NULL matrix");
     if (uplo == 'U' || uplo == 'u') KCHK(mirror_upper(c->stream, (double*)A, lda, n, ept_of(cplx)), "mirror_upper");
     else KCHK(mirror_lower(c->stream, (double*)A, lda, n, ept_of(cplx), 0), "mirror_lower");
+    return 0;
+}
+
+int chase_hip_is_hermitian(chase_hip_ctx* c, int cplx, int n, const void* A, long lda, int* out)
+{
+    if (!c || !out) return set_error(CHASE_HIP_EINVAL, "is_hermitian: NULL argument");
+    (void)hipSetDevice(c->device);
+    if (n < 0 || lda < n) return set_error(CHASE_HIP_EINVAL, "is_hermitian: bad shape");
+    *out = 1;
+    if (n == 0) return 0;
+    if (!A) return set_error(CHASE_HIP_EINVAL, "is_hermitian: NULL matrix");
+    RCCHK(c->ensure_buf(chase_hip_ctx::BUF_SCAL, 4096));
+    int* d = (int*)c->bufs[chase_hip_ctx::BUF_SCAL];
+    int bad = 0;
+    HIPCHK(hipMemsetAsync(d, 0, sizeof(int), c->stream));
+    KCHK(herm_check(c->stream, (const double*)A, lda, n, ept_of(cplx), d), "herm_check");
+    HIPCHK(hipMemcpyAsync(&bad, d, sizeof(int), hipMemcpyDeviceToHost, c->stream));
+    HIPCHK(hipStreamSynchronize(c->stream));
+    *out = bad ? 0 : 1;
     return 0;
 }
 
diff --git a/chase_amd/csrc/gemm_mfma_f64.hip b/chase_amd/csrc/gemm_mfma_f64.hip
--- a/chase_amd/csrc/gemm_mfma_f64.hip
+++ b/chase_amd/csrc/gemm_mfma_f64.hip
@@ -8,12 +8,6 @@
 #include "../../include/chase_hip.h"
 #include "kernels.h"
 
-#ifndef CHASE_M3_PIPELINE
-#define CHASE_M3_PIPELINE 1
-#endif
-#ifndef CHASE_M3_SPLANE
-#define CHASE_M3_SPLANE 1
-#endif
 #ifndef CHASE_M3_DEPTH
 #define CHASE_M3_DEPTH 2
 #endif
@@ -76,6 +70,7 @@
     int group_rows;
     int bn_cols;
     int full_tiles, tail_sk, tail_kchunk;
+    int piece_order;
     double* slabs;
     int glds_ok;
     const double* S; int s_nkt;
@@ -106,12 +101,17 @@
         tile = xcd_remap(blockIdx.x, (unsigned)p.full_tiles);
     } else {
         const unsigned P = xcd_remap(blockIdx.x - (unsigned)p.full_tiles, gridDim.x - (unsigned)p.full_tiles);
-        tile = (unsigned)p.full_tiles + P / (unsigned)p.tail_sk;
-        const int bz = (int)(P % (unsigned)p.tail_sk);
-        kbeg = bz * p.tail_kchunk;
+        unsigned tt = P / (unsigned)p.tail_sk, bz = P % (unsigned)p.tail_sk;
+        if (p.piece_order == 1) {
+            const unsigned c = P >> 6;
+            tt = (c / (unsigned)p.tail_sk) * 64u + (P & 63u);
+            bz = c % (unsigned)p.tail_sk;
+        }
+        tile = (unsigned)p.full_tiles + tt;
+        kbeg = (int)bz * p.tail_kchunk;
         kend = min(p.k, kbeg + p.tail_kchunk);
         raw = true;
-        slab = p.slabs + (size_t)P * (BM * BN * EPT);
+        slab = p.slabs + ((size_t)tt * (unsigned)p.tail_sk + bz) * (BM * BN * EPT);
     }
     int bm, bn;
     tile_coords((int)tile, p.gm, p.gn, p.group_rows, bm, bn);
@@ -341,28 +341,18 @@
             constexpr int NA = C_::A_GLDS / 4, NB = C_::B_GLDS / 4;
             const char* sa[NA];
             unsigned va[NA];
-#ifdef CHASE_DIAG_SAME_A
-            const int row0_src = 0;
-#else
-            const int row0_src = row0;
-#endif
-#ifdef CHASE_DIAG_SAME_B
-            const int col0_src = 0;
-#else
-            const int col0_src = col0;
-#endif
-            const char* sb = (const char*)(p.B + ((long)col0_src * p.ldb + kbeg) * EPT);
+            const char* sb = (const char*)(p.B + ((long)col0 * p.ldb + kbeg) * EPT);
             unsigned vb[NB];
             #pragma unroll
             for (int u = 0; u < NA; ++u) {
                 const int t = wv * NA + u;
                 if constexpr (!OPA_C) {
                     const int kk = CPLX ? (t >> 1) : t, half = CPLX ? (t & 1) : 0;
-                    sa[u] = (const char*)(p.A + ((long)(kbeg + kk) * p.lda + row0_src) * EPT + (long)half * 128);
+                    sa[u] = (const char*)(p.A + ((long)(kbeg + kk) * p.lda + row0) * EPT + (long)half * 128);
                     va[u] = (unsigned)lane * 16u;
                 } else {
                     const int rl = lane >> 3, ku = (lane & 7) ^ ((4 * t + (lane >> 4)) & 7);
-                    sa[u] = (const char*)(p.A + ((long)(row0_src + 8 * t) * p.lda + kbeg) * EPT);
+                    sa[u] = (const char*)(p.A + ((long)(row0 + 8 * t) * p.lda + kbeg) * EPT);
                     va[u] = (unsigned)(((long)rl * p.lda + ku * KPU) * EPT * 8);
                 }
             }
@@ -377,7 +367,7 @@
             constexpr long stepB = (long)BK * EPT * 8;
             int st_issue = 0;
             auto issue_one = [&](int u, int stage) __attribute__((always_inline)) {
-                constexpr bool SPLIT = CPLX && M3 && CHASE_M3_SPLANE;
+                constexpr bool SPLIT = CPLX && M3;
                 d2_t* sA = SPLIT ? lds + stage * C_::A_UNITS : lds + stage * C_::STAGE_UNITS;
                 d2_t* sB = SPLIT ? lds + C_::STAGES * C_::A_UNITS + stage * C_::B_UNITS : sA + C_::A_UNITS;
                 if (u < NA) {
@@ -443,7 +433,7 @@
                 mfma_chunk(fA, no_hook);
                 __builtin_amdgcn_sched_barrier(0);
                 mfma_chunk(fB, no_hook);
-            } else if constexpr (CPLX && M3 && CHASE_M3_SPLANE) {
+            } else if constexpr (CPLX && M3) {
                 constexpr int G = C_::GLDS_PER_WAVE;
                 constexpr int S_UNITS = 256;
                 d2_t* const sring = lds + C_::STAGES * C_::STAGE_UNITS;
@@ -494,11 +484,7 @@
                     constexpr bool fill_s = decltype(fill_s_c)::value;
                     #pragma unroll
                     for (int i = 0; i < TM; ++i) {
-#ifdef CHASE_DIAG_NO_SA
-                        const double sa = aC[i].x;
-#else
                         const double sa = OPA_C ? aC[i].x - aC[i].y : aC[i].x + aC[i].y;
-#endif
                         #pragma unroll
                         for (int j = 0; j < TN; ++j) {
                             if (!RAGGED || j < jv) {
@@ -557,96 +543,6 @@
                 cluster(st, 1, yes, no, no);
                 __builtin_amdgcn_sched_barrier(0);
                 cluster(st, 1, no, no, no);
-            } else if constexpr (CPLX && M3 && CHASE_M3_PIPELINE) {
-                constexpr int G = C_::GLDS_PER_WAVE;
-                const int npre = min(nfull, C_::STAGES);
-                for (int t = 0; t < npre; ++t) issue();
-                if (npre == 3)      asm volatile("s_waitcnt vmcnt(%0)" ::"n"(2 * G) : "memory");
-                else if (npre == 2) asm volatile("s_waitcnt vmcnt(%0)" ::"n"(G) : "memory");
-                else                asm volatile("s_waitcnt vmcnt(0)" ::: "memory");
-                __builtin_amdgcn_s_barrier();
-                asm volatile("" ::: "memory");
-                auto ld_a = [&](int stage, int ch, d2_t (&a)[TM]) __attribute__((always_inline)) {
-                    const d2_t* sA = lds + stage * C_::STAGE_UNITS;
-                    const int ku = 4 * ch + q;
-                    #pragma unroll
-                    for (int i = 0; i < TM; ++i) {
-                        const int r = wrow + 16 * i + c16;
-                        if constexpr (OPA_C) a[i] = sA[kidx(r, ku)];
-                        else                 a[i] = sA[ku * UM + r];
-                    }
-                };
-                auto ld_b = [&](int stage, int ch, int j) __attribute__((always_inline)) -> d2_t {
-                    const d2_t* sB = lds + stage * C_::STAGE_UNITS + C_::A_UNITS;
-                    return sB[kidx(wcol + 16 * j + c16, 4 * ch + q)];
-                };
-                d2_t aC[TM], aN[TM], bF[TN];
-                ld_a(0, 0, aC);
-                #pragma unroll
-                for (int j = 0; j < TN; ++j) bF[j] = ld_b(0, 0, j);
-                auto cluster = [&](int nstage, int nch, auto more_c, auto fill_c, int fstage = 0) __attribute__((always_inline)) {
-                    constexpr bool more = decltype(more_c)::value;
-                    constexpr bool fill = decltype(fill_c)::value;
-                    double sa[TM];
-                    #pragma unroll
-                    for (int i = 0; i < TM; ++i) sa[i] = OPA_C ? aC[i].x - aC[i].y : aC[i].x + aC[i].y;
-                    if (more) ld_a(nstage, nch, aN);
-                    #pragma unroll
-                    for (int j = 0; j < TN; ++j) {
-                        const double sb = bF[j].x + bF[j].y;
-                        #pragma unroll
-                        for (int i = 0; i < TM; ++i) {
-                            if (!RAGGED || j < jv) {
-                                acc[0][j][i] = __builtin_amdgcn_mfma_f64_16x16x4f64(bF[j].x, aC[i].x, acc[0][j][i], 0, 0, 0);
-                                acc[1][j][i] = __builtin_amdgcn_mfma_f64_16x16x4f64(bF[j].y, aC[i].y, acc[1][j][i], 0, 0, 0);
-                                acc[2][j][i] = __builtin_amdgcn_mfma_f64_16x16x4f64(sb, sa[i], acc[2][j][i], 0, 0, 0);
-                            }
-                            if (fill && (TM * j + i) < NA + NB) {
-                                __builtin_amdgcn_sched_barrier(0);
-                                issue_one(TM * j + i, fstage);
-                                __builtin_amdgcn_sched_barrier(0);
-                            }
-                        }
-                        if (more) bF[j] = ld_b(nstage, nch, j);
-                        __builtin_amdgcn_sched_barrier(0);
-                    }
-                    #pragma unroll
-                    for (int i = 0; i < TM; ++i) aC[i] = aN[i];
-                };
-                static_assert(TM * TN >= NA + NB, "one copy per (j, i) slot of the cluster");
-                constexpr std::true_type yes{};
-                constexpr std::false_type no{};
-                auto kstep = [&](int kt, int st, auto fill_c) __attribute__((always_inline)) {
-                    const int stn = (st + 1 == C_::STAGES) ? 0 : st + 1;
-                    cluster(st, 1, yes, no);
-                    if (C_::STAGES > 2 && (decltype(fill_c)::value || kt + 2 < nfull))
-                        asm volatile("s_waitcnt vmcnt(%0) lgkmcnt(0)" ::"n"(G) : "memory");
-                    else
-                        asm volatile("s_waitcnt vmcnt(0) lgkmcnt(0)" ::: "memory");
-                    __builtin_amdgcn_s_barrier();
-                    asm volatile("" ::: "memory");
-                    __builtin_amdgcn_sched_barrier(0);
-                    cluster(stn, 0, yes, fill_c, st);
-                };
-                int kt = 0;
-#ifdef CHASE_NO_RAGGED_C_UNROLL
-                constexpr bool unroll3 = (C_::STAGES == 3) && !(RAGGED && OPA_C);
-#else
-                constexpr bool unroll3 = (C_::STAGES == 3);
-#endif
-                if constexpr (unroll3) {
-                    for (; kt + 2 + C_::STAGES < nfull; kt += 3) {
-                        kstep(kt, 0, yes);
-                        kstep(kt + 1, 1, yes);
-                        kstep(kt + 2, 2, yes);
-                    }
-                }
-                int st = 0;
-                for (; kt + C_::STAGES < nfull; ++kt) { kstep(kt, st, yes); st = (st + 1 == C_::STAGES) ? 0 : st + 1; }
-                for (; kt + 1 < nfull; ++kt)          { kstep(kt, st, no);  st = (st + 1 == C_::STAGES) ? 0 : st + 1; }
-                cluster(st, 1, yes, no);
-                __builtin_amdgcn_sched_barrier(0);
-                cluster(st, 1, no, no);
             } else {
                 constexpr int DEPTH = C_::STAGES - 1;
                 issue();
@@ -936,7 +832,7 @@
 }
 
 struct PartDecision {
-    int gm, gn, bn_cols, group_rows;
+    int gm, gn, bn_cols, group_rows, piece_order;
     PartPlan pl;
     int kchunk;
     bool glds_ok, ragged, m3;
@@ -957,12 +853,14 @@
     d.pl = plan_part<CPLX, OPA_C, NARROW>(m, n, k, bn_cols, num_cu, min_rounds);
     if (!have_ws) d.pl = PartPlan{(long)d.gm * d.gn, 0, 1, 0};
     d.kchunk = ((nkt + d.pl.sk - 1) / d.pl.sk) * C_::BK;
+    static const int piece_env = [] { const char* e = getenv("CHASE_HIP_PIECE_ORDER"); return e ? atoi(e) : 1; }();
+    d.piece_order = (piece_env != 0 && d.pl.forced && d.pl.full == 0 && d.pl.tail % 64 == 0) ? 1 : 0;
     d.glds_ok = aligned16 && (CPLX || ((lda % 2 == 0) && (ldb % 2 == 0))) &&
                 (double)std::max(lda, ldb) * C_::BM * C_::EPT * 8 < 4.0e9;
     d.ragged = (bn_cols < C_::BN) || (d.gn * C_::BN - n) >= 16;
     d.m3 = CPLX && allow3m && gemm3m_enabled() != 0 && d.glds_ok && k > 0 && (m % C_::BM == 0) && (k % C_::BK == 0) &&
-           (d.kchunk % C_::BK == 0) && (!CHASE_M3_SPLANE || have_ws);
-    d.plane_bytes = (d.m3 && CHASE_M3_SPLANE) ? splane_bytes(n, k, bn_cols) : 0;
+           (d.kchunk % C_::BK == 0) && have_ws;
+    d.plane_bytes = d.m3 ? splane_bytes(n, k, bn_cols) : 0;
     return d;
 }
 
@@ -984,11 +882,11 @@
     a.beta_re = beta[0];   a.beta_im = CPLX ? beta[1] : 0.0;
     const long full = d.pl.full, tail = d.pl.tail;
     const int sk = d.pl.sk;
-    a.full_tiles = (int)full; a.tail_sk = sk; a.tail_kchunk = d.kchunk; a.slabs = ws;
+    a.full_tiles = (int)full; a.tail_sk = sk; a.tail_kchunk = d.kchunk; a.piece_order = d.piece_order; a.slabs = ws;
     a.glds_ok = d.glds_ok;
     const unsigned grid = (unsigned)(full + tail * sk);
     const size_t lds_bytes = (size_t)C_::STAGES * C_::STAGE_UNITS * sizeof(d2_t);
-    const size_t lds_bytes3 = lds_bytes + (CHASE_M3_SPLANE ? 2 * 4096 : 0);
+    const size_t lds_bytes3 = lds_bytes + 2 * 4096;
     const bool ragged = d.ragged;
     const int dev = (li.device >= 0 && li.device < MAX_DEVICES) ? li.device : 0;
     static std::atomic<bool> attr_set[MAX_DEVICES];
@@ -1007,7 +905,7 @@
             (void)hipFuncSetAttribute((const void*)gemm_f64_kernel<CPLX, OPA_C, TAG, true, CAN3M>, hipFuncAttributeMaxDynamicSharedMemorySize, (int)lds_bytes3);
             attr3[dev].store(true, std::memory_order_relaxed);
         }
-        if (ok3m && CHASE_M3_SPLANE) {
+        if (ok3m) {
             const size_t off = (d.pl.ws_bytes + 255) & ~(size_t)255;
             if (off + d.plane_bytes > ws_bytes) return GEMM_F64_EWORKSPACE;
             double* S = (double*)((char*)ws + off);
@@ -1114,7 +1012,7 @@
                           : plan_part<CPLX, OPA_C, false>(m, pc.n, k, pc.bn_cols, num_cu, min_rounds).ws_bytes;
         } else {
             b = plan_part<CPLX, OPA_C, false>(m, pc.n, k, pc.bn_cols, num_cu, min_rounds).ws_bytes;
-            if (CHASE_M3_SPLANE && gemm3m_enabled() != 0) b = ((b + 255) & ~(size_t)255) + splane_bytes(pc.n, k, pc.bn_cols);
+            if (gemm3m_enabled() != 0) b = ((b + 255) & ~(size_t)255) + splane_bytes(pc.n, k, pc.bn_cols);
         }
         need = std::max(need, b);
     }
@@ -1179,7 +1077,7 @@
             r.beta_one = pc.beta_one; r.bn_cols = d.bn_cols; r.narrow = pc.narrow; r.m3 = d.m3; r.ragged = d.ragged;
             r.glds_ok = d.glds_ok; r.gm = d.gm; r.gn = d.gn; r.full_tiles = d.pl.full; r.tail_tiles = d.pl.tail;
             r.tail_sk = d.pl.sk; r.tail_kchunk = d.kchunk; r.group_rows = d.group_rows; r.forced_split = d.pl.forced;
-            r.slab_bytes = d.pl.ws_bytes; r.plane_bytes = d.plane_bytes;
+            r.slab_bytes = d.pl.ws_bytes; r.plane_bytes = d.plane_bytes; r.piece_order = d.piece_order;
         }
         ++cnt;
         return 0;
diff --git a/chase_amd/csrc/kernels.h b/chase_amd/csrc/kernels.h
--- a/chase_amd/csrc/kernels.h
+++ b/chase_amd/csrc/kernels.h
@@ -51,6 +51,7 @@
 int pack_upper(hipStream_t st, const double* A, long lda, int n, int ept, double* P);
 int unpack_upper(hipStream_t st, double* P, int n, int ept, double* A, long lda);
 int mirror_upper(hipStream_t st, double* A, long lda, int n, int ept);
+int herm_check(hipStream_t st, const double* A, long lda, int n, int ept, int* flag_dev);
 int mirror_lower(hipStream_t st, double* A, long lda, int n, int ept, int zero_diag_imag = 1);
 
 int fill_normal(hipStream_t st, bool cplx, double* X, long ldx, int m, int n, long grow0, long gcol0, long gld,
diff --git a/chase_amd/csrc/vec_kernels.hip b/chase_amd/csrc/vec_kernels.hip
--- a/chase_amd/csrc/vec_kernels.hip
+++ b/chase_amd/csrc/vec_kernels.hip
@@ -382,6 +382,31 @@
     if ((threadIdx.x & 63) == 0) atomicAdd(out, acc);
 }
 
+template <int EPT>
+__global__ __launch_bounds__(256) void herm_check_kernel(const double* __restrict__ A, long lda, int n, int* __restrict__ flag)
+{
+    __shared__ double sm[EPT][32][33];
+    const int bi = blockIdx.x, bj = blockIdx.y;
+    if (bi > bj) return;
+    const int tx = threadIdx.x & 31, ty = threadIdx.x >> 5;
+    for (int c = ty; c < 32; c += 8) {
+        const int gi = 32 * bj + tx, gj = 32 * bi + c;
+        #pragma unroll
+        for (int e = 0; e < EPT; ++e) sm[e][c][tx] = (gi < n && gj < n) ? A[((long)gj * lda + gi) * EPT + e] : 0.0;
+    }
+    __syncthreads();
+    bool bad = false;
+    for (int c = ty; c < 32; c += 8) {
+        const int gi = 32 * bi + tx, gj = 32 * bj + c;
+        if (gi < n && gj < n) {
+            const double* a = A + ((long)gj * lda + gi) * EPT;
+            if (!(a[0] == sm[0][tx][c])) bad = true;
+            if (EPT == 2 && !(a[1] == -sm[EPT - 1][tx][c])) bad = true;
+        }
+    }
+    if (bad) *flag = 1;
+}
+
 __global__ void mirror_lower_kernel(double* __restrict__ A, long lda, int n, int ept, int zero_diag_imag)
 {
     const int j = blockIdx.x;
@@ -449,6 +474,14 @@
                        ld_dst_d, md, src_idx_dev, (const int*)nullptr, cnt);
     return (int)hipGetLastError();
 }
+int herm_check(hipStream_t st, const double* A, long lda, int n, int ept, int* flag_dev)
+{
+    if (n <= 0) return 0;
+    const unsigned nb = cdiv(n, 32);
+    if (ept == 2) hipLaunchKernelGGL(herm_check_kernel<2>, dim3(nb, nb), dim3(256), 0, st, A, lda, n, flag_dev);
+    else          hipLaunchKernelGGL(herm_check_kernel<1>, dim3(nb, nb), dim3(256), 0, st, A, lda, n, flag_dev);
+    return (int)hipGetLastError();
+}
 int hash64(hipStream_t st, const double* x, long ld_d, long md, int ncols, unsigned long long* out_dev)
 {
     if (md <= 0 || ncols <= 0) return 0;
diff --git a/chase_amd/host/chase_hip_impl.hpp b/chase_amd/host/chase_hip_impl.hpp
--- a/chase_amd/host/chase_hip_impl.hpp
+++ b/chase_amd/host/chase_hip_impl.hpp
@@ -106,7 +106,7 @@
     {
         if (h_on_device_) {
             hip_ok(chase_hip_complete_hermitian(ctx_, CP, uplo, (int)N_, dH_, (long)ldd_h_), "complete_hermitian");
-            hv_valid_ = false;
+            hv_valid_ = false; h_herm_ = -1;
             return;
         }
         const bool up = (uplo == 'U' || uplo == 'u');
@@ -118,7 +118,7 @@
         h_resident_ = false;
     }
 
-    void Start() override { locked_ = 0; }
+    void Start() override { locked_ = 0; h_herm_ = -1; }
 
     void initVecs(bool random) override
     {
@@ -181,7 +181,9 @@
         roctx_pop(ctx_);
     }
     void set_device_rng(bool f) override { device_rng_ = f; }
-    void reset_counters() override { filter_ms_ = 0; hemm_calls_ = 0; hemm_reused_vecs_ = 0; }
+    void set_rr_opn(bool f) override { rr_opn_ = f; }
+    std::size_t rr_opn_products() const override { return rr_opn_count_; }
+    void reset_counters() override { filter_ms_ = 0; hemm_calls_ = 0; hemm_reused_vecs_ = 0; rr_opn_count_ = 0; }
     std::size_t hemm_calls() const override { return hemm_calls_; }
     std::size_t hemm_reused_vecs() const override { return hemm_reused_vecs_; }
 
@@ -250,7 +252,7 @@
         T* Q = dV1_ + locked_ * N_;
         T* W = dV2_ + locked_ * N_;
         chase_hip_ctx_set_phase(ctx_, 2);
-        gemm('C', N_, block, N_, T(1), dH_, ldd_h_, Q, N_, T(0), W, N_);
+        gemm(rr_op(), N_, block, N_, T(1), dH_, ldd_h_, Q, N_, T(0), W, N_);
         chase_hip_ctx_set_phase(ctx_, 0);
         hip_ok(chase_hip_herkx(ctx_, CP, (int)block, (int)N_, W, (long)N_, Q, (long)N_, dA_, (long)block, 1), "herkx");
         hip_ok(chase_hip_heevd(ctx_, CP, (int)block, dA_, (long)block, ritzv), "heevd");
@@ -381,8 +383,20 @@
         if (rc) throw HipStatusError(rc, "chase_hip_malloc");
         owned_.push_back(*p);
     }
+    char rr_op()
+    {
+        if (!CP || !rr_opn_) return 'C';
+        if (h_herm_ < 0) {
+            int yes = 0;
+            hip_ok(chase_hip_is_hermitian(ctx_, CP, (int)N_, dH_, (long)ldd_h_, &yes), "is_hermitian");
+            h_herm_ = yes;
+        }
+        if (h_herm_) ++rr_opn_count_;
+        return h_herm_ ? 'N' : 'C';
+    }
     void upload_H()
     {
+        h_herm_ = -1;
         if (!h_on_device_)
             hip_ok(chase_hip_upload_matrix(ctx_, CP, (int)N_, (int)N_, H_, (long)ldh_, dH_, (long)ldd_h_), "upload H");
         h_resident_ = true;
@@ -504,6 +518,9 @@
     std::size_t locked_ = 0, lanczosIter_ = 0, numLanczos_ = 0;
     T *dH_ = nullptr, *dV1_ = nullptr, *dV2_ = nullptr, *dA_ = nullptr, *dHV_ = nullptr;
     std::size_t ldd_h_ = 0;
+    int h_herm_ = -1;
+    bool rr_opn_ = std::getenv("CHASE_HIP_RR_OPN") ? std::atoi(std::getenv("CHASE_HIP_RR_OPN")) != 0 : true;
+    std::size_t rr_opn_count_ = 0;
     bool hv_valid_ = false, resd_reuse_ = std::getenv("CHASE_HIP_RESD_REUSE") ? std::atoi(std::getenv("CHASE_HIP_RESD_REUSE")) != 0 : true;
     std::size_t hv_locked_ = 0, hv_block_ = 0, hemm_reused_vecs_ = 0;
     double hv_shift_ = 0.0;
diff --git a/chase_amd/host/impl_extras.hpp b/chase_amd/host/impl_extras.hpp
--- a/chase_amd/host/impl_extras.hpp
+++ b/chase_amd/host/impl_extras.hpp
@@ -11,6 +11,8 @@
     virtual std::size_t hemm_calls() const = 0;
     virtual std::size_t hemm_reused_vecs() const { return 0; }
     virtual std::size_t resd_rechecked() const { return 0; }
+    virtual void set_rr_opn(bool) {}
+    virtual std::size_t rr_opn_products() const { return 0; }
     virtual void set_device_rng(bool) = 0;
     virtual void reset_counters() = 0;
     virtual void* device_V1() = 0;
diff --git a/chase_amd/host/solver_capi.cpp b/chase_amd/host/solver_capi.cpp
--- a/chase_amd/host/solver_capi.cpp
+++ b/chase_amd/host/solver_capi.cpp
@@ -194,6 +194,7 @@
         else if (name == "clusteraware") c.SetClusterAwareDegrees(v != 0);
         else if (name == "upperbscale") c.SetUpperbScaleRate((float)v);
         else if (name == "device_rng") s->ex->set_device_rng(v != 0);
+        else if (name == "rr_opn") s->ex->set_rr_opn(v != 0);
         else if (name == "panel_cols" && (s->pd || s->pz)) { if (s->pz) s->pz->set_panel_cols((size_t)v); else s->pd->set_panel_cols((size_t)v); }
         else if (name == "panel_rounds" && (s->pd || s->pz)) { if (s->pz) s->pz->set_panel_rounds((int)v); else s->pd->set_panel_rounds((int)v); }
         else if (name == "pipeline" && (s->pd || s->pz)) { if (s->pz) s->pz->set_pipeline(v != 0); else s->pd->set_pipeline(v != 0); }
@@ -234,6 +235,7 @@
         else if (name == "hemm_calls") *out = (double)s->ex->hemm_calls();
         else if (name == "hemm_reused_vecs") *out = (double)s->ex->hemm_reused_vecs();
         else if (name == "resd_rechecked") *out = (double)s->ex->resd_rechecked();
+        else if (name == "rr_opn_products") *out = (double)s->ex->rr_opn_products();
         else if (name == "tape_qr_mismatches") *out = (double)s->tape.qr_variant_mismatches;
         else if (name == "tape_qr_retries") *out = (double)s->ex->forced_qr_retries();
         else if (name == "tape_tolerated") *out = (double)s->ex->replay_tolerated();
diff --git a/include/chase_hip.h b/include/chase_hip.h
--- a/include/chase_hip.h
+++ b/include/chase_hip.h
@@ -64,6 +64,7 @@
     int forced_split;
     size_t slab_bytes;
     size_t plane_bytes;
+    int piece_order;
 } chase_hip_gemm_launch;
 int chase_hip_gemm_plan(int cplx, char opA, int m, int n, int k, long lda, long ldb, int aligned16, int phase, int num_cu,
                         int min_rounds, chase_hip_gemm_launch* out, int max_out);
@@ -87,6 +88,7 @@
 int chase_hip_cols_indexed(chase_hip_ctx* ctx, int cplx, int m, const void* in, long ld_in, void* out, long ld_out,
                            const int* idx_dev, int ncols);
 int chase_hip_complete_hermitian(chase_hip_ctx* ctx, int cplx, char uplo, int n, void* A, long lda);
+int chase_hip_is_hermitian(chase_hip_ctx* ctx, int cplx, int n, const void* A, long lda, int* out);
 int chase_hip_tri_mask_bc(chase_hip_ctx* ctx, int cplx, char uplo, int mloc, int nloc, void* H, long ldh, long mb, int pr, int pi,
                           long nb, int pc, int pj);
 int chase_hip_conj_transpose_add(chase_hip_ctx* ctx, int cplx, int nr, int nc, const void* P, long ldp, const int* rowmap_dev,
```

New measurement: 100,400, median of 3. About the same (-0.0%).
